# Xiugapurin/Etude

Measured on AMD Instinct MI355X. Metric: audio-sec/s transcribed + decoder tokens/s, 3-min clip batch, higher is better.
Workload: dtype f16

## Files before the change

etude_amd/_lib.py:

```python
from __future__ import annotations

import ctypes as C
import os
from pathlib import Path

import torch

LIB_PATH = Path(os.environ["ETD_LIB_PATH"]) if os.environ.get("ETD_LIB_PATH") else Path(__file__).resolve().parent / "libetude_hip.so"

c_int_p = C.POINTER(C.c_int)
c_i32_p = C.POINTER(C.c_int32)
c_i64_p = C.POINTER(C.c_int64)
c_f32_p = C.POINTER(C.c_float)


class _SizedCfg(C.Structure):

    def __init__(self, *a, **k):
        super().__init__(*a, **k)
        self.struct_bytes = C.sizeof(type(self))


class ExtCfg(_SizedCfg):
    _fields_ = [("struct_bytes", C.c_int)] + [(n, C.c_int) for n in ("n_margin", "n_frame", "n_bin", "cnn_channel", "cnn_kernel", "hid_dim", "pf_dim",
# ... 13 lines not shown
    _fields_ = [("struct_bytes", C.c_int)] + [(n, C.c_int) for n in ("attn_len", "instr", "ntoken", "dmodel", "nhead", "d_hid", "nlayers", "norm_first",
                                       "n_mels", "tempo_out", "max_rows")]


class DbnCfg(_SizedCfg):
    _fields_ = [("struct_bytes", C.c_int), ("fps", C.c_double), ("min_bpm", C.c_double), ("max_bpm", C.c_double), ("transition_lambda", C.c_double),
                ("observation_lambda", C.c_double), ("threshold", C.c_double), ("correct", C.c_int), ("num_tempi", C.c_int), ("n_bars", C.c_int),
                ("beats_per_bar", C.c_int * 8)]


class StemFeatCfg(_SizedCfg):
    _fields_ = [("struct_bytes", C.c_int), ("n_fft", C.c_int), ("hop", C.c_int), ("n_mels", C.c_int), ("framing", C.c_int), ("amin", C.c_float), ("top_db", C.c_float)]


class DtwCfg(_SizedCfg):
    _fields_ = [("struct_bytes", C.c_int), ("cens_window", C.c_int), ("cens_decimation", C.c_int), ("reserved", C.c_int), ("step_weights", C.c_double * 3),
                ("shift_weights", C.c_double * 3), ("alpha", C.c_float), ("norm_threshold", C.c_float)]


class G3Case(_SizedCfg):
    _fields_ = [("struct_bytes", C.c_int), ("kernel", C.c_int), ("epi", C.c_int)] + [(n, C.c_int) for n in ("M", "N", "K", "ldx", "ldy")] + \
               [("X", C.c_void_p), ("x_elems", C.c_longlong), ("W", C.c_void_p), ("bias", C.c_void_p), ("x_bound", C.c_float),
                ("ln_g", C.c_void_p), ("ln_b", C.c_void_p), ("ln_eps", C.c_float), ("Y", C.c_void_p), ("y_elems", C.c_longlong),
                ("add", C.c_void_p), ("hin", C.c_void_p), ("hout", C.c_void_p), ("h_elems", C.c_longlong),
                ("pos", C.c_void_p), ("slot", C.c_void_p), ("active", C.c_void_p)] + [(n, C.c_int) for n in ("n_heads", "max_ctx", "n_slots", "rope_rows")] + \
               [("rope_cos", C.c_void_p), ("rope_sin", C.c_void_p), ("Q", C.c_void_p), ("q_elems", C.c_longlong), ("Kc", C.c_void_p), ("Vc", C.c_void_p), ("kv_elems", C.c_longlong)]


G3_KERNEL_AUTO, G3_KERNEL_TILE, G3_KERNEL_SMALL = 0, 1, 2
G3_EPI = {"bias": 0, "gelu": 1, "resid": 2, "logits": 3, "qkv": 4, "relu": 6}


class Job(C.Structure):
    _fields_ = [("x_ids", C.c_void_p), ("x_offsets", C.c_void_p), ("n_bars", C.c_int), ("attrs4", C.c_void_p), ("ready", C.c_void_p)]


class ScoreJob(C.Structure):
    _fields_ = [("x_ids", C.c_void_p), ("x_offsets", C.c_void_p), ("n_bars", C.c_int), ("attrs4", C.c_void_p),
                ("y_ids", C.c_void_p), ("y_offsets", C.c_void_p), ("n_y_bars", C.c_int)]


class SchedCfg(_SizedCfg):
    _fields_ = [("struct_bytes", C.c_int)] + [(n, C.c_int) for n in ("bar_bos_id", "bar_eos_id", "n_ctx_pairs", "max_position_embeddings", "max_output_tokens",
                                       "max_bar_token_limit")] + [("context_overlap_ratio", C.c_float)] + \
               [(n, C.c_int) for n in ("force_bar_tokens", "max_streams", "max_prefill_rows", "steps_per_poll")] + \
               [("temperature", C.c_float), ("top_p", C.c_float), ("seed", C.c_ulonglong), ("job_key_offset", C.c_int), ("job_key_stride", C.c_int)]


class TempoRegion(C.Structure):
    _fields_ = [("bpm", C.c_double), ("time_sig", C.c_int), ("start", C.c_double), ("downbeats", C.c_void_p), ("n_downbeats", C.c_int)]


class TokEvent(C.Structure):
    _fields_ = [("type", C.c_int32), ("value", C.c_int32)]


class Note(C.Structure):
    _fields_ = [("onset", C.c_double), ("offset", C.c_double), ("pitch", C.c_int32), ("velocity", C.c_int32)]


ABI_VERSION = 3

SIGNATURES = {
    "etd_version": (C.c_int, []),
    "etd_last_error": (C.c_char_p, []),
    "etd_build_id": (C.c_char_p, []),
    "etd_extractor_operand_type": (C.c_int, []),
    "etd_decoder_operand_type": (C.c_int, []),
    "etd_has_experiments": (C.c_int, []),
    "etd_prof_enable": (C.c_int, [C.c_int]),
    "etd_prof_reset": (C.c_int, []),
    "etd_prof_collect": (C.c_int, []),
    "etd_prof_count": (C.c_int, []),
    "etd_prof_entry": (C.c_int, [C.c_int, C.c_char_p, C.c_int, C.POINTER(C.c_double), C.POINTER(C.c_longlong),
                                 C.POINTER(C.c_double), C.POINTER(C.c_double)]),
    "etd_debug_boundary_cost": (C.c_int, [C.c_int, C.c_int, C.c_int, C.c_void_p, C.POINTER(C.c_double), C.POINTER(C.c_double)]),
    "etd_debug_linear": (C.c_int, [C.c_int, C.c_int, C.c_int, C.c_int, C.c_void_p, C.POINTER(C.c_double)]),
    "etd_debug_kernel_loop": (C.c_int, [C.c_int, C.c_int, C.c_void_p]),
    "etd_debug_g3_bounds": (C.c_int, [C.c_void_p, C.c_void_p, C.c_int, C.c_int, C.c_void_p, C.c_void_p, C.c_float, C.c_void_p, C.c_void_p]),
    "etd_debug_gemm3": (C.c_int, [C.c_void_p, C.c_int, C.c_int, C.c_void_p, C.c_void_p, C.c_int, C.c_float, C.c_int, C.c_void_p, C.c_void_p, C.c_void_p, C.c_void_p]),
    "etd_debug_gemm3_case": (C.c_int, [C.POINTER(G3Case), C.c_void_p]),
    "etd_debug_ln_rows_f32": (C.c_int, [C.c_void_p, C.c_int, C.c_int, C.c_void_p, C.c_void_p, C.c_void_p, C.c_void_p, C.c_float, C.c_void_p, C.c_void_p, C.c_void_p]),
    "etd_debug_g3_pack": (C.c_int, [C.c_void_p, C.c_int, C.c_int, C.c_void_p, C.c_longlong, C.POINTER(C.c_longlong), C.POINTER(C.c_int32)]),
    "etd_debug_attn3": (C.c_int, [C.c_void_p, C.c_void_p, C.c_void_p, C.c_void_p, C.c_int, C.c_int, C.c_int, C.c_int, C.c_float, C.c_float, C.c_float, C.c_int, C.c_void_p, C.c_void_p]),
    "etd_debug_empty_launch": (C.c_int, [C.c_int, C.c_int, C.c_int, C.c_void_p, C.c_void_p]),
    "etd_frontend_create": (C.c_int, [C.c_int, C.c_int, C.c_int, C.c_int, C.c_int, C.c_int, C.c_void_p, C.c_int, C.c_int,
                                      C.c_void_p, C.c_int, C.c_void_p, C.c_void_p, C.c_void_p, C.c_float, C.POINTER(C.c_void_p)]),
    "etd_frontend_destroy": (None, [C.c_void_p]),
    "etd_frontend_set_pad_mode": (C.c_int, [C.c_void_p, C.c_int]),
    "etd_rms_frames": (C.c_int, [C.c_void_p, C.c_longlong, C.c_int, C.c_int, C.c_void_p, C.c_longlong, C.c_void_p]),
    "etd_frontend_resampled_len": (C.c_longlong, [C.c_void_p, C.c_longlong]),
    "etd_frontend_num_frames": (C.c_longlong, [C.c_void_p, C.c_longlong]),
    "etd_frontend_run": (C.c_int, [C.c_void_p, C.c_void_p, C.c_int, C.c_longlong, C.c_void_p, C.c_void_p, C.c_longlong,
                                   C.POINTER(C.c_longlong), C.c_void_p]),
    "etd_extractor_create": (C.c_int, [C.POINTER(ExtCfg), C.POINTER(C.c_char_p), C.POINTER(C.c_void_p), c_i64_p, C.c_int,
                                       C.POINTER(C.c_void_p)]),
    "etd_extractor_destroy": (None, [C.c_void_p]),
    "etd_transcript": (C.c_int, [C.c_void_p, C.c_void_p, C.c_longlong] + [C.c_void_p] * 8 + [C.c_void_p]),
    "etd_transcript_windows": (C.c_int, [C.c_void_p, C.c_void_p, C.c_int] + [C.c_void_p] * 8 + [C.c_void_p]),
    "etd_extractor_debug_vel_logits": (C.c_int, [C.c_void_p, C.c_void_p]),
    "etd_extractor_debug_tap": (C.c_int, [C.c_void_p, C.c_int, C.c_void_p]),
    "etd_extractor_window_flops": (C.c_double, [C.c_void_p]),
    "etd_mpe2note": (C.c_int, [C.c_void_p, C.c_void_p, C.c_void_p, C.c_void_p, C.c_longlong, C.c_int, C.c_float, C.c_float,
                               C.c_float, C.c_int, C.c_int, C.c_int, C.POINTER(Note), C.c_longlong, C.POINTER(C.c_longlong)]),
    "etd_mpe2note_modes": (C.c_int, [C.c_void_p, C.c_void_p, C.c_void_p, C.c_void_p, C.c_longlong, C.c_int, C.c_float, C.c_float,
                                     C.c_float, C.c_int, C.c_int, C.c_int, C.c_int, C.c_int, C.POINTER(Note), C.c_longlong, C.POINTER(C.c_longlong)]),
    "etd_mpe2note_dev_create": (C.c_int, [C.c_int, C.POINTER(C.c_void_p)]),
    "etd_mpe2note_dev_destroy": (None, [C.c_void_p]),
    "etd_mpe2note_dev": (C.c_int, [C.c_void_p, C.c_void_p, C.c_void_p, C.c_void_p, C.c_void_p, C.c_longlong, C.c_float, C.c_float, C.c_float,
                                   C.c_int, C.c_int, C.c_int, C.POINTER(Note), C.c_longlong, C.POINTER(C.c_longlong), C.c_void_p]),
    "etd_mpe2note_dev_modes": (C.c_int, [C.c_void_p, C.c_void_p, C.c_void_p, C.c_void_p, C.c_void_p, C.c_longlong, C.c_float, C.c_float, C.c_float,
                                         C.c_int, C.c_int, C.c_int, C.c_int, C.c_int, C.POINTER(Note), C.c_longlong, C.POINTER(C.c_longlong), C.c_void_p]),
    "etd_tok_create": (C.c_int, [C.c_void_p, C.c_int, C.POINTER(C.c_void_p)]),
    "etd_tok_destroy": (None, [C.c_void_p]),
    "etd_tok_num_measures": (C.c_int, [C.c_void_p]),
    "etd_tok_measures": (C.c_int, [C.c_void_p, C.c_void_p, C.c_void_p, C.c_void_p, C.c_void_p]),
    "etd_tok_encode": (C.c_int, [C.c_void_p, C.c_void_p, C.c_longlong, C.c_int, C.c_void_p, C.c_longlong, C.POINTER(C.c_longlong)]),
    "etd_tok_split_bars": (C.c_int, [C.c_void_p, C.c_longlong, C.c_int, C.c_int, C.c_void_p, C.c_longlong, C.c_void_p, C.c_longlong,
                                     C.POINTER(C.c_longlong)]),
    "etd_tok_decode": (C.c_int, [C.c_void_p, C.c_void_p, C.c_longlong, C.c_void_p, C.c_longlong, C.c_void_p, C.c_longlong,
                                 C.POINTER(C.c_longlong)]),
    "etd_midi_write": (C.c_int, [C.c_void_p, C.c_longlong, C.c_char_p]),
    "etd_decoder_create": (C.c_int, [C.POINTER(DecCfg), C.POINTER(C.c_char_p), C.POINTER(C.c_void_p), c_i64_p, C.c_int,
                                     C.POINTER(C.c_void_p)]),
    "etd_decoder_destroy": (None, [C.c_void_p]),
    "etd_decoder_clone": (C.c_int, [C.c_void_p, C.POINTER(C.c_void_p)]),
    "etd_decoder_set_sampling": (C.c_int, [C.c_void_p, C.c_float, C.c_float, C.c_ulonglong, C.c_void_p]),
    "etd_decoder_set_keys": (C.c_int, [C.c_void_p, C.c_int, C.c_void_p, C.c_void_p]),
    "etd_decoder_begin_bar": (C.c_int, [C.c_void_p, C.c_int, C.c_void_p, C.c_void_p, C.c_void_p, C.c_int, C.c_void_p, C.c_int,
                                        C.c_int, C.c_void_p]),
    "etd_decoder_begin_bars": (C.c_int, [C.c_void_p, C.c_int] + [C.c_void_p] * 8 + [C.c_void_p]),
    "etd_decoder_step": (C.c_int, [C.c_void_p, C.c_void_p, C.c_int, C.c_int, C.c_void_p]),
    "etd_decoder_poll": (C.c_int, [C.c_void_p, C.c_void_p, C.c_int, C.c_void_p, C.c_void_p, C.c_void_p]),
    "etd_decoder_read_tokens": (C.c_int, [C.c_void_p, C.c_int, C.c_void_p, C.c_int, c_int_p, C.c_void_p]),
    "etd_decoder_read_many": (C.c_int, [C.c_void_p, C.c_int, C.c_void_p, C.c_void_p, C.c_int, C.c_void_p, C.c_void_p]),
    "etd_decoder_run_jobs": (C.c_int, [C.c_void_p, C.POINTER(SchedCfg), C.POINTER(Job), C.c_int, C.c_void_p, C.c_longlong, C.c_void_p,
                                       C.POINTER(C.c_longlong), C.c_void_p]),
    "etd_debug_assemble_prompt": (C.c_int, [C.POINTER(SchedCfg), C.c_int, C.c_void_p, C.c_void_p, C.c_void_p, C.c_void_p, C.c_void_p, C.c_void_p,
                                            C.c_int, C.c_void_p, C.c_void_p, C.c_void_p, C.c_void_p, C.c_int, c_int_p]),
    "etd_decoder_generate_bar": (C.c_int, [C.c_void_p, C.c_int, C.c_void_p, C.c_void_p, C.c_void_p, C.c_int, C.c_void_p,
                                           C.c_int, C.c_int, C.c_void_p, c_int_p, C.c_void_p]),
    "etd_decoder_prefill_logits": (C.c_int, [C.c_void_p, C.c_int, C.c_void_p, C.c_void_p, C.c_void_p, C.c_int, C.c_void_p,
                                             C.c_void_p]),
    "etd_decoder_score": (C.c_int, [C.c_void_p, C.c_int] + [C.c_void_p] * 11 + [C.c_void_p]),
    "etd_decoder_score_jobs": (C.c_int, [C.c_void_p, C.POINTER(SchedCfg), C.POINTER(ScoreJob), C.c_int, C.c_void_p, C.c_void_p, C.c_void_p, C.c_void_p]),
    "etd_debug_assemble_scored": (C.c_int, [C.POINTER(SchedCfg), C.c_int, C.c_void_p, C.c_void_p, C.c_void_p, C.c_void_p, C.c_void_p, C.c_void_p,
                                            C.c_int, C.c_void_p, C.c_int, C.c_void_p, C.c_void_p, C.c_void_p, C.c_void_p, C.c_void_p, C.c_int, c_int_p]),
    "etd_decoder_step_bytes": (C.c_double, [C.c_void_p, C.c_int, C.c_int]),
    "etd_decoder_stats": (C.c_int, [C.c_void_p, C.POINTER(C.c_double), C.c_int, C.c_void_p]),
    "etd_decoder_stats_reset": (C.c_int, [C.c_void_p, C.c_void_p]),
    "etd_decoder_stamp": (C.c_int, [C.c_void_p, C.c_int, C.c_int, C.c_void_p]),
    "etd_decoder_stamp_log": (C.c_int, [C.c_void_p, C.c_void_p, C.c_longlong, C.POINTER(C.c_longlong), C.c_void_p]),
    "etd_debug_decoder_force_pair": (C.c_int, [C.c_void_p, C.c_int]),
    "etd_debug_decoder_step_logits": (C.c_int, [C.c_void_p, C.c_int, C.c_void_p, C.c_int, C.c_void_p]),
    "etd_debug_decoder_checksum": (C.c_int, [C.c_void_p, C.POINTER(C.c_ulonglong), C.c_int, C.c_void_p]),
    "etd_debug_decoder_kv_rowsums": (C.c_int, [C.c_void_p, C.c_void_p, C.c_longlong, C.c_void_p]),
    "etd_debug_decoder_trace_begin": (C.c_int, [C.c_void_p, C.c_int, C.c_void_p]),
    "etd_debug_decoder_trace_slabs": (C.c_int, [C.c_void_p, C.c_void_p, C.c_longlong, C.c_int, C.c_void_p]),
    "etd_debug_decoder_trace_lanes": (C.c_int, [C.c_void_p, C.c_void_p, C.c_longlong, C.c_int, C.c_void_p]),
    "etd_debug_decoder_trace_q": (C.c_int, [C.c_void_p, C.c_void_p, C.c_longlong, C.c_int, C.c_void_p]),
    "etd_debug_decoder_peek_kv": (C.c_int, [C.c_void_p, C.c_int, C.c_int, C.c_int, C.c_int, C.c_void_p, C.c_void_p, C.c_void_p]),
    "etd_beat_create": (C.c_int, [C.POINTER(BeatCfg), C.POINTER(C.c_char_p), C.POINTER(C.c_void_p), c_i64_p, C.c_int, C.POINTER(C.c_void_p)]),
    "etd_beat_destroy": (None, [C.c_void_p]),
    "etd_beat_forward": (C.c_int, [C.c_void_p, C.c_void_p, C.c_int, c_i64_p, C.c_void_p, C.c_void_p, C.c_void_p]),
    "etd_beat_flops": (C.c_double, [C.c_void_p, C.c_longlong]),
    "etd_beat_debug_taps": (C.c_int, [C.c_void_p, C.c_void_p, C.c_void_p]),
    "etd_dbn_describe": (C.c_int, [C.POINTER(DbnCfg), C.c_int, C.c_void_p, C.c_int, c_int_p, c_int_p, c_int_p, C.c_void_p, C.c_void_p]),
    "etd_dbn_workspace_bytes": (C.c_longlong, [C.POINTER(DbnCfg), C.c_longlong, C.c_int]),
    "etd_dbn_create": (C.c_int, [C.POINTER(DbnCfg), C.POINTER(C.c_void_p)]),
    "etd_dbn_destroy": (None, [C.c_void_p]),
    "etd_dbn_track": (C.c_int, [C.c_void_p, C.c_void_p, C.c_int, C.c_int, c_i64_p, C.c_void_p, C.c_longlong, C.c_void_p, C.c_void_p, C.c_void_p, C.c_longlong,
                                C.c_void_p, C.c_void_p, C.POINTER(C.c_longlong), C.c_void_p]),
    "etd_dbn_debug_viterbi": (C.c_int, [C.c_void_p, C.c_int, C.c_void_p, C.c_longlong, C.c_void_p, C.POINTER(C.c_double)]),
    "etd_stemfeat_create": (C.c_int, [C.POINTER(StemFeatCfg), C.c_void_p, C.c_void_p, C.c_void_p, C.c_void_p, C.POINTER(C.c_void_p)]),
    "etd_stemfeat_destroy": (None, [C.c_void_p]),
    "etd_stemfeat_num_frames": (C.c_longlong, [C.c_void_p, C.c_longlong]),
    "etd_stemfeat_workspace_bytes": (C.c_longlong, [C.c_void_p, C.c_int, C.c_int, c_i64_p]),
    "etd_stemfeat_run": (C.c_int, [C.c_void_p, C.POINTER(C.c_void_p), C.c_int, C.c_int, C.c_int, c_i64_p, C.c_void_p, C.c_void_p]),
    "etd_dtw_create": (C.c_int, [C.POINTER(DtwCfg), C.POINTER(C.c_void_p)]),
    "etd_dtw_destroy": (None, [C.c_void_p]),
    "etd_dtw_limits": (C.c_int, [c_int_p, c_int_p, C.POINTER(C.c_longlong), c_int_p]),
    "etd_dtw_workspace_bytes": (C.c_longlong, [C.c_void_p, C.c_int, c_i64_p, c_i64_p, C.POINTER(C.c_longlong), c_i64_p]),
    "etd_dtw_align": (C.c_int, [C.c_void_p, C.POINTER(C.c_void_p), C.c_int, c_i64_p, c_i64_p, C.c_void_p, C.c_longlong, C.c_void_p, C.c_longlong, C.c_void_p, C.c_void_p]),
    "etd_dtw_debug_cost": (C.c_int, [C.c_void_p, C.POINTER(C.c_void_p), C.c_longlong, C.c_longlong, C.c_int, C.c_void_p]),
    "etd_dtw_debug_path": (C.c_int, [C.c_void_p, C.POINTER(C.c_void_p), C.c_longlong, C.c_longlong, C.c_int, C.c_void_p, C.c_longlong, C.POINTER(C.c_longlong)]),
    "etd_dtw_debug_total": (C.c_int, [C.c_void_p, C.POINTER(C.c_void_p), C.c_longlong, C.c_longlong, C.c_int, C.POINTER(C.c_double)]),
    "etd_debug_decoder_trace_read": (C.c_int, [C.c_void_p, C.c_void_p, C.c_longlong, C.c_int, C.POINTER(C.c_int), C.c_void_p]),
}

_lib = None


class EtudeHipError(RuntimeError):
    pass


def lib() -> C.CDLL:
    global _lib
    if _lib is None:
        if not LIB_PATH.exists():
            raise EtudeHipError(f"{LIB_PATH} not found: build it with `python -m etude_amd.build` "
                                "(hipcc --offload-arch=gfx950); etude_amd has no CPU fallback")
        l = C.CDLL(str(LIB_PATH))
        for name, (res, args) in SIGNATURES.items():
            if os.environ.get("ETD_PARTIAL") and not hasattr(l, name):
                continue
            fn = getattr(l, name)
            fn.restype = res
            fn.argtypes = args
        if l.etd_version() != ABI_VERSION:
            raise EtudeHipError(f"{LIB_PATH} speaks ABI version {l.etd_version()}, this binding {ABI_VERSION}; rebuild with `python -m etude_amd.build`")
        if not os.environ.get("ETD_PARTIAL") and not os.environ.get("ETD_ALLOW_STALE_LIB"):
            from .build import src_hash
            have, want = (l.etd_build_id() or b"").decode(), src_hash()
            if have != want:
                raise EtudeHipError(f"{LIB_PATH} is stale: built from sources {have}, the tree is {want}; rebuild with `python -m etude_amd.build`")
        _lib = l
    return _lib


def check(rc: int, what: str = "") -> None:
    if rc != 0:
        msg = lib().etd_last_error()
        raise EtudeHipError(f"{what} failed (rc={rc}): {msg.decode() if msg else ''}")


def weights_arrays(state: dict):
    import numpy as np
    names = list(state.keys())
    arrs = [np.ascontiguousarray(np.asarray(state[k], dtype=np.float32)) for k in names]
    c_names = (C.c_char_p * len(names))(*[k.encode() for k in names])
    c_ptrs = (C.c_void_p * len(names))(*[a.ctypes.data for a in arrs])
    c_num = (C.c_int64 * len(names))(*[a.size for a in arrs])
    return c_names, c_ptrs, c_num, len(names), arrs


def prof_enable(on: bool) -> None:
    lib().etd_prof_enable(1 if on else 0)


def prof_reset() -> None:
    lib().etd_prof_reset()


def prof_report() -> dict:
    l = lib()
    l.etd_prof_collect()
    out = {}
    for i in range(l.etd_prof_count()):
        name = C.create_string_buffer(64)
        ms, n, fl, by = C.c_double(), C.c_longlong(), C.c_double(), C.c_double()
        check(l.etd_prof_entry(i, name, 64, C.byref(ms), C.byref(n), C.byref(fl), C.byref(by)), "etd_prof_entry")
        out[name.value.decode()] = dict(ms=ms.value, launches=n.value, flops=fl.value, bytes=by.value)
    return out
```

etude_amd/csrc/api_dec.hip:

```cpp
#include <algorithm>
#include <atomic>
#include <chrono>
#include <cmath>
#include <cstdlib>
#include <cstring>
#include <map>
#include <string>
#include <mutex>
#include <vector>

#include "../../include/etude_hip_debug.h"
#include "dec_kernels.h"
#include "gemm3.h"
#include "ext_kernels.h"
#include "dec_score.h"
#include "prof.h"

namespace {

inline uint16_t f2bf_h(float f) { return ETD_DEC_IS_F16 ? f32_to_f16_bits(f) : f32_to_bf16_bits(f); }

struct Lin { void* W = nullptr; float* b = nullptr; int N = 0, Npad = 0, K = 0;
             void* Wf = nullptr;
             G3Lin g3; };
struct Layer { float *ln1g, *ln1b, *ln2g, *ln2b; Lin qkv, dense, up, down;
               void* dense_hw = nullptr;
               Lin cat;
               void* mlp_frag = nullptr;
               int q_log2 = 0, k_log2 = 0, v_log2 = 0; };

}

#define ETD_STAMP_WORDS (ETD_STAMP_HDR + 2 * ETD_STAMP_LOGCAP)
struct etd_dec {
  etd_dec_cfg cfg;
  DevPool pool;
  bool bf16w = false;
  int H, I, V, L, nh, S, ctx, Mmax, Mcap, out_cap;
  float *word = nullptr, *cls_emb = nullptr, *attr_tab = nullptr;
  std::vector<Layer> layers;
  float *lnfg = nullptr, *lnfb = nullptr;
  Lin head;
  float *X1f = nullptr, *X2f = nullptr;
  float *t_q = nullptr, *t_ao = nullptr, *t_do = nullptr, *t_m1 = nullptr;
  void* head_frag = nullptr;
  float *rope_cos = nullptr, *rope_sin = nullptr;
  void *Kc = nullptr, *Vc = nullptr;
  long long slot_stride = 0, layer_stride = 0;
  float *h = nullptr, *h2 = nullptr, *Q = nullptr, *AO = nullptr, *DO = nullptr, *M1 = nullptr, *logits = nullptr;
  int *row_slot = nullptr, *row_pos = nullptr, *row_active = nullptr, *row_sp = nullptr, *ids = nullptr, *slots_dev = nullptr;
  int *cur_tok = nullptr, *len = nullptr, *done = nullptr, *n_out = nullptr, *eos = nullptr, *limit = nullptr, *tgt_attrs = nullptr, *out_tok = nullptr;
  float* tgt_proj = nullptr;
  std::vector<int> last_slots;
  float* qkv_raw = nullptr;
  d16 *X1b = nullptr, *X2b = nullptr, *AOb = nullptr, *M1b = nullptr;
  d16* Qb = nullptr;
  float* hlast = nullptr;
  DSampleCfg* samp_dev = nullptr;
  unsigned long long* rng_key = nullptr;
  std::vector<unsigned long long> host_key; bool keys_dirty = true; bool sampling = false;
  float* Pk = nullptr;
  unsigned* trace = nullptr; int* trace_step = nullptr; int trace_cap = 0; float* trace_pk = nullptr; float* trace_q = nullptr; float* trace_dbg = nullptr;
  int* row_cnt = nullptr;
  d16* Xcat = nullptr;
  std::vector<int> stage;
  int* pin_stage = nullptr; size_t pin_stage_ints = 0; hipEvent_t pin_stage_evt = nullptr;
  int* pin_rb = nullptr;
  std::vector<int> host_n_out; bool host_n_out_valid = false;
  std::map<int, hipGraphExec_t> graphs;
  bool rows_identity = false;
  std::vector<int> host_len;
  double attn_bytes_hint = 0;
  bool step_pair = false;
  double stat_steps = 0, stat_row_steps = 0, stat_kv_bytes = 0, stat_attn_launches = 0, stat_stamp_bytes = 0;
  int force_pair = -1;
  unsigned long long* stamp_dev = nullptr;
  bool stamp_on = false, stamp_armed = false; long long stamp_skip = 0;
  float* logits_dbg = nullptr; bool logits_dbg_on = false, last_step_fused = false;
  int* sc_i = nullptr; float* sc_f = nullptr; double* sc_d = nullptr; float* sc_x = nullptr; int score_hb = 0;
  etd_dec* weights_owner = nullptr;
  size_t n_weight_allocs = 0;
  int n_clones = 0; bool zombie = false;
};

namespace {

int load_lin(etd_dec* d, const WeightTable& L, const std::string& pfx, int N, int K, bool has_bias, Lin* w) {
  const float* W = L.get(pfx + ".weight", (int64_t)N * K);
  if (!W) return ETD_EINVAL;
  const float* b = nullptr;
  if (has_bias) { b = L.get(pfx + ".bias", N); if (!b) return ETD_EINVAL; }
  const int Npad = ((N + 127) / 128) * 128;
  w->N = N; w->Npad = Npad; w->K = K;
  DevPool& P = d->pool;
  if (d->bf16w) {
    std::vector<uint16_t> hb((size_t)Npad * K, 0);
    for (size_t i = 0; i < (size_t)N * K; ++i) hb[i] = f2bf_h(W[i]);
    uint16_t* p; ETD_TRY(P.upload(&p, hb.data(), hb.size()));
    w->W = p;
    if (K % 16 == 0) {
      std::vector<uint16_t> hp(hb.size());
      pack_wfrag_host(hb.data(), Npad, K, hp.data());
      uint16_t* pf; ETD_TRY(P.upload(&pf, hp.data(), hp.size()));
      w->Wf = pf;
    }
  } else {
    std::vector<float> hf((size_t)Npad * K, 0.f);
    memcpy(hf.data(), W, (size_t)N * K * 4);
    float* p; ETD_TRY(P.upload(&p, hf.data(), hf.size()));
    w->W = p;
    if (K % 32 == 0) {
      ETD_TRY(g3_lin_upload(P, W, b, N, K, 0.f, &w->g3));
      w->b = w->g3.b;
      return ETD_OK;
    }
  }
  std::vector<float> hb2(Npad, 0.f);
  if (b) memcpy(hb2.data(), b, (size_t)N * 4);
  return P.upload(&w->b, hb2.data(), hb2.size());
}

int load_vec(etd_dec* d, const WeightTable& L, const std::string& name, int n, float** dst) {
  const float* p = L.get(name, n);
  if (!p) return ETD_EINVAL;
  return d->pool.upload(dst, p, n);
}

struct PrefillInfo { int n; const int* seq_row0; const int* seq_len; int max_len; double attn_flops; };
__global__ __launch_bounds__(64) void k_trace_rows(const unsigned* buf, long long row_stride, int words, long long slab_stride, int M,
                                                   unsigned* trace, const int* step, int cap, long long wps, int off) {
  const int row = blockIdx.x, slab = blockIdx.y, lane = threadIdx.x;
  const unsigned* p = buf + (long long)slab * slab_stride + (long long)row * row_stride;
  unsigned acc = 0;
  for (int i = lane; i < words; i += 64) acc += p[i] * (2654435761u * (unsigned)(i + 1) | 1u);
  for (int o = 32; o; o >>= 1) acc += __shfl_xor(acc, o);
  if (lane == 0) trace[(long long)(*step % cap) * wps + off + slab * M + row] = acc;
}
__global__ __launch_bounds__(64) void k_trace_kv(const unsigned* Kc, const unsigned* Vc, long long slot_stride_w, int max_ctx, const int* row_slot, const int* row_pos, int M,
                                                 unsigned* trace, const int* step, int cap, long long wps, int off) {
  const int row = blockIdx.x, head = blockIdx.y, lane = threadIdx.x;
  const int slot = row_slot[row], pos = row_pos[row] < max_ctx ? row_pos[row] : max_ctx - 1;
  unsigned* out = trace + (long long)(*step % cap) * wps + off;
  for (int which = 0; which < 2; ++which) {
    const unsigned* base = (which ? Vc : Kc) + (long long)slot * slot_stride_w + (long long)head * max_ctx * 32;
    unsigned a_new = 0, a_all = 0;
    for (long long i = lane; i < (long long)(pos + 1) * 32; i += 64) {
      const unsigned w = base[i] * (2654435761u * (unsigned)(i + 1) | 1u);
      a_all += w;
      if (i >= (long long)pos * 32) a_new += w;
    }
    for (int o = 32; o; o >>= 1) { a_new += __shfl_xor(a_new, o); a_all += __shfl_xor(a_all, o); }
    if (lane == 0) { out[(which * 8 + head) * M + row] = a_new; out[(16 + which * 8 + head) * M + row] = a_all; }
  }
}
__global__ void k_trace_next(int* step) { *step += 1; }
#define ETD_TRACE_LAYER 49
static inline long long trace_wps(const etd_dec* d, int M) { return (long long)(ETD_TRACE_LAYER * d->L + 2) * M; }
static int trace_rows(etd_dec* d, const void* buf, long long row_stride, int words, int nslab, long long slab_stride, int M, int off, hipStream_t st) {
  hipLaunchKernelGGL(k_trace_rows, dim3(M, nslab), dim3(64), 0, st, (const unsigned*)buf, row_stride, words, slab_stride, M, d->trace, d->trace_step,
                     d->trace_cap, trace_wps(d, M), off);
  HIP_TRY(hipGetLastError());
  return ETD_OK;
}

static inline bool fused_pmlp_on() { const char* e = getenv("ETD_FUSED_PMLP"); return !e || atoi(e) > 0; }
struct LastOnly { int n; const int* idx; DecRows rows; };
constexpr int DS_K_SPLITS = 5;
static inline bool ksplit_fits(const etd_dec* d) { return (d->I + d->H) % (DS_K_SPLITS * 64 * 8) == 0; }
static inline bool step_shape(const etd_dec* d) { return ksplit_fits(d) && d->H == 512; }
#ifdef ETD_EXPERIMENTS
static inline bool rowfin_on() { static const bool on = getenv("ETD_ROWFIN") && atoi(getenv("ETD_ROWFIN")) > 0; return on; }
#else
static inline bool rowfin_on() { return false; }
#endif

static DGemmArgs lin_args(const Lin& w, const float* X, int ldx, int M) {
  DGemmArgs a = {};
  a.X = X; a.ldx = ldx; a.M = M; a.W = w.W; a.Wf = w.Wf; a.bias = w.b; a.N = w.N; a.Npad = w.Npad; a.K = w.K; a.Wp = w.g3.Wp; a.w_log2 = w.g3.w_log2; a.x_log2 = w.g3.x_log2;
  return a;
}
static inline void* kv_layer(const etd_dec* d, void* cache, int l) { return (char*)cache + (size_t)l * d->layer_stride * (d->bf16w ? 2 : 4); }
static DGemmArgs qkv_args(const etd_dec* d, int l, const float* X, const DecRows& rows, int M) {
  DGemmArgs q = lin_args(d->layers[l].qkv, X, d->H, M);
  q.rows = rows; q.rope_cos = d->rope_cos; q.rope_sin = d->rope_sin; q.rot_half = 8; q.Q = d->Q;
  q.Kc = kv_layer(d, d->Kc, l); q.Vc = kv_layer(d, d->Vc, l); q.slot_stride = d->slot_stride; q.max_ctx = d->ctx; q.n_heads = d->nh;
  return q;
}
static DAttnArgs attn_args(const etd_dec* d, int l, const DecRows& rows, int M) {
  DAttnArgs at = {};
  at.Q = d->Q; at.Kc = kv_layer(d, d->Kc, l); at.Vc = kv_layer(d, d->Vc, l); at.slot_stride = d->slot_stride; at.max_ctx = d->ctx; at.n_heads = d->nh;
  at.rows = rows; at.M = M; at.scale = 0.125f; at.bytes_hint = d->attn_bytes_hint;
  return at;
}
static inline void attn_step_pairs(const etd_dec* d, DAttnArgs* at) { at->row_sp = d->row_sp; at->identity = d->rows_identity ? 1 : 0; }
static inline void attn_stamp(const etd_dec* d, int l, DAttnArgs* at) { at->stamp = d->stamp_on ? d->stamp_dev : nullptr; at->stamp_par = l & 1; }
struct NextLn { const float *g1, *b1, *g2, *b2; d16 *x1, *x2; };
static NextLn next_ln(const etd_dec* d, int l) {
  const Layer* nx = l + 1 < d->L ? &d->layers[l + 1] : nullptr;
  return nx ? NextLn{nx->ln1g, nx->ln1b, nx->ln2g, nx->ln2b, d->X1b, d->X2b} : NextLn{};
}
static int ln_rows16(etd_dec* d, int l, const float* h, int M, hipStream_t st) {
  const Layer& w = d->layers[l];
  return launch_ln_rows(h, M, d->H, w.ln1g, w.ln1b, w.ln2g, w.ln2b, d->cfg.layer_norm_eps, d->X1b, d->X2b, st);
}
static int layer_dattn(etd_dec* d, int l, const DecRows& rows, int M, d16* Ob, int ldob, hipStream_t st) {
  DAttnArgs at = attn_args(d, l, rows, M); at.O = d->AO; at.Ob = Ob; at.ldob = ldob;
  if (rows.slot == d->row_slot) { attn_step_pairs(d, &at); attn_stamp(d, l, &at); }
  return launch_dattn(at, d->bf16w, st);
}
static int step_qkv_up(etd_dec* d, int l, const float* X, const DecRows& rows, int M, hipStream_t st) {
  DGemmArgs q = qkv_args(d, l, X, rows, M); q.Xb = d->X1b; q.Y = d->qkv_raw; q.ldy = 3 * d->H;
  DGemmArgs up = lin_args(d->layers[l].up, X, d->H, M); up.Xb = d->X2b; up.Y = d->M1; up.Yb = d->Xcat; up.ldy = d->I + d->H;
  return launch_dstep_qkv_up(q, up, st);
}
static int resid_ln(etd_dec* d, int l, int nslab, const float* hin, float* hout, int M, const NextLn& nx, hipStream_t st) {
  return launch_resid_ln_rows(d->Pk, nslab, d->layers[l].cat.b, nullptr, hin, hout, M, d->H, nx.g1, nx.b1, nx.g2, nx.b2, d->cfg.layer_norm_eps, nx.x1, nx.x2, st);
}
static int down_splitk(etd_dec* d, int l, const float* hin, float* hout, int M, const NextLn& nx, hipStream_t st) {
  DGemmArgs dn = lin_args(d->layers[l].cat, d->M1, d->I + d->H, M); dn.Xb = d->Xcat; dn.hin = hin; dn.hout = hout; dn.k_splits = DS_K_SPLITS; dn.Y = d->Pk; dn.ldy = d->H;
  ETD_TRY(launch_dgemm(dn, DEPI_PARTIAL, true, st));
  return resid_ln(d, l, DS_K_SPLITS, hin, hout, M, nx, st);
}
static int linear16(const Lin& w, const d16* X, int M, const DGemmArgs& dec, int epi, hipStream_t st) {
  LinArgs a = {};
  a.X = (const e16*)X; a.ldx = w.K; a.W = (const e16*)w.Wf;
  a.bias = w.b; a.M = M; a.N = w.N; a.K = w.K; a.vt_block = -1; a.dec = dec;
  return launch_linear_dec(a, epi, st);
}

static int gemm3_auto(const DGemmArgs& a, int epi, hipStream_t st) { return gemm3_s_takes(a, epi) ? launch_gemm3_s(a, epi, st) : launch_gemm3(a, epi, st); }
static int x3_last_rows(etd_dec* d, const LastOnly& lo, const float* hin, float* hout, hipStream_t st) {
  const int n = lo.n, l = d->L - 1, H = d->H; const Layer& w = d->layers[l];
  ETD_TRY(launch_gather_rows(hin, lo.idx, n, H, d->hlast, st)); ETD_TRY(launch_gather_rows(d->Q, lo.idx, n, H, d->t_q, st));
  DAttnArgs at = attn_args(d, l, lo.rows, n); at.Q = d->t_q; at.O = d->t_ao; at.bytes_hint = 0;
  ETD_TRY(launch_dattn(at, false, st));
  DGemmArgs de = lin_args(w.dense, d->t_ao, H, n); de.Y = d->t_do; de.ldy = H;
  ETD_TRY(launch_dgemm(de, DEPI_BIAS, false, st));
  DGemmArgs up = lin_args(w.up, d->hlast, H, n); up.Y = d->t_m1; up.ldy = d->I; up.ln_g = w.ln2g; up.ln_b = w.ln2b; up.ln_eps = d->cfg.layer_norm_eps;
  ETD_TRY(launch_dgemm(up, DEPI_GELU, false, st));
  DGemmArgs dn = lin_args(w.down, d->t_m1, d->I, n); dn.add = d->t_do; dn.hin = d->hlast; dn.hout = hout;
  return launch_dgemm(dn, DEPI_RESID, false, st);
}
static int x3_layer_rest(etd_dec* d, int l, const DecRows& rows, int M, const PrefillInfo* pf, const float* hin, float* hout, hipStream_t st) {
  const Layer& w = d->layers[l]; const int H = d->H;
  if (pf) {
    Attn3Args t = {};
    t.Q = d->Q; t.ldq = H; t.K = (const float*)kv_layer(d, d->Kc, l); t.V = (const float*)kv_layer(d, d->Vc, l); t.O = d->AO; t.ldo = H; t.n_seq = pf->n; t.n_heads = d->nh;
    t.seq_row0 = pf->seq_row0; t.seq_len = pf->seq_len; t.row_slot = rows.slot; t.slot_stride = d->slot_stride; t.max_ctx = d->ctx; t.max_len = pf->max_len;
    t.scale = 0.125f; t.q_log2 = w.q_log2; t.k_log2 = w.k_log2; t.v_log2 = w.v_log2; t.flops_hint = pf->attn_flops;
    ETD_TRY(launch_attn3(t, st));
  } else {
    DAttnArgs at = attn_args(d, l, rows, M);
    at.O = d->AO; attn_stamp(d, l, &at);
    if (rows.slot == d->row_slot) attn_step_pairs(d, &at);
    ETD_TRY(launch_dattn(at, false, st));
  }
  DGemmArgs de = lin_args(w.dense, d->AO, H, M); de.Y = d->DO; de.ldy = H;
  ETD_TRY(gemm3_auto(de, DEPI_BIAS, st));
  DGemmArgs up = lin_args(w.up, d->X2f, H, M); up.Y = d->M1; up.ldy = d->I;
  ETD_TRY(gemm3_auto(up, DEPI_GELU, st));
  DGemmArgs dn = lin_args(w.down, d->M1, d->I, M); dn.add = d->DO; dn.hin = hin; dn.hout = hout;
  return gemm3_auto(dn, DEPI_RESID, st);
}
static int forward_x3(etd_dec* d, int M, const DecRows& rows, const PrefillInfo* pf, const LastOnly* lo, hipStream_t st, float** hfinal, bool* compact) {
  const bool tail = lo && pf && lo->n >= 1 && lo->n < G3_MIN_ROWS && lo->n <= d->S;
  float* hin = d->h; float* hout = d->h2;
  for (int l = 0; l < d->L; ++l) {
    const Layer& w = d->layers[l];
    ETD_TRY(launch_ln_rows_f32(hin, M, d->H, w.ln1g, w.ln1b, w.ln2g, w.ln2b, d->cfg.layer_norm_eps, d->X1f, d->X2f, st));
    ETD_TRY(gemm3_auto(qkv_args(d, l, d->X1f, rows, M), DEPI_QKV, st));
    ETD_TRY(tail && l == d->L - 1 ? x3_last_rows(d, *lo, hin, hout, st) : x3_layer_rest(d, l, rows, M, pf, hin, hout, st));
    std::swap(hin, hout);
  }
  *hfinal = hin; if (tail) *compact = true;
  return ETD_OK;
}

static int forward_plain(etd_dec* d, int M, const DecRows& rows, bool act16, hipStream_t st, float** hfinal) {
  float* hin = d->h; float* hout = d->h2; const float eps = d->cfg.layer_norm_eps;
  for (int l = 0; l < d->L; ++l) {
    const Layer& w = d->layers[l];
    if (act16) ETD_TRY(ln_rows16(d, l, hin, M, st));
    DGemmArgs q = qkv_args(d, l, hin, rows, M); q.Y = d->qkv_raw; q.ldy = 3 * d->H;
    if (act16) q.Xb = d->X1b; else { q.ln_g = w.ln1g; q.ln_b = w.ln1b; q.ln_eps = eps; }
    ETD_TRY(launch_dgemm(q, DEPI_QKV, d->bf16w, st));
    ETD_TRY(layer_dattn(d, l, rows, M, act16 ? d->AOb : nullptr, 0, st));
    DGemmArgs de = lin_args(w.dense, d->AO, d->H, M); de.Y = d->DO; de.ldy = d->H; if (act16) de.Xb = d->AOb;
    ETD_TRY(launch_dgemm(de, DEPI_BIAS, d->bf16w, st));
    DGemmArgs up = lin_args(w.up, hin, d->H, M); up.Y = d->M1; up.ldy = d->I;
    if (act16) { up.Xb = d->X2b; up.Yb = d->M1b; } else { up.ln_g = w.ln2g; up.ln_b = w.ln2b; up.ln_eps = eps; }
    ETD_TRY(launch_dgemm(up, DEPI_GELU, d->bf16w, st));
    DGemmArgs dn = lin_args(w.down, d->M1, d->I, M); dn.add = d->DO; dn.hin = hin; dn.hout = hout; if (act16) dn.Xb = d->M1b;
    ETD_TRY(launch_dgemm(dn, DEPI_RESID, d->bf16w, st));
    std::swap(hin, hout);
  }
  *hfinal = hin;
  return ETD_OK;
}

static int trace_qkv_up(etd_dec* d, int l, int M, hipStream_t st) {
  if (!d->trace) return ETD_OK;
  ETD_TRY(trace_rows(d, d->Q, d->H, d->H, 1, 0, M, l * ETD_TRACE_LAYER * M, st));
  if (l == 0) HIP_TRY(hipMemcpyAsync(d->trace_q, d->Q, (size_t)M * d->H * 4, hipMemcpyDeviceToDevice, st));
  ETD_TRY(trace_rows(d, d->Xcat, (d->I + d->H) / 2, d->I / 2, 1, 0, M, l * ETD_TRACE_LAYER * M + M, st));
  if (d->nh == 8) {
    hipLaunchKernelGGL(k_trace_kv, dim3(M, 8), dim3(64), 0, st, (const unsigned*)kv_layer(d, d->Kc, l), (const unsigned*)kv_layer(d, d->Vc, l), d->slot_stride / 2, d->ctx,
                       d->row_slot, d->row_pos, M, d->trace, d->trace_step, d->trace_cap, trace_wps(d, M), l * ETD_TRACE_LAYER * M + 17 * M);
    HIP_TRY(hipGetLastError());
  }
  return ETD_OK;
}
static int skinny_attn_down(etd_dec* d, int l, const DecRows& rows, int M, const float* hin, float* hout, hipStream_t st) {
  const Layer& w = d->layers[l]; const NextLn nx = next_ln(d, l);
  const int ksd = d->I / 512;
  DAttnArgs at = attn_args(d, l, rows, M);
  attn_step_pairs(d, &at); attn_stamp(d, l, &at); at.pair = d->step_pair ? 1 : 0;
  at.dense_w = (const d16*)w.dense_hw; at.dense_out = d->Pk + (size_t)ksd * M * d->H; at.dbg = (d->trace && l == 0) ? d->trace_dbg : nullptr;
  DGemmArgs dn = lin_args(w.cat, nullptr, d->I + d->H, M); dn.Xb = d->Xcat; dn.k_splits = ksd; dn.Y = d->Pk; dn.ldy = d->H;
  if (rowfin_on() && ksd + d->nh == 12 && M <= DS_STEP_MAX_ROWS) {
    DRowFin fin = {};
    fin.cnt = d->row_cnt + (size_t)l * DS_STEP_MAX_ROWS; fin.target = d->nh + 16 * ksd; fin.P = d->Pk; fin.nslab = 12;
    fin.bias = w.cat.b; fin.hin = hin; fin.hout = hout; fin.eps = d->cfg.layer_norm_eps;
    fin.g1 = nx.g1; fin.b1 = nx.b1; fin.g2 = nx.g2; fin.b2 = nx.b2; fin.x1 = nx.x1; fin.x2 = nx.x2;
    return launch_dstep_attn_down(at, dn, &fin, st);
  }
  ETD_TRY(launch_dstep_attn_down(at, dn, nullptr, st));
  if (d->trace && ksd + d->nh == 12) ETD_TRY(trace_rows(d, d->Pk, d->H, d->H, 12, (long long)M * d->H, M, l * ETD_TRACE_LAYER * M + 2 * M, st));
  if (d->trace && l == 0 && ksd + d->nh == 12) HIP_TRY(hipMemcpyAsync(d->trace_pk, d->Pk, (size_t)12 * M * d->H * 4, hipMemcpyDeviceToDevice, st));
  ETD_TRY(resid_ln(d, l, ksd + d->nh, hin, hout, M, nx, st));
  if (d->trace) {
    ETD_TRY(trace_rows(d, hout, d->H, d->H, 1, 0, M, l * ETD_TRACE_LAYER * M + 14 * M, st));
    if (nx.x1) {
      ETD_TRY(trace_rows(d, d->X1b, d->H / 2, d->H / 2, 1, 0, M, l * ETD_TRACE_LAYER * M + 15 * M, st));
      ETD_TRY(trace_rows(d, d->X2b, d->H / 2, d->H / 2, 1, 0, M, l * ETD_TRACE_LAYER * M + 16 * M, st));
    }
  }
  return ETD_OK;
}
static int forward_skinny16(etd_dec* d, int M, const DecRows& rows, bool ln0_done, hipStream_t st, float** hfinal) {
  const bool attn_down = rows.slot == d->row_slot && d->H == 512 && d->nh == 8 && d->I % 512 == 0 && d->I / 512 + d->nh <= 12 && d->layers[0].dense_hw &&
                         d->ctx >= 256 && !getenv("ETD_NO_ATTN_DOWN");
  float* hin = d->h; float* hout = d->h2;
  if (!ln0_done) ETD_TRY(ln_rows16(d, 0, hin, M, st));
  for (int l = 0; l < d->L; ++l) {
    ETD_TRY(step_qkv_up(d, l, hin, rows, M, st));
    ETD_TRY(trace_qkv_up(d, l, M, st));
    if (attn_down) ETD_TRY(skinny_attn_down(d, l, rows, M, hin, hout, st));
    else { ETD_TRY(layer_dattn(d, l, rows, M, d->Xcat + d->I, d->I + d->H, st)); ETD_TRY(down_splitk(d, l, hin, hout, M, next_ln(d, l), st)); }
    std::swap(hin, hout);
  }
  *hfinal = hin;
  return ETD_OK;
}

static int prefill16_qkv(etd_dec* d, int l, const float* hin, const DecRows& rows, int M, bool mfma_attn, hipStream_t st) {
  const Layer& w = d->layers[l];
  DGemmArgs q = qkv_args(d, l, hin, rows, M); q.Xb = d->X1b; q.Y = d->qkv_raw; q.ldy = 3 * d->H;
  if (mfma_attn) q.Qb = d->Qb;
  static const bool pqkv_on = !getenv("ETD_NO_PQKV");
  if (!(mfma_attn && pqkv_on && M >= 49152 && d->H == 512 && d->nh == 8 && w.qkv.N == 1536)) return linear16(w.qkv, d->X1b, M, q, DEPI_QKV, st);
  PQkvArgs pa = {};
  pa.X = d->X1b; pa.ldx = d->H; pa.Wf = (const d16*)w.qkv.Wf; pa.bias = w.qkv.b; pa.M = M; pa.N = w.qkv.N; pa.rows = rows;
  pa.rope_cos = d->rope_cos; pa.rope_sin = d->rope_sin; pa.Qb = d->Qb; pa.Kc = (d16*)q.Kc; pa.Vc = (d16*)q.Vc; pa.slot_stride = d->slot_stride; pa.max_ctx = d->ctx; pa.n_heads = d->nh;
  return launch_pqkv(pa, st);
}
static int prefill16_layer_rest(etd_dec* d, int l, const DecRows& rows, int M, const PrefillInfo* pf, bool fmlp, const float* hin, float* hout, hipStream_t st) {
  const Layer& w = d->layers[l];
  if (pf) {
    PAttnArgs t = {};
    t.Q = d->Qb; t.ldq = d->H; t.Kc = (const d16*)kv_layer(d, d->Kc, l); t.Vc = (const d16*)kv_layer(d, d->Vc, l); t.slot_stride = d->slot_stride; t.max_ctx = d->ctx; t.n_heads = d->nh;
    t.O = d->Xcat + d->I; t.ldo = d->I + d->H; t.seq_row0 = pf->seq_row0; t.seq_len = pf->seq_len; t.row_slot = rows.slot;
    t.n_seq = pf->n; t.max_len = pf->max_len; t.scale_log2e = 0.125f * 1.4426950408889634f; t.flops_hint = pf->attn_flops;
    ETD_TRY(launch_pattn(t, st));
  } else ETD_TRY(layer_dattn(d, l, rows, M, d->Xcat + d->I, d->I + d->H, st));
  if (fmlp) {
    const NextLn nx = next_ln(d, l); DMlpArgs ma = {};
    ma.X2 = d->X2b; ma.AO = d->Xcat + d->I; ma.ldao = d->I + d->H; ma.hin = hin; ma.hout = hout; ma.Wm = (const d16*)w.mlp_frag;
    ma.b_up = w.up.b; ma.b_cat = w.cat.b; ma.eps = d->cfg.layer_norm_eps; ma.M = M;
    ma.g1 = nx.g1; ma.b1 = nx.b1; ma.g2 = nx.g2; ma.b2 = nx.b2; ma.nx1 = nx.x1; ma.nx2 = nx.x2;
    return launch_dmlp_fused(ma, st);
  }
  DGemmArgs up = {}; up.Yb = d->Xcat; up.ldy = d->I + d->H;
  ETD_TRY(linear16(w.up, d->X2b, M, up, DEPI_GELU, st));
  DGemmArgs dn = {}; dn.N = d->H; dn.hin = hin; dn.hout = hout;
  return linear16(w.cat, d->Xcat, M, dn, DEPI_RESID, st);
}
static int prefill16_last_rows(etd_dec* d, const LastOnly& lo, const float* hin, float* hout, hipStream_t st) {
  const int n = lo.n, l = d->L - 1;
  ETD_TRY(launch_gather_rows(hin, lo.idx, n, d->H, d->hlast, st));
  ETD_TRY(ln_rows16(d, l, d->hlast, n, st));
  ETD_TRY(step_qkv_up(d, l, d->hlast, lo.rows, n, st));
  DAttnArgs at = attn_args(d, l, lo.rows, n); at.O = d->AO; at.Ob = d->Xcat + d->I; at.ldob = d->I + d->H; at.bytes_hint = 0;
  ETD_TRY(launch_dattn(at, d->bf16w, st));
  return down_splitk(d, l, d->hlast, hout, n, NextLn{}, st);
}
static int forward_prefill16(etd_dec* d, int M, const DecRows& rows, const PrefillInfo* pf, const LastOnly* lo, hipStream_t st, float** hfinal, bool* compact) {
  const bool fmlp = d->layers[0].mlp_frag && d->H == 512 && d->I == 2048 && fused_pmlp_on();
  const bool tail = lo && pf && lo->n > 1 && lo->n <= DS_STEP_MAX_ROWS && step_shape(d) && !getenv("ETD_NO_LAST_ONLY");
  float* hin = d->h; float* hout = d->h2;
  for (int l = 0; l < d->L; ++l) {
    if (l == 0 || !fmlp) ETD_TRY(ln_rows16(d, l, hin, M, st));
    ETD_TRY(prefill16_qkv(d, l, hin, rows, M, pf != nullptr, st));
    ETD_TRY(tail && l == d->L - 1 ? prefill16_last_rows(d, *lo, hin, hout, st) : prefill16_layer_rest(d, l, rows, M, pf, fmlp, hin, hout, st));
    std::swap(hin, hout);
  }
  *hfinal = hin; if (tail) *compact = true;
  return ETD_OK;
}

static int forward_rows(etd_dec* d, int M, const DecRows& rows, const PrefillInfo* pf, const LastOnly* lo, hipStream_t st, float** hfinal, bool* compact) {
  if (compact) *compact = false; else lo = nullptr;
  const Layer& w0 = d->layers[0];
  if (!d->bf16w && M >= G3_MIN_ROWS && d->X1f && w0.qkv.g3.Wp && w0.down.g3.Wp && g3_enabled()) return forward_x3(d, M, rows, pf, lo, st, hfinal, compact);
  const bool act16 = d->bf16w && M > 1;
  if (act16 && M > DS_MAX_ROWS && w0.qkv.Wf && w0.up.Wf && w0.cat.Wf) return forward_prefill16(d, M, rows, pf, lo, st, hfinal, compact);
  if (act16 && ksplit_fits(d)) return forward_skinny16(d, M, rows, false, st, hfinal);
  return forward_plain(d, M, rows, act16, st, hfinal);
}

int head_logits(etd_dec* d, const float* X, int n, float* logits, hipStream_t st) {
  const bool g3 = !d->bf16w && n >= G3_MIN_ROWS && d->X1f && d->head.g3.Wp && g3_enabled();
  if (g3) ETD_TRY(launch_ln_rows_f32(X, n, d->H, d->lnfg, d->lnfb, nullptr, nullptr, d->cfg.layer_norm_eps, d->X1f, nullptr, st));
  DGemmArgs lm = lin_args(d->head, g3 ? d->X1f : X, d->H, n);
  lm.bias = nullptr; lm.Y = logits; lm.ldy = d->V;
  if (g3) return launch_gemm3(lm, DEPI_LOGITS, st);
  lm.ln_g = d->lnfg; lm.ln_b = d->lnfb; lm.ln_eps = d->cfg.layer_norm_eps;
  return launch_dgemm(lm, DEPI_LOGITS, d->bf16w, st);
}

int check_slot(etd_dec* d, int slot) {
  if (!d || slot < 0 || slot >= d->S) ETD_FAIL(ETD_EINVAL, "decoder: bad slot %d", slot);
  return ETD_OK;
}

__global__ void k_init_slots(const int* __restrict__ init, int n, int* tgt_attrs, int* cur_tok, int* len, int* done, int* n_out, int* eos, int* limit) {
  const int i = blockIdx.x * blockDim.x + threadIdx.x;
  if (i >= n) return;
  const int* p = init + i * 7;
  const int s = p[0];
  tgt_attrs[4 * s] = p[1]; tgt_attrs[4 * s + 1] = p[2]; tgt_attrs[4 * s + 2] = p[3]; tgt_attrs[4 * s + 3] = p[4];
  cur_tok[s] = 0; len[s] = 0; done[s] = 0; n_out[s] = 0; eos[s] = p[5]; limit[s] = p[6];
}

__global__ __launch_bounds__(128) void k_slot_proj(const int* __restrict__ init, const float* __restrict__ attr_tab, int n_bins, int H, float* proj) {
  const int* p = init + blockIdx.x * 7;
  const int s = p[0];
  for (int k = threadIdx.x * 4; k < H; k += 128 * 4) {
    f32x4 t[4];
#pragma unroll
    for (int a = 0; a < 4; ++a) t[a] = *reinterpret_cast<const f32x4*>(attr_tab + (long long)(a * n_bins + p[1 + a]) * H + k);
    f32x4 o;
#pragma unroll
    for (int c = 0; c < 4; ++c) o[c] = ((t[0][c] + t[1][c]) + t[2][c]) + t[3][c];
    *reinterpret_cast<f32x4*>(proj + (long long)s * H + k) = o;
  }
}

struct Staged { int Mtot; const int *ids, *cls, *attrs, *row_slot, *row_pos, *row_active, *last_idx, *last_slot, *last_pos, *last_active, *init, *row_seq, *seq_row0, *seq_len; };

int stage_and_forward(etd_dec* d, int n, const int32_t* slots, const int32_t* T, const int32_t* ids, const int32_t* cls,
                      const int32_t* attrs4, const int32_t* init7 , Staged* sg, float** hfinal, hipStream_t st, bool* last_only = nullptr) {
  if (!d || n < 1 || n > d->S || !slots || !T || !ids || !cls || !attrs4) ETD_FAIL(ETD_EINVAL, "prefill: bad arguments");
  long long Mtot = 0;
  std::vector<char> seen((size_t)d->S, 0);
  for (int i = 0; i < n; ++i) {
    ETD_TRY(check_slot(d, slots[i]));
    if (T[i] <= 0 || T[i] > d->ctx) ETD_FAIL(ETD_EINVAL, "prefill: prompt %d has T=%d (max_ctx=%d)", i, T[i], d->ctx);
    if (seen[slots[i]]) ETD_FAIL(ETD_EINVAL, "prefill: slot %d listed twice", slots[i]);
    seen[slots[i]] = 1;
    Mtot += T[i];
  }
  if (Mtot > d->Mcap) ETD_FAIL(ETD_EINVAL, "prefill: %lld prompt rows exceed max_prefill_rows=%d", Mtot, d->Mcap);
  const int M = (int)Mtot;
  for (int i = 0; i < M; ++i) {
    if (ids[i] < 0 || ids[i] >= d->V || cls[i] < 0 || cls[i] >= d->cfg.num_classes) ETD_FAIL(ETD_EINVAL, "prefill: token/class id out of range at row %d", i);
    for (int k = 0; k < 4; ++k) if (attrs4[(size_t)k * M + i] < 0 || attrs4[(size_t)k * M + i] >= d->cfg.num_attribute_bins) ETD_FAIL(ETD_EINVAL, "prefill: attribute bin out of range at row %d", i);
  }
  const size_t sv_ints = (size_t)10 * M + 13 * n;
  int* svp;
  const bool pinned = d->pin_stage && sv_ints <= d->pin_stage_ints;
  if (pinned) {
    HIP_TRY(hipEventSynchronize(d->pin_stage_evt));
    svp = d->pin_stage;
  } else {
    d->stage.resize(sv_ints);
    svp = d->stage.data();
  }
  memcpy(svp, ids, (size_t)M * 4);
  memcpy(svp + M, cls, (size_t)M * 4);
  memcpy(svp + 2 * (size_t)M, attrs4, (size_t)4 * M * 4);
  int* rs = svp + 6 * (size_t)M; int* rp = rs + M; int* ra = rp + M;
  int* li = ra + M; int* ls = li + n; int* lp = ls + n; int* la = lp + n; int* in7 = la + n;
  int* rq = in7 + 7 * n; int* sr0 = rq + M; int* sln = sr0 + n;
  int row = 0, max_len = 0; double kvb = 0, aflops = 0;
  for (int i = 0; i < n; ++i) {
    sr0[i] = row; sln[i] = T[i]; if (T[i] > max_len) max_len = T[i];
    aflops += 0.5 * 256.0 * d->nh * (double)T[i] * T[i];
    for (int t = 0; t < T[i]; ++t, ++row) { rs[row] = slots[i]; rp[row] = t; ra[row] = 1; rq[row] = i; }
    li[i] = row - 1; ls[i] = slots[i]; lp[i] = T[i] - 1; la[i] = 1;
    d->host_len[slots[i]] = T[i];
    kvb += (double)T[i] * d->nh * 64 * (2.0 * (d->bf16w ? 2 : 4) + 4 + 4);
  }
  if (init7) memcpy(in7, init7, (size_t)7 * n * 4); else memset(in7, 0, (size_t)7 * n * 4);
  d->attn_bytes_hint = kvb;
  HIP_TRY(hipMemcpyAsync(d->ids, svp, sv_ints * 4, hipMemcpyHostToDevice, st));
  if (pinned) HIP_TRY(hipEventRecord(d->pin_stage_evt, st));
  d->host_n_out_valid = false;
  const int* b = d->ids;
  *sg = Staged{M, b, b + M, b + 2 * (size_t)M, b + 6 * (size_t)M, b + 7 * (size_t)M, b + 8 * (size_t)M, b + 9 * (size_t)M, b + 9 * (size_t)M + n,
               b + 9 * (size_t)M + 2 * n, b + 9 * (size_t)M + 3 * n, b + 9 * (size_t)M + 4 * n,
               b + 9 * (size_t)M + 11 * n, b + 10 * (size_t)M + 11 * n, b + 10 * (size_t)M + 12 * n};
  if (init7) {
    hipLaunchKernelGGL(k_init_slots, dim3((n + 63) / 64), dim3(64), 0, st, sg->init, n, d->tgt_attrs, d->cur_tok, d->len, d->done, d->n_out, d->eos, d->limit);
    HIP_TRY(hipGetLastError());
    hipLaunchKernelGGL(k_slot_proj, dim3(n), dim3(128), 0, st, sg->init, d->attr_tab, d->cfg.num_attribute_bins, d->H, d->tgt_proj);
    HIP_TRY(hipGetLastError());
  }
  DEmbedArgs e = {};
  e.ids = sg->ids; e.cls = sg->cls; e.attrs = sg->attrs; e.M = M; e.H = d->H; e.n_bins = d->cfg.num_attribute_bins;
  e.word = d->word; e.cls_emb = d->cls_emb; e.attr_tab = d->attr_tab; e.h = d->h;
  e.rows = DecRows{sg->row_slot, sg->row_pos, sg->row_active, sg->row_seq};
  ETD_TRY(launch_dembed(e, st));
  PrefillInfo pf{n, sg->seq_row0, sg->seq_len, max_len, aflops};
  const bool can_mfma_attn = (d->bf16w ? d->Qb != nullptr : d->X1f != nullptr) && !ETD_XENV("ETD_NO_MFMA_PREFILL_ATTN");
  LastOnly lo{n, sg->last_idx, DecRows{sg->last_slot, sg->last_pos, sg->last_active}};
  return forward_rows(d, M, e.rows, can_mfma_attn ? &pf : nullptr, &lo, st, hfinal, last_only);
}

int alloc_workspaces(etd_dec* d) {
  const int H = d->H;
  DevPool& P = d->pool;
  d->slot_stride = (long long)d->nh * d->ctx * 64;
  d->layer_stride = d->slot_stride * d->S;
  const size_t kv_elems = (size_t)d->layer_stride * d->L;
  if (d->bf16w) { uint16_t *k, *v; ETD_TRY(P.alloc(&k, kv_elems, true)); ETD_TRY(P.alloc(&v, kv_elems, true)); d->Kc = k; d->Vc = v; }
  else { float *k, *v; ETD_TRY(P.alloc(&k, kv_elems, true)); ETD_TRY(P.alloc(&v, kv_elems, true)); d->Kc = k; d->Vc = v; }
  const size_t M = d->Mcap;
  const size_t Mf = d->bf16w ? (size_t)(d->S > 1 ? d->S : 1) : M;
  ETD_TRY(P.alloc(&d->h, M * H)); ETD_TRY(P.alloc(&d->h2, M * H));
  ETD_TRY(P.alloc(&d->Q, M * H)); ETD_TRY(P.alloc(&d->AO, M * H)); ETD_TRY(P.alloc(&d->DO, M * H));
  ETD_TRY(P.alloc(&d->M1, Mf * d->I)); ETD_TRY(P.alloc(&d->logits, (size_t)d->Mmax * d->V));
  ETD_TRY(P.alloc(&d->qkv_raw, (size_t)3 * H)); ETD_TRY(P.alloc(&d->hlast, (size_t)d->S * H));
  if (d->bf16w) {
    ETD_TRY(P.alloc(&d->X1b, M * H)); ETD_TRY(P.alloc(&d->X2b, M * H)); ETD_TRY(P.alloc(&d->AOb, M * H));
    ETD_TRY(P.alloc(&d->M1b, M * d->I));
    ETD_TRY(P.alloc(&d->Pk, (size_t)12 * DS_STEP_MAX_ROWS * H));
    ETD_TRY(P.alloc(&d->row_cnt, (size_t)d->L * DS_STEP_MAX_ROWS, true));
    ETD_TRY(P.alloc(&d->Xcat, M * (d->I + H)));
    ETD_TRY(P.alloc(&d->Qb, M * H));
  }
  if (!d->bf16w) {
    ETD_TRY(P.alloc(&d->X1f, M * H)); ETD_TRY(P.alloc(&d->X2f, M * H));
    const size_t Sr = d->S > 1 ? d->S : 1;
    ETD_TRY(P.alloc(&d->t_q, Sr * H)); ETD_TRY(P.alloc(&d->t_ao, Sr * H)); ETD_TRY(P.alloc(&d->t_do, Sr * H)); ETD_TRY(P.alloc(&d->t_m1, Sr * d->I));
  }
  ETD_TRY(P.alloc(&d->samp_dev, (size_t)1, true)); ETD_TRY(P.alloc(&d->rng_key, (size_t)d->S, true));
// ... 368 lines not shown
    d->step_pair = d->force_pair < 0 ? pair : (d->force_pair > 0 && n_active >= 2);
  }
  d->rows_identity = true;
  for (int i = 0; i < n_active; ++i) if (slots[i] != i) { d->rows_identity = false; break; }
  const int vpad = (d->V + 31) / 32 * 32;
  static const bool fused_m1 = !(ETD_XENV("ETD_FUSED_M1") && atoi(ETD_XENV("ETD_FUSED_M1")) == 0);
  const bool fused = d->bf16w && (n_active > 1 || fused_m1) && n_active <= DS_STEP_MAX_ROWS && step_shape(d) && vpad <= 256 &&
                     vpad <= d->head.Npad && d->head_frag && !ETD_XENV("ETD_NO_FUSED_STEP");
  d->last_step_fused = fused;
  d->stamp_on = d->stamp_armed && d->stamp_skip <= 0;
  if (d->stamp_armed && d->stamp_skip > 0) d->stamp_skip -= n_steps;
  auto embed = [&](hipStream_t s_) -> int {
    DEmbedArgs e = {};
    e.slots = d->slots_dev; e.len = d->len; e.done = d->done; e.row_slot_out = d->row_slot; e.row_pos_out = d->row_pos; e.row_active_out = d->row_active; e.row_sp_out = d->row_sp;
    e.cur_tok = d->cur_tok; e.tgt_attrs = d->tgt_attrs; e.tgt_cls = 2 ;
    e.M = n_active; e.H = d->H; e.n_bins = d->cfg.num_attribute_bins;
    e.word = d->word; e.cls_emb = d->cls_emb; e.attr_tab = d->attr_tab; e.h = d->h;
    e.rows = DecRows{d->row_slot, d->row_pos, d->row_active};
    return launch_dembed(e, s_);
  };
  const double kv_row_bytes = (double)d->nh * 64 * 2 * (d->bf16w ? 2 : 4);
  auto step_kv_bytes = [&](int s) {
    double b = 0;
    for (int i = 0; i < n_active; ++i) { const int c = d->host_len[slots[i]] + 1 + s; b += (double)(c < d->ctx ? c : d->ctx) * kv_row_bytes; }
    return b;
  };
  int eager_step = 0;
  auto one_step = [&](hipStream_t s_) -> int {
    d->attn_bytes_hint = step_kv_bytes(eager_step);
    ++eager_step;
    const DecRows rows{d->row_slot, d->row_pos, d->row_active};
    if (!fused) ETD_TRY(embed(s_));
    float* hf = nullptr;
    ETD_TRY(fused ? forward_skinny16(d, n_active, rows, true, s_, &hf) : forward_rows(d, n_active, rows, nullptr, nullptr, s_, &hf, nullptr));
    if (fused) {
      ETD_TRY(launch_dstep_head(head_args(d, hf, n_active, vpad), s_));
      if (d->trace) {
        ETD_TRY(trace_rows(d, d->h, d->H, d->H, 1, 0, n_active, ETD_TRACE_LAYER * d->L * n_active, s_));
        ETD_TRY(trace_rows(d, d->cur_tok, 1, 1, 1, 0, n_active, ETD_TRACE_LAYER * d->L * n_active + n_active, s_));
        hipLaunchKernelGGL(k_trace_next, dim3(1), dim3(1), 0, s_, d->trace_step);
      }
      return ETD_OK;
    }
    ETD_TRY(head_logits(d, hf, n_active, d->logits, s_));
    DArgmaxArgs am = argmax_args(d, rows, n_active);
    am.samp = d->samp_dev; am.rng_key = d->rng_key;
    ETD_TRY(launch_dargmax(am, s_));
    return ETD_OK;
  };
  if (fused) {
    ETD_TRY(embed(st));
    ETD_TRY(ln_rows16(d, 0, d->h, n_active, st));
  }
  const bool use_graph = st != nullptr && !prof_enabled() && !ETD_XENV("ETD_NO_GRAPH");
  if (use_graph) {
    const int gkey = 16 * n_active + (d->logits_dbg_on ? 8 : 0) + (d->stamp_on ? 4 : 0) + (d->step_pair ? 2 : 0) + (d->rows_identity ? 1 : 0);
    auto it = d->graphs.find(gkey);
    if (it == d->graphs.end()) {
      hipGraph_t g = nullptr;
      HIP_TRY(hipStreamBeginCapture(st, hipStreamCaptureModeThreadLocal));
      const int rc = one_step(st);
      const hipError_t ce = hipStreamEndCapture(st, &g);
      eager_step = 0;
      if (rc != ETD_OK) { if (g) (void)hipGraphDestroy(g); return rc; }
      if (ce != hipSuccess || !g) ETD_FAIL(ETD_EHIP, "decoder_step: stream capture failed: %s", hipGetErrorString(ce));
      hipGraphExec_t ge = nullptr;
      const hipError_t ie = hipGraphInstantiate(&ge, g, nullptr, nullptr, 0);
      (void)hipGraphDestroy(g);
      if (ie != hipSuccess) ETD_FAIL(ETD_EHIP, "decoder_step: graph instantiate failed: %s", hipGetErrorString(ie));
      it = d->graphs.emplace(gkey, ge).first;
    }
    for (int s = 0; s < n_steps; ++s) HIP_TRY(hipGraphLaunch(it->second, st));
  } else {
    for (int s = 0; s < n_steps; ++s) ETD_TRY(one_step(st));
  }
  {
    double kv = 0;
    for (int s2 = 0; s2 < n_steps; ++s2) kv += step_kv_bytes(s2);
    kv *= d->L;
    d->stat_steps += n_steps; d->stat_row_steps += (double)n_steps * n_active; d->stat_kv_bytes += kv; d->stat_attn_launches += (double)n_steps * d->L;
    if (d->stamp_on) d->stat_stamp_bytes += kv + (fused ? (double)n_steps * d->L * ((double)d->I + d->H) * d->H * 2.0 : 0.0);
    for (int i = 0; i < n_active; ++i) { int& hl = d->host_len[slots[i]]; hl = hl + n_steps < d->ctx - 1 ? hl + n_steps : d->ctx - 1; }
  }
  return ETD_OK;
}

extern "C" int etd_decoder_stats(etd_dec* d, double* out, int n, void* stream) {
  if (!d || !out || n < 1) ETD_FAIL(ETD_EINVAL, "decoder_stats: bad arguments");
  unsigned long long sum_ticks = 0, n_stamped = 0;
  if (d->stamp_dev) {
    std::vector<unsigned long long> sp(ETD_STAMP_HDR);
    HIP_TRY(hipStreamSynchronize((hipStream_t)stream));
    HIP_TRY(hipMemcpy(sp.data(), d->stamp_dev, ETD_STAMP_HDR * 8, hipMemcpyDeviceToHost));
    sum_ticks = sp[0]; n_stamped = sp[1];
    for (int bank = 0; bank < 2; ++bank) {
      unsigned long long e = 0;
      for (int i = 0; i < 64; ++i) e = std::max(e, sp[8 + 64 * bank + i]);
      if (sp[2 + bank] != 0 && e > sp[2 + bank]) { sum_ticks += e - sp[2 + bank]; ++n_stamped; }
    }
  }
  double w = 0;
  for (const Layer& l : d->layers) w += ((double)l.qkv.N * l.qkv.K + (double)l.dense.N * l.dense.K + (double)l.up.N * l.up.K + (double)l.down.N * l.down.K) * (d->bf16w ? 2.0 : 4.0);
  w += (double)d->V * d->H * (d->bf16w ? 2.0 : 4.0);
  const double v[8] = {d->stat_steps, d->stat_row_steps, d->stat_kv_bytes, d->stat_attn_launches, (double)n_stamped, (double)sum_ticks * 1e-8 , d->stat_stamp_bytes, w};
  for (int i = 0; i < n; ++i) out[i] = i < 8 ? v[i] : 0.0;
  return ETD_OK;
}

extern "C" int etd_decoder_stamp_log(etd_dec* d, unsigned long long* out_pairs, long long cap, long long* n, void* stream) {
  if (!d || !out_pairs || cap < 1 || !n) ETD_FAIL(ETD_EINVAL, "decoder_stamp_log: bad arguments");
  *n = 0;
  if (!d->stamp_dev) return ETD_OK;
  std::vector<unsigned long long> sp(ETD_STAMP_WORDS);
  HIP_TRY(hipStreamSynchronize((hipStream_t)stream));
  HIP_TRY(hipMemcpy(sp.data(), d->stamp_dev, ETD_STAMP_WORDS * 8, hipMemcpyDeviceToHost));
  long long k = (long long)std::min<unsigned long long>(sp[1], ETD_STAMP_LOGCAP), w = 0;
  for (long long i = 0; i < k && w < cap; ++i, ++w) { out_pairs[2 * w] = sp[ETD_STAMP_HDR + 2 * i]; out_pairs[2 * w + 1] = sp[ETD_STAMP_HDR + 2 * i + 1]; }
  for (int bank = 0; bank < 2 && w < cap; ++bank) {
    unsigned long long e = 0;
    for (int i = 0; i < 64; ++i) e = std::max(e, sp[8 + 64 * bank + i]);
    if (sp[2 + bank] != 0 && e > sp[2 + bank]) { out_pairs[2 * w] = sp[2 + bank]; out_pairs[2 * w + 1] = e; ++w; }
  }
  *n = w;
  return ETD_OK;
}

extern "C" int etd_decoder_stats_reset(etd_dec* d, void* stream) {
  if (!d) ETD_FAIL(ETD_EINVAL, "decoder_stats_reset: null handle");
  d->stat_steps = d->stat_row_steps = d->stat_kv_bytes = d->stat_attn_launches = d->stat_stamp_bytes = 0;
  if (d->stamp_dev) {
    HIP_TRY(hipStreamSynchronize((hipStream_t)stream));
    HIP_TRY(hipMemset(d->stamp_dev, 0, ETD_STAMP_HDR * 8));
  }
  return ETD_OK;
}

extern "C" int etd_decoder_stamp(etd_dec* d, int on, int skip_steps, void* stream) {
  if (!d || skip_steps < 0) ETD_FAIL(ETD_EINVAL, "decoder_stamp: bad arguments");
  if (on && !d->stamp_dev) {
    HIP_TRY(hipMalloc((void**)&d->stamp_dev, ETD_STAMP_WORDS * 8));
    HIP_TRY(hipMemset(d->stamp_dev, 0, ETD_STAMP_WORDS * 8));
  }
  HIP_TRY(hipStreamSynchronize((hipStream_t)stream));
  d->stamp_armed = on != 0; d->stamp_on = false; d->stamp_skip = on ? skip_steps : 0;
  return ETD_OK;
}

extern "C" int etd_debug_decoder_force_pair(etd_dec* d, int mode) {
  if (!d || mode < -1 || mode > 1) ETD_FAIL(ETD_EINVAL, "force_pair: bad arguments");
  d->force_pair = mode;
  return ETD_OK;
}

extern "C" int etd_debug_decoder_step_logits(etd_dec* d, int on, float* out_host, int n_active, void* stream) {
  hipStream_t st = (hipStream_t)stream;
  if (!d || n_active < 0 || n_active > d->S) ETD_FAIL(ETD_EINVAL, "step_logits: bad arguments");
  HIP_TRY(hipStreamSynchronize(st));
  if (out_host && n_active > 0) {
    if (d->last_step_fused && !(d->logits_dbg_on && d->logits_dbg)) ETD_FAIL(ETD_EINVAL, "step_logits: the fused step stores its logits only while the hook is on");
    const float* src = d->last_step_fused ? d->logits_dbg : d->logits;
    HIP_TRY(hipMemcpy(out_host, src, (size_t)n_active * d->V * 4, hipMemcpyDeviceToHost));
  }
  if (on && !d->logits_dbg) HIP_TRY(hipMalloc((void**)&d->logits_dbg, (size_t)d->S * d->V * 4));
  d->logits_dbg_on = on != 0;
  return ETD_OK;
}

extern "C" int etd_decoder_poll(etd_dec* d, const int32_t* slots, int n, int32_t* done_out, int32_t* n_out_out, void* stream) {
  hipStream_t st = (hipStream_t)stream;
  if (!d || !slots || n < 1 || !done_out || !n_out_out) ETD_FAIL(ETD_EINVAL, "decoder_poll: bad args");
  std::vector<int> dnv, nov;
  int *dn, *no;
  if (d->pin_rb) { dn = d->pin_rb; no = d->pin_rb + d->S; }
  else { dnv.resize(d->S); nov.resize(d->S); dn = dnv.data(); no = nov.data(); }
  HIP_TRY(hipMemcpyAsync(dn, d->done, (size_t)d->S * 4, hipMemcpyDeviceToHost, st));
  HIP_TRY(hipMemcpyAsync(no, d->n_out, (size_t)d->S * 4, hipMemcpyDeviceToHost, st));
  HIP_TRY(hipStreamSynchronize(st));
  for (int i = 0; i < n; ++i) { ETD_TRY(check_slot(d, slots[i])); done_out[i] = dn[slots[i]]; n_out_out[i] = no[slots[i]]; }
  memcpy(d->host_n_out.data(), no, (size_t)d->S * 4);
  d->host_n_out_valid = true;
  return ETD_OK;
}

extern "C" int etd_decoder_read_tokens(etd_dec* d, int slot, int32_t* out, int cap, int* n, void* stream) {
  hipStream_t st = (hipStream_t)stream;
  ETD_TRY(check_slot(d, slot));
  if (!out || !n) ETD_FAIL(ETD_EINVAL, "read_tokens: null");
  int cnt = 0;
  HIP_TRY(hipMemcpyAsync(&cnt, d->n_out + slot, 4, hipMemcpyDeviceToHost, st));
  HIP_TRY(hipStreamSynchronize(st));
  if (cnt > d->out_cap) cnt = d->out_cap;
  *n = cnt;
  if (cnt > cap) ETD_FAIL(ETD_ENOMEM, "read_tokens: need room for %d tokens", cnt);
  if (cnt > 0) {
    HIP_TRY(hipMemcpyAsync(out, d->out_tok + (size_t)slot * d->out_cap, (size_t)cnt * 4, hipMemcpyDeviceToHost, st));
    HIP_TRY(hipStreamSynchronize(st));
  }
  return ETD_OK;
}

extern "C" int etd_decoder_read_many(etd_dec* d, int n, const int32_t* slots, int32_t* out, int cap, int32_t* counts, void* stream) {
  hipStream_t st = (hipStream_t)stream;
  if (!d || n < 1 || !slots || !out || !counts || cap < 1) ETD_FAIL(ETD_EINVAL, "read_many: bad args");
  for (int i = 0; i < n; ++i) ETD_TRY(check_slot(d, slots[i]));
  if (!d->host_n_out_valid) {
    HIP_TRY(hipMemcpyAsync(d->host_n_out.data(), d->n_out, (size_t)d->S * 4, hipMemcpyDeviceToHost, st));
    HIP_TRY(hipStreamSynchronize(st));
  }
  int wmax = 0;
  for (int i = 0; i < n; ++i) { int c = d->host_n_out[slots[i]]; if (c > d->out_cap) c = d->out_cap; if (c > wmax) wmax = c; }
  std::vector<int> allv;
  int* all;
  if (d->pin_rb) all = d->pin_rb + 2 * (size_t)d->S; else { allv.resize((size_t)d->S * (wmax > 0 ? wmax : 1)); all = allv.data(); }
  if (wmax > 0) {
    HIP_TRY(hipMemcpy2DAsync(all, (size_t)wmax * 4, d->out_tok, (size_t)d->out_cap * 4, (size_t)wmax * 4, (size_t)d->S, hipMemcpyDeviceToHost, st));
    HIP_TRY(hipStreamSynchronize(st));
  }
  for (int i = 0; i < n; ++i) {
    int c = d->host_n_out[slots[i]]; if (c > d->out_cap) c = d->out_cap;
    if (c > cap) ETD_FAIL(ETD_ENOMEM, "read_many: slot %d holds %d tokens (cap %d)", slots[i], c, cap);
    counts[i] = c;
    memcpy(out + (size_t)i * cap, all + (size_t)slots[i] * wmax, (size_t)c * 4);
  }
  return ETD_OK;
}

extern "C" int etd_decoder_generate_bar(etd_dec* d, int slot, const int32_t* ids, const int32_t* cls, const int32_t* attrs4, int T,
                                        const int32_t* tgt_attrs4, int eos_id, int limit, int32_t* out, int* n_out, void* stream) {
  ETD_TRY(etd_decoder_begin_bar(d, slot, ids, cls, attrs4, T, tgt_attrs4, eos_id, limit, stream));
  int dn = 0, no = 0;
  const int32_t sl = slot;
  int chunk = 8;
  while (true) {
    ETD_TRY(etd_decoder_poll(d, &sl, 1, &dn, &no, stream));
    if (dn) break;
    ETD_TRY(etd_decoder_step(d, &sl, 1, chunk, stream));
    if (chunk < 32) chunk *= 2;
  }
  return etd_decoder_read_tokens(d, slot, out, limit, n_out, stream);
}

extern "C" int etd_decoder_prefill_logits(etd_dec* d, int slot, const int32_t* ids, const int32_t* cls, const int32_t* attrs4, int T,
                                          float* logits_host, void* stream) {
  hipStream_t st = (hipStream_t)stream;
  if (!logits_host) ETD_FAIL(ETD_EINVAL, "prefill_logits: null");
  if (T > d->Mmax) ETD_FAIL(ETD_EINVAL, "prefill_logits: T=%d exceeds %d", T, d->Mmax);
  const int32_t sl = slot, tt = T;
  Staged sg; float* hf = nullptr;
  ETD_TRY(stage_and_forward(d, 1, &sl, &tt, ids, cls, attrs4, nullptr, &sg, &hf, st));
  ETD_TRY(head_logits(d, hf, T, d->logits, st));
  HIP_TRY(hipMemcpyAsync(logits_host, d->logits, (size_t)T * d->V * 4, hipMemcpyDeviceToHost, st));
  HIP_TRY(hipStreamSynchronize(st));
  return ETD_OK;
}

extern "C" int etd_decoder_score(etd_dec* d, int n, const int32_t* T, const int32_t* ids, const int32_t* cls, const int32_t* attrs4,
                                 const int32_t* labels, double* seq_logprob, int32_t* seq_tokens, int32_t* seq_hits,
                                 float* row_lp, int32_t* row_argmax, float* logits_dev, void* stream) {
  hipStream_t st = (hipStream_t)stream;
  if (!d || n < 1 || !T || !ids || !cls || !attrs4 || !labels || !seq_logprob || !seq_tokens || !seq_hits) ETD_FAIL(ETD_EINVAL, "score: bad arguments");
  long long M = 0;
  for (int i = 0; i < n; ++i) {
    if (T[i] < 1 || T[i] > d->ctx) ETD_FAIL(ETD_EINVAL, "score: sequence %d has %d rows (max_ctx=%d)", i, T[i], d->ctx);
    M += T[i];
  }
  if (M > 0x7fffffffLL) ETD_FAIL(ETD_EINVAL, "score: %lld rows in one call", M);
  for (long long r = 0; r < M; ++r) {
    if (ids[r] < 0 || ids[r] >= d->V) ETD_FAIL(ETD_EINVAL, "score: token id %d out of range [0, %d) at row %lld", ids[r], d->V, r);
    if (cls[r] < 0 || cls[r] >= d->cfg.num_classes) ETD_FAIL(ETD_EINVAL, "score: class id %d out of range [0, %d) at row %lld", cls[r], d->cfg.num_classes, r);
    for (int k = 0; k < 4; ++k)
      if (attrs4[k * M + r] < 0 || attrs4[k * M + r] >= d->cfg.num_attribute_bins) ETD_FAIL(ETD_EINVAL, "score: attribute bin %d out of range [0, %d) at row %lld", attrs4[k * M + r], d->cfg.num_attribute_bins, r);
    if (labels[r] != ETD_IGNORE_LABEL && (labels[r] < 0 || labels[r] >= d->V)) ETD_FAIL(ETD_EINVAL, "score: label %d at row %lld is neither -100 nor in [0, %d)", labels[r], r, d->V);
  }
  const int S = d->S, Mcap = d->Mcap;
  if (!d->sc_x) {
    for (void* p : {(void*)d->sc_i, (void*)d->sc_f, (void*)d->sc_d}) if (p) (void)hipFree(p);
    d->sc_i = nullptr; d->sc_f = nullptr; d->sc_d = nullptr;
    d->score_hb = d->Mmax < 256 ? d->Mmax : 256;
    const int hb = d->score_hb;
    HIP_TRY(hipMalloc((void**)&d->sc_i, ((size_t)3 * Mcap + hb + 4 * (size_t)S) * sizeof(int)));
    HIP_TRY(hipMalloc((void**)&d->sc_f, (size_t)2 * Mcap * sizeof(float)));
    HIP_TRY(hipMalloc((void**)&d->sc_d, (size_t)S * sizeof(double)));
    HIP_TRY(hipMalloc((void**)&d->sc_x, (size_t)hb * d->H * sizeof(float)));
  }
  const int hb = d->score_hb;
  int* lab_dev = d->sc_i; int* idx_dev = lab_dev + Mcap; int* r0_dev = idx_dev + Mcap + hb; int* len_dev = r0_dev + S;
  int* am_dev = len_dev + S; int* tok_dev = am_dev + Mcap; int* hit_dev = tok_dev + S;
  float* lp_dev = d->sc_f; float* lse_dev = lp_dev + Mcap;
  const int rowcap = d->bf16w ? Mcap : std::min(Mcap, G3_MIN_ROWS - 1);
  const bool full = logits_dev != nullptr;
  std::vector<int32_t> slots(S), a4c, up;
  for (int i = 0; i < S; ++i) slots[i] = i;
  long long r0 = 0;
  for (int i0 = 0; i0 < n;) {
    int k = 0; long long Mc = 0;
    while (i0 + k < n && k < S && (k == 0 || Mc + T[i0 + k] <= rowcap)) Mc += T[i0 + k++];
    const int mc = (int)Mc;
    a4c.resize((size_t)4 * mc);
    for (int a = 0; a < 4; ++a) memcpy(a4c.data() + (size_t)a * mc, attrs4 + a * M + r0, (size_t)mc * 4);
    up.assign(labels + r0, labels + r0 + mc);
    for (int r = 0; r < mc; ++r) if (full || labels[r0 + r] != ETD_IGNORE_LABEL) up.push_back(r);
    const int nl = (int)up.size() - mc;
    const int nblk = (nl + hb - 1) / hb;
    up.resize((size_t)mc + (size_t)nblk * hb, 0);
    HIP_TRY(hipMemcpyAsync(lab_dev, up.data(), (size_t)mc * 4, hipMemcpyHostToDevice, st));
    if (nblk) HIP_TRY(hipMemcpyAsync(idx_dev, up.data() + mc, (size_t)nblk * hb * 4, hipMemcpyHostToDevice, st));
// ... 156 lines not shown
```

etude_amd/csrc/dec_kernels.h:

```cpp
#pragma once
#include "common.h"

#ifdef ETD_DEC_BF16
typedef bf16 d16; typedef bf16x8 d16x8; typedef bf16x4 d16x4; typedef bf16x2 d16x2;
#define ETD_MFMA16_DEC "v_mfma_f32_32x32x16_bf16"
#define ETD_DEC_IS_F16 0
#ifdef __HIPCC__
__device__ __forceinline__ d16x4 pack4d(float a, float b, float c, float d) { return pack4(a, b, c, d); }
#endif
#else
typedef f16 d16; typedef f16x8 d16x8; typedef f16x4 d16x4; typedef f16x2 d16x2;
#define ETD_MFMA16_DEC "v_mfma_f32_32x32x16_f16"
#define ETD_DEC_IS_F16 1
#ifdef __HIPCC__
__device__ __forceinline__ d16x4 pack4d(float a, float b, float c, float d) { return pack4h(a, b, c, d); }
#endif
#endif

#define DS_MAX_ROWS 512
#define DS_STEP_MAX_ROWS 2048

struct DecRows {
  const int* slot;
  const int* pos;
  const int* active;
  const int* seq;
};

struct DSampleCfg { float inv_temp; float top_p; unsigned long long seed; };

#define ETD_STAMP_HDR (8 + 2 * 64)
#define ETD_STAMP_LOGCAP 131072

enum { DEPI_BIAS = 0, DEPI_GELU = 1, DEPI_RESID = 2, DEPI_LOGITS = 3, DEPI_QKV = 4, DEPI_PARTIAL = 5, DEPI_RELU = 6  };

struct DGemmArgs {
  const float* X; int ldx;
  const void* W;
  const void* Wf;
  const float* bias;
  int M, N, K;
  int Npad;
  const float* ln_g; const float* ln_b; float ln_eps;
  float* Y; int ldy;
  d16* Yb;
  int k_splits;
  const d16* Xb;
  const float* add; const float* hin; float* hout;
  DecRows rows;
  const float* rope_cos; const float* rope_sin;
  int rot_half;
  float* Q;
  void* Kc; void* Vc;
  long long slot_stride;
  int max_ctx, n_heads;
  d16* Qb;
  const void* Wp; int w_log2;
  int x_log2;
};
int launch_dgemm(const DGemmArgs& a, int epi, bool w_bf16, hipStream_t st);
int launch_dstep_qkv_up(const DGemmArgs& q, const DGemmArgs& up, hipStream_t st);

struct DHeadArgs {
  const float* hfin; int M, H, V, Vpad;
  const float* lnf_g; const float* lnf_b; float eps;
  const d16* Whead;
  int* row_slot; int* row_pos; int* row_active; int* row_sp;
  int* cur_tok; int* len; int* done; int* n_out; int* out_tok; int out_cap; const int* eos; const int* limit;
  const int* tgt_attrs; const float* tgt_proj ; int tgt_cls; int n_bins;
  const float* word; const float* cls_emb; const float* attr_tab;
  const float* g1; const float* b1; const float* g2; const float* b2;
  float* h; d16* x1; d16* x2;
  const DSampleCfg* samp; const unsigned long long* rng_key;
  float* logits_dbg;
};
int launch_dstep_head(const DHeadArgs& a, hipStream_t st);

struct DAttnArgs {
  const float* Q;
  const void* Kc; const void* Vc; long long slot_stride; int max_ctx, n_heads;
  DecRows rows; int M;
  const int* row_sp;
  int identity;
  int pair;
  float* O;
  d16* Ob; int ldob;
  float scale;
  double bytes_hint;
  const d16* dense_w;
  float* dense_out;
  float* dbg;
  unsigned long long* stamp;
  int stamp_par;
};
int launch_dattn(const DAttnArgs& a, bool kv_bf16, hipStream_t st);
struct DRowFin {
  int* cnt; int target;
  const float* P; int nslab;
  const float* bias; const float* hin; float* hout;
  const float* g1; const float* b1; const float* g2; const float* b2; float eps;
  d16* x1; d16* x2;
};
int launch_dstep_attn_down(const DAttnArgs& a, const DGemmArgs& down, const DRowFin* fin, hipStream_t st);

struct PAttnArgs {
  const d16* Q; int ldq;
  const d16* Kc; const d16* Vc;
  long long slot_stride; int max_ctx, n_heads;
  d16* O; int ldo;
  const int* seq_row0; const int* seq_len; const int* row_slot;
  int n_seq, max_len;
  float scale_log2e;
  double flops_hint;
};
int launch_pattn(const PAttnArgs& a, hipStream_t st);

struct PQkvArgs {
  const d16* X; int ldx;
  const d16* Wf;
  const float* bias;
  int M, N;
  DecRows rows;
  const float* rope_cos; const float* rope_sin;
  d16* Qb;
  d16* Kc; d16* Vc; long long slot_stride; int max_ctx, n_heads;
};
int launch_pqkv(const PQkvArgs& a, hipStream_t st);

int launch_ln_rows(const float* h, int M, int H, const float* g1, const float* b1, const float* g2, const float* b2, float eps,
                   d16* x1, d16* x2, hipStream_t st);
int launch_resid_ln_rows(const float* P, int k_splits, const float* bias, const float* add, const float* hin, float* hout, int M, int H,
                         const float* g1, const float* b1, const float* g2, const float* b2, float eps, d16* x1, d16* x2, hipStream_t st);
int launch_gather_rows(const float* src, const int* idx, int n, int H, float* out, hipStream_t st);

#define DMLP_NCHUNK 73
#define DMLP_STREAM_ELEMS (DMLP_NCHUNK * 32 * 1024)
struct DMlpArgs {
  const d16* X2;
  const d16* AO; int ldao;
  const float* hin; float* hout;
  const d16* Wm;
  const float* b_up;
  const float* b_cat;
  const float* g1; const float* b1; const float* g2; const float* b2; float eps;
  d16* nx1; d16* nx2;
  int M;
};
int launch_dmlp_fused(const DMlpArgs& a, hipStream_t st);
void pack_dmlp_weights(const uint16_t* Wup_bf16 , const uint16_t* Wcat_bf16 , uint16_t* dst );

struct DEmbedArgs {
  const int* ids; const int* cls; const int* attrs;
  const int* cur_tok; const int* tgt_attrs;
  int tgt_cls;
  DecRows rows; int M, H, n_bins;
  const int* slots; const int* len; const int* done;
  int* row_slot_out; int* row_pos_out; int* row_active_out; int* row_sp_out;
  const float* word; const float* cls_emb; const float* attr_tab;
  float* h;
};
int launch_dembed(const DEmbedArgs& a, hipStream_t st);

struct DArgmaxArgs {
  const float* logits; int ldl; int V; int M;
  DecRows rows;
  int* cur_tok; int* len; int* done; int* n_out; int* out_tok; int out_cap; const int* eos; const int* limit;
  int set_len_from_pos;
  const DSampleCfg* samp; const unsigned long long* rng_key;
};
int launch_dargmax(const DArgmaxArgs& a, hipStream_t st);
```

etude_amd/csrc/dec_kernels.hip:

```cpp
#include "dec_kernels.h"
#include "prof.h"

#define DLD32 36
#define DLD16 72

#include "dec_epilogue.h"

#ifdef ETD_STEP_STAMP
__device__ long long* g_ss_buf;
__device__ unsigned long long g_ss_cap;
__device__ unsigned long long g_ss_cnt;
#define SS_DECL() long long ss_t[6] = {0, 0, 0, 0, 0, 0}
#define SS(i) do { __builtin_amdgcn_sched_barrier(0); ss_t[i] = (long long)__builtin_amdgcn_s_memrealtime(); __builtin_amdgcn_sched_barrier(0); } while (0)
#define SS_LANDED() asm volatile("s_waitcnt vmcnt(0)" ::: "memory")
#define SS_FLUSH(kid, role) do { if (threadIdx.x == 0 && g_ss_buf) { const unsigned long long i_ = atomicAdd(&g_ss_cnt, 1ull); if (i_ < g_ss_cap) { long long* o_ = g_ss_buf + i_ * 8;          \
      o_[0] = (long long)(kid) | ((long long)(role) << 8) | ((long long)blockIdx.x << 16); o_[1] = ss_t[0]; o_[2] = ss_t[1]; o_[3] = ss_t[2]; o_[4] = ss_t[3]; o_[5] = ss_t[4]; o_[6] = ss_t[5];   \
      o_[7] = (long long)__builtin_amdgcn_s_getreg((20 << 0) | (0 << 6) | (3 << 11)); } } } while (0)
extern "C" int etd_debug_step_stamps(long long* dev_buf, unsigned long long cap_records, unsigned long long* count_out) {
  HIP_TRY(hipDeviceSynchronize());
  if (count_out) HIP_TRY(hipMemcpyFromSymbol(count_out, HIP_SYMBOL(g_ss_cnt), 8));
  const unsigned long long zero = 0;
  HIP_TRY(hipMemcpyToSymbol(HIP_SYMBOL(g_ss_cnt), &zero, 8));
  HIP_TRY(hipMemcpyToSymbol(HIP_SYMBOL(g_ss_buf), &dev_buf, 8));
  HIP_TRY(hipMemcpyToSymbol(HIP_SYMBOL(g_ss_cap), &cap_records, 8));
// ... 705 lines not shown
    for (int j = 0; j < 4; ++j) {
      const int rl = wave * 4 + j;
      const float rstd = rsqrtf(q4[j] / (float)H + a.eps);
#pragma unroll
      for (int half = 0; half < 2; ++half) {
        const int k = lane * 4 + half * 256;
        const f32x4 x = half ? hv1[j] : hv0[j];
        const f32x4 g = lg_[half], b = lb_[half];
        *reinterpret_cast<d16x4*>(Xs + rl * DH_LDX + k) =
            pack4d((x[0] - mean[j]) * rstd * g[0] + b[0], (x[1] - mean[j]) * rstd * g[1] + b[1], (x[2] - mean[j]) * rstd * g[2] + b[2], (x[3] - mean[j]) * rstd * g[3] + b[3]);
      }
    }
  }
  __builtin_amdgcn_sched_barrier(0);
  int statev;
  {
    const int j = lane & 3, f = (lane >> 2) < 5 ? (lane >> 2) : 5;
    const int sl = __shfl(mapv, j, 64);
    const int* sp = f == 0 ? a.cur_tok : f == 1 ? a.len : f == 2 ? a.done : f == 3 ? a.n_out : f == 4 ? a.eos : a.limit;
    statev = sp[sl];
  }
  __builtin_amdgcn_sched_barrier(0);
  HSTAMP(7);
  __syncthreads();
  HSTAMP(1);
  if (wave * 32 < a.Vpad) {
    const d16* xrow = Xs + r * DH_LDX;
    f32x16 tot;
#pragma unroll
    for (int sl = 0; sl < 8; ++sl) {
      f32x16 acc;
#pragma unroll
      for (int i = 0; i < 16; ++i) acc[i] = 0.f;
#pragma unroll
      for (int s4 = 0; s4 < 4; ++s4) {
        const int k = sl * 64 + s4 * 16 + h * 8;
        acc = mfma32(wf[sl * 4 + s4], *reinterpret_cast<const d16x8*>(xrow + k), acc);
      }
      if (sl == 0) tot = acc;
      else {
#pragma unroll
        for (int i = 0; i < 16; ++i) tot[i] += acc[i];
      }
    }
#pragma unroll
    for (int i = 0; i < 16; ++i) {
      const int f = wave * 32 + acc_row(i, h);
      if (f < a.V) Ls[r * DH_LDL + f] = tot[i];
    }
  }
  __syncthreads();
  HSTAMP(2);
  if (a.logits_dbg) {
    for (int i = tid; i < 32 * a.V; i += 512) {
      const int rr = i / a.V, f = i - rr * a.V;
      if (m0 + rr < a.M) a.logits_dbg[(long long)(m0 + rr) * a.V + f] = Ls[rr * DH_LDL + f];
    }
  }
  int gbi[4] = {0, 0, 0, 0};
  if (inv_temp > 0.f) {
#pragma unroll
    for (int j = 0; j < 4; ++j) {
      if (m0 + wave * 4 + j >= a.M) continue;
      gbi[j] = wave_sample(Ls + (wave * 4 + j) * DH_LDL, a.V, lane, inv_temp, a.samp->top_p, a.samp->seed, a.rng_key[__builtin_amdgcn_readlane(mapv, j)],
                           (unsigned)__builtin_amdgcn_readlane(statev, 12 + j), sps[wave], sss[wave], sis[wave]);
    }
  } else {
    wave_argmax4(Ls + wave * 4 * DH_LDL, DH_LDL, a.V, lane, gbi);
  }
  int n_tok[4], r_slot[4];
  {
    const int jr = lane & 3, m = m0 + wave * 4 + jr;
    const int slot = __shfl(mapv, jr, 64), act = __shfl(mapv, 4 + jr, 64), pos = __shfl(mapv, 8 + jr, 64);
    const int tok = __shfl(statev, jr, 64), len0 = __shfl(statev, 4 + jr, 64), done0 = __shfl(statev, 8 + jr, 64);
    const int n = __shfl(statev, 12 + jr, 64), eos = __shfl(statev, 16 + jr, 64), lim = __shfl(statev, 20 + jr, 64);
    const int bi = jr == 0 ? gbi[0] : jr == 1 ? gbi[1] : jr == 2 ? gbi[2] : gbi[3];
    int ntok = tok, ln = len0, dn = done0;
    const bool mine = (lane < 4) & (m < a.M);
    if (act && !done0) {
      ntok = bi; ln = pos + 1;
      const int fin = ((bi == eos) | (n + 1 >= lim)) ? 1 : 0;
      if (mine) {
        if (n < a.out_cap) a.out_tok[(long long)slot * a.out_cap + n] = bi;
        a.n_out[slot] = n + 1;
        a.cur_tok[slot] = bi;
        a.len[slot] = ln;
        if (fin) a.done[slot] = 1;
      }
      dn = fin;
    }
    if (mine) { a.row_pos[m] = ln; a.row_active[m] = dn ? 0 : 1; if (a.row_sp) a.row_sp[2 * m + 1] = ln; }
#pragma unroll
    for (int j = 0; j < 4; ++j) {
      n_tok[j] = __builtin_amdgcn_readlane(ntok, j); r_slot[j] = __builtin_amdgcn_readlane(mapv, j);
    }
  }
  HSTAMP(3);
  f32x4 r_c[2], pg1[2], pb1[2], pg2[2], pb2[2], wv[4][2], pv[4][2];
#pragma unroll
  for (int j = 0; j < 4; ++j)
#pragma unroll
    for (int hh = 0; hh < 2; ++hh) {
      wv[j][hh] = *reinterpret_cast<const f32x4*>(a.word + (long long)n_tok[j] * H + k8 + 4 * hh);
      pv[j][hh] = *reinterpret_cast<const f32x4*>(a.tgt_proj + (long long)r_slot[j] * H + k8 + 4 * hh);
    }
#pragma unroll
  for (int hh = 0; hh < 2; ++hh) {
    r_c[hh] = *reinterpret_cast<const f32x4*>(a.cls_emb + (long long)a.tgt_cls * H + k8 + 4 * hh);
    pg1[hh] = *reinterpret_cast<const f32x4*>(a.g1 + k8 + 4 * hh); pb1[hh] = *reinterpret_cast<const f32x4*>(a.b1 + k8 + 4 * hh);
    pg2[hh] = *reinterpret_cast<const f32x4*>(a.g2 + k8 + 4 * hh); pb2[hh] = *reinterpret_cast<const f32x4*>(a.b2 + k8 + 4 * hh);
  }
  {
    float v[4][8], s4[4], q4[4], mean[4];
#pragma unroll
    for (int j = 0; j < 4; ++j) {
      float s1 = 0.f;
#pragma unroll
      for (int e = 0; e < 8; ++e) {
        const int hh = e >> 2, c = e & 3;
        v[j][e] = (wv[j][hh][c] + r_c[hh][c]) + pv[j][hh][c];
        s1 += v[j][e];
      }
      s4[j] = s1;
    }
    wave_sum_n<4>(s4);
#pragma unroll
    for (int j = 0; j < 4; ++j) {
      mean[j] = s4[j] / (float)H;
      float q = 0.f;
#pragma unroll
      for (int e = 0; e < 8; ++e) { const float d0 = v[j][e] - mean[j]; q += d0 * d0; }
      q4[j] = q;
    }
    wave_sum_n<4>(q4);
#pragma unroll
    for (int j = 0; j < 4; ++j) {
      const int m = m0 + wave * 4 + j;
      if (m >= a.M) continue;
      const long long ro = (long long)m * H;
      { const f32x4 oa = {v[j][0], v[j][1], v[j][2], v[j][3]}, ob = {v[j][4], v[j][5], v[j][6], v[j][7]};
        *reinterpret_cast<f32x4*>(a.h + ro + k8) = oa; *reinterpret_cast<f32x4*>(a.h + ro + k8 + 4) = ob; }
      const float rstd = rsqrtf(q4[j] / (float)H + a.eps);
      d16x8 o1, o2;
#pragma unroll
      for (int e = 0; e < 8; ++e) {
        o1[e] = (d16)((v[j][e] - mean[j]) * rstd * pg1[e >> 2][e & 3] + pb1[e >> 2][e & 3]);
        o2[e] = (d16)((v[j][e] - mean[j]) * rstd * pg2[e >> 2][e & 3] + pb2[e >> 2][e & 3]);
      }
      *reinterpret_cast<d16x8*>(a.x1 + ro + k8) = o1;
      *reinterpret_cast<d16x8*>(a.x2 + ro + k8) = o2;
    }
  }
  HSTAMP(4);
  SS_FLUSH(0, 0);
}

#ifdef ETD_HEAD_STAMP
extern "C" int etd_debug_head_stamps(long long* out) {
  HIP_TRY(hipDeviceSynchronize());
  HIP_TRY(hipMemcpyFromSymbol(out, HIP_SYMBOL(g_head_stamp), sizeof(long long) * 8 * 16));
  return ETD_OK;
}
#endif
int launch_dstep_head(const DHeadArgs& a, hipStream_t st) {
  if (a.samp && !a.rng_key) ETD_FAIL(ETD_EINVAL, "dstep_head: sampling needs stream keys");
  if (a.M < 1 || a.H != 512 || a.V < 1 || a.V > a.Vpad || a.Vpad % 32 || a.Vpad > 256 || !a.hfin || !a.Whead || !a.tgt_proj || !a.h || !a.x1 || !a.x2)
    ETD_FAIL(ETD_EINVAL, "dstep_head: bad arguments (needs hidden 512, vocabulary <= 256)");
  ProfScope ps("k_dstep_head", st, 2.0 * a.M * a.V * a.H, (double)a.Vpad * a.H * 2);
  hipLaunchKernelGGL(k_dstep_head, dim3((a.M + 31) / 32), dim3(512), 0, st, a.hfin, a.M, a.row_slot, a.row_active, a.row_pos, a);
  HIP_TRY(hipGetLastError());
  return ETD_OK;
}

__device__ __forceinline__ float fma_scalar(float a, float b, float c) {
  asm volatile("v_fma_f32 %0, %1, %2, %0" : "+v"(c) : "v"(a), "v"(b));
  return c;
}
template <bool WBF16, int EPI>
__global__ __launch_bounds__(256) void k_dgemv(DGemmArgs a) {
  const int tid = threadIdx.x, lane = tid & 63, wave = tid >> 6;
  const int nb = (blockIdx.x * 4 + wave) * 4;
  const bool ln = a.ln_g != nullptr;
  float mean = 0.f, rstd = 1.f;
  if (ln) {
    float s = 0.f;
    for (int k = lane * 4; k < a.K; k += 256) { const f32x4 v = *reinterpret_cast<const f32x4*>(a.X + k); s += v[0] + v[1] + v[2] + v[3]; }
    s = wave_sum(s);
    mean = s / (float)a.K;
    float q = 0.f;
    for (int k = lane * 4; k < a.K; k += 256) {
      const f32x4 v = *reinterpret_cast<const f32x4*>(a.X + k);
      const float d0 = v[0] - mean, d1 = v[1] - mean, d2 = v[2] - mean, d3 = v[3] - mean;
      q += d0 * d0 + d1 * d1 + d2 * d2 + d3 * d3;
    }
    q = wave_sum(q);
    rstd = rsqrtf(q / (float)a.K + a.ln_eps);
  }
  float acc[4] = {0.f, 0.f, 0.f, 0.f};
  for (int k = lane * 8; k < a.K; k += 512) {
    f32x4 x0 = *reinterpret_cast<const f32x4*>(a.X + k), x1 = *reinterpret_cast<const f32x4*>(a.X + k + 4);
    if (ln) {
      const f32x4 g0 = *reinterpret_cast<const f32x4*>(a.ln_g + k), g1 = *reinterpret_cast<const f32x4*>(a.ln_g + k + 4);
      const f32x4 b0 = *reinterpret_cast<const f32x4*>(a.ln_b + k), b1 = *reinterpret_cast<const f32x4*>(a.ln_b + k + 4);
#pragma unroll
      for (int j = 0; j < 4; ++j) { x0[j] = (x0[j] - mean) * rstd * g0[j] + b0[j]; x1[j] = (x1[j] - mean) * rstd * g1[j] + b1[j]; }
    }
#pragma unroll
    for (int f = 0; f < 4; ++f) {
      float w[8];
      if constexpr (WBF16) {
        const d16x8 wv = *reinterpret_cast<const d16x8*>(reinterpret_cast<const d16*>(a.W) + (long long)(nb + f) * a.K + k);
#pragma unroll
        for (int j = 0; j < 8; ++j) w[j] = bf2f(wv[j]);
#pragma unroll
        for (int j = 0; j < 4; ++j) { acc[f] = fmaf(w[j], bf2f((d16)x0[j]), acc[f]); acc[f] = fmaf(w[4 + j], bf2f((d16)x1[j]), acc[f]); }
      } else {
        const float* wp = reinterpret_cast<const float*>(a.W) + (long long)(nb + f) * a.K + k;
        const f32x4 w0 = *reinterpret_cast<const f32x4*>(wp), w1 = *reinterpret_cast<const f32x4*>(wp + 4);
#pragma unroll
        for (int j = 0; j < 4; ++j) { acc[f] = fma_scalar(w0[j], x0[j], acc[f]); acc[f] = fma_scalar(w1[j], x1[j], acc[f]); }
      }
    }
  }
#pragma unroll
  for (int f = 0; f < 4; ++f) acc[f] = wave_sum(acc[f]);
  if (lane != 0) return;
#pragma unroll
  for (int f = 0; f < 4; ++f) {
    const int n = nb + f;
    if (n >= a.N) break;
    float v = acc[f];
    if (EPI != DEPI_LOGITS) v += a.bias[n];
    if (EPI == DEPI_GELU) v = gelu_erf(v);
    if (EPI == DEPI_RESID) a.hout[n] = (v + a.add[n]) + a.hin[n];
    else a.Y[n] = v;
  }
}

template <typename KVT>
__global__ void k_rope_scatter(DGemmArgs a, const float* __restrict__ raw) {
  const int m = blockIdx.x;
  const int pos = a.rows.pos[m], slot = a.rows.slot[m];
  const bool act = a.rows.active[m] && pos < a.max_ctx;
  const int H3 = a.n_heads * 192;
  for (int n = threadIdx.x; n < H3; n += blockDim.x) {
    const int head = n / 192, j = n - head * 192, part = j >> 6, d = j & 63;
    float v = raw[(long long)m * H3 + n];
    if (part < 2 && d < 2 * a.rot_half) {
      const int dd = d < a.rot_half ? d : d - a.rot_half;
      const float c = a.rope_cos[(long long)pos * a.rot_half + dd], s = a.rope_sin[(long long)pos * a.rot_half + dd];
      const float other = raw[(long long)m * H3 + (d < a.rot_half ? n + a.rot_half : n - a.rot_half)];
      v = d < a.rot_half ? v * c - other * s : v * c + other * s;
    }
    if (part == 0) a.Q[(long long)m * (a.n_heads * 64) + head * 64 + d] = v;
    else if (act) {
      const long long off = (long long)slot * a.slot_stride + ((long long)head * a.max_ctx + pos) * 64 + d;
      KVT* base = reinterpret_cast<KVT*>(part == 1 ? a.Kc : a.Vc);
      base[off] = (KVT)v;
    }
  }
}

template <bool WBF16>
static void dgemm_dispatch(const DGemmArgs& a, int epi, int path, hipStream_t st) {
  const int wtiles = (a.Npad / 32) * (a.k_splits > 1 ? a.k_splits : 1);
  const dim3 g0((a.M + 31) / 32, a.Npad / 128), g1((unsigned)(((wtiles + 7) / 8) * 8 * ((a.M + 31) / 32))), g2(a.Npad / 16);
#define ETD_DG(E)                                                                                   \
  if (path == 0) hipLaunchKernelGGL((k_dgemm<WBF16, E>), g0, dim3(256), 0, st, a);                  \
  else if (path == 1) hipLaunchKernelGGL((k_dgemm_s<WBF16, E>), g1, dim3(64 * DS_WAVES), 0, st, a.M, a.Npad, a.k_splits, a.K, a.W, a.Xb, a.ldx, a);  \
  else hipLaunchKernelGGL((k_dgemv<WBF16, E>), g2, dim3(256), 0, st, a);
  switch (epi) {
    case DEPI_BIAS: ETD_DG(DEPI_BIAS) break;
    case DEPI_GELU: ETD_DG(DEPI_GELU) break;
    case DEPI_RESID: ETD_DG(DEPI_RESID) break;
    case DEPI_LOGITS: ETD_DG(DEPI_LOGITS) break;
    case DEPI_PARTIAL: hipLaunchKernelGGL((k_dgemm_s<WBF16, DEPI_PARTIAL>), g1, dim3(64 * DS_WAVES), 0, st, a.M, a.Npad, a.k_splits, a.K, a.W, a.Xb, a.ldx, a); break;
    default:
      if (path == 0) hipLaunchKernelGGL((k_dgemm<WBF16, DEPI_QKV>), g0, dim3(256), 0, st, a);
      else hipLaunchKernelGGL((k_dgemm_s<WBF16, DEPI_QKV>), g1, dim3(64 * DS_WAVES), 0, st, a.M, a.Npad, a.k_splits, a.K, a.W, a.Xb, a.ldx, a);
      break;
  }
#undef ETD_DG
}

bool g3_enabled();
bool gemm3_s_takes(const DGemmArgs& a, int epi);
int launch_gemm3_s(const DGemmArgs& a, int epi, hipStream_t st);
int launch_dgemm(const DGemmArgs& a, int epi, bool w_bf16, hipStream_t st) {
  const bool g3s_on = g3_enabled();
  if (!w_bf16 && g3s_on && gemm3_s_takes(a, epi)) return launch_gemm3_s(a, epi, st);
  if (a.M <= 0 || a.Npad % 128 || a.K % 256 || a.N > a.Npad) ETD_FAIL(ETD_EINVAL, "dgemm: bad shape M=%d N=%d Npad=%d K=%d", a.M, a.N, a.Npad, a.K);
  if (epi == DEPI_QKV && (a.rot_half != 8 || a.N % 192)) ETD_FAIL(ETD_EINVAL, "dgemm: QKV epilogue needs head_dim 64 and rotary_ndims 16");
  if (epi == DEPI_RESID && (a.N % 4)) ETD_FAIL(ETD_EINVAL, "dgemm: resid needs N %% 4 == 0");
  const int path = a.M == 1 ? 2 : (a.M <= DS_MAX_ROWS || (epi == DEPI_PARTIAL && a.M <= DS_STEP_MAX_ROWS) ? 1 : 0);
  if (epi == DEPI_PARTIAL && (path != 1 || a.k_splits < 1 || (a.K / a.k_splits) % (64 * DS_WAVES) || !a.Y)) ETD_FAIL(ETD_EINVAL, "dgemm: bad split-K request");
  if (epi != DEPI_PARTIAL && a.k_splits > 1) ETD_FAIL(ETD_EINVAL, "dgemm: k_splits needs DEPI_PARTIAL");
  ProfScope ps(path == 2 ? "k_dgemv" : (path == 1 ? "k_dgemm_s" : "k_dgemm"), st, 2.0 * a.M * a.N * a.K, (double)a.Npad * a.K * (w_bf16 ? 2 : 4));
  if (path == 2 && epi == DEPI_QKV) {
    if (!a.Y) ETD_FAIL(ETD_EINVAL, "dgemm: M == 1 QKV path needs a scratch row in Y");
    if (w_bf16) { dgemm_dispatch<true>(a, DEPI_BIAS, 2, st); hipLaunchKernelGGL(k_rope_scatter<d16>, dim3(1), dim3(256), 0, st, a, a.Y); }
    else { dgemm_dispatch<false>(a, DEPI_BIAS, 2, st); hipLaunchKernelGGL(k_rope_scatter<float>, dim3(1), dim3(256), 0, st, a, a.Y); }
  } else if (w_bf16) dgemm_dispatch<true>(a, epi, path, st);
  else dgemm_dispatch<false>(a, epi, path, st);
  HIP_TRY(hipGetLastError());
  return ETD_OK;
}

template <typename KVT> struct Raw8;
template <> struct Raw8<float> {
  f32x4 a, b;
  __device__ __forceinline__ void load(const float* p) { a = *reinterpret_cast<const f32x4*>(p); b = *reinterpret_cast<const f32x4*>(p + 4); }
  __device__ __forceinline__ float get(int j) const { return j < 4 ? a[j] : b[j - 4]; }
};
template <> struct Raw8<d16> {
  d16x8 v;
  __device__ __forceinline__ void load(const d16* p) { v = __builtin_nontemporal_load(reinterpret_cast<const d16x8*>(p)); }
  __device__ __forceinline__ float get(int j) const { return bf2f(v[j]); }
};

#ifndef ETD_FIN_ZB
#define ETD_FIN_ZB 12
#endif
typedef __amdgpu_buffer_rsrc_t drsrc_t;
__device__ __forceinline__ drsrc_t d_rsrc(const void* p, long long bytes) {
  return __builtin_amdgcn_make_buffer_rsrc(const_cast<void*>(p), 0, (int)(bytes > 0x7fffffffLL ? 0x7fffffffLL : bytes), 0x00020000);
}
#define D_SC1 16
__device__ __forceinline__ void row_finish(const DRowFin& f, const int row_in, const int M_in, const int lane) {
  const int row = __builtin_amdgcn_readfirstlane(row_in), M = __builtin_amdgcn_readfirstlane(M_in);
  const drsrc_t ps = d_rsrc(f.P, (long long)f.nslab * M * 512 * 4);
  const long long ro = (long long)row * 512;
  const int k = lane * 8;
  float acc[8];
#pragma unroll
  for (int j = 0; j < 8; ++j) acc[j] = 0.f;
  const f32x4 ba = *reinterpret_cast<const f32x4*>(f.bias + k), bb = *reinterpret_cast<const f32x4*>(f.bias + k + 4);
  const f32x4 ha = *reinterpret_cast<const f32x4*>(f.hin + ro + k), hb = *reinterpret_cast<const f32x4*>(f.hin + ro + k + 4);
  f32x4 pg1[2], pb1[2], pg2[2], pb2[2];
  if (f.x1) {
#pragma unroll
    for (int hh = 0; hh < 2; ++hh) {
      pg1[hh] = *reinterpret_cast<const f32x4*>(f.g1 + k + 4 * hh); pb1[hh] = *reinterpret_cast<const f32x4*>(f.b1 + k + 4 * hh);
      pg2[hh] = *reinterpret_cast<const f32x4*>(f.g2 + k + 4 * hh); pb2[hh] = *reinterpret_cast<const f32x4*>(f.b2 + k + 4 * hh);
    }
  }
  constexpr int ZB = ETD_FIN_ZB;
#pragma unroll
  for (int z0 = 0; z0 < 12; z0 += ZB) {
    f32x4 pa[ZB], pb[ZB];
#pragma unroll
    for (int z = 0; z < ZB; ++z) {
      const int so = (int)((((long long)(z0 + z) * M + row) * 512) * 4);
      pa[z] = __builtin_bit_cast(f32x4, __builtin_amdgcn_raw_buffer_load_b128(ps, k * 4, so, D_SC1));
      pb[z] = __builtin_bit_cast(f32x4, __builtin_amdgcn_raw_buffer_load_b128(ps, k * 4 + 16, so, D_SC1));
    }
#pragma unroll
    for (int z = 0; z < ZB; ++z)
#pragma unroll
      for (int j = 0; j < 4; ++j) { acc[j] += pa[z][j]; acc[4 + j] += pb[z][j]; }
  }
  float v[8];
#pragma unroll
  for (int j = 0; j < 4; ++j) { v[j] = ((acc[j] + ba[j]) + 0.f) + ha[j]; v[4 + j] = ((acc[4 + j] + bb[j]) + 0.f) + hb[j]; }
  {
    const f32x4 oa = {v[0], v[1], v[2], v[3]}, ob = {v[4], v[5], v[6], v[7]};
    *reinterpret_cast<f32x4*>(f.hout + ro + k) = oa;
    *reinterpret_cast<f32x4*>(f.hout + ro + k + 4) = ob;
  }
  if (!f.x1) return;
  float s = 0.f;
#pragma unroll
  for (int j = 0; j < 8; ++j) s += v[j];
  s = wave_sum(s);
  const float mean = s / 512.f;
  float q = 0.f;
#pragma unroll
  for (int j = 0; j < 8; ++j) { const float d0 = v[j] - mean; q += d0 * d0; }
  q = wave_sum(q);
  const float rstd = rsqrtf(q / 512.f + f.eps);
  d16x8 o1, o2;
#pragma unroll
  for (int j = 0; j < 8; ++j) {
    const float n = (v[j] - mean) * rstd;
    o1[j] = (d16)(n * pg1[j >> 2][j & 3] + pb1[j >> 2][j & 3]);
    o2[j] = (d16)(n * pg2[j >> 2][j & 3] + pb2[j >> 2][j & 3]);
  }
  *reinterpret_cast<d16x8*>(f.x1 + ro + k) = o1;
  *reinterpret_cast<d16x8*>(f.x2 + ro + k) = o2;
}
#define D_ARRIVE(p) __hip_atomic_fetch_add((p), 1, __ATOMIC_RELAXED, __HIP_MEMORY_SCOPE_AGENT)
#define D_CNT_RESET(p) __hip_atomic_store((p), 0, __ATOMIC_RELAXED, __HIP_MEMORY_SCOPE_AGENT)

#define ABL_DENSE_LOAD(p) (*reinterpret_cast<const d16x8*>(p))
#define ABL_GEMMW_LOAD(p) (*reinterpret_cast<const d16x8*>(p))
#define ETD_XCH(v, O) __shfl_xor(v, O, 64)
#define ETD_TRANS_SETTLE(a_, b_) ((void)0)
#define ETD_TRANS_SETTLE_LOOP(a_, b_) ((void)0)
#define EXPF(x) (FAST ? __builtin_amdgcn_exp2f(x) : expf(x))
__device__ __forceinline__ float merge_sum(float a, float b, float c, float d) {
  float t, u, r;
  asm volatile("v_mul_f32 %0, %1, %2" : "=v"(t) : "v"(a), "v"(b));
  asm volatile("v_mul_f32 %0, %1, %2" : "=v"(u) : "v"(c), "v"(d));
  asm volatile("v_add_f32 %0, %1, %2" : "=v"(r) : "v"(t), "v"(u));
  return r;
}
template <typename KVT, bool DENSE, int NW, bool FIN = false, bool PAIR = false>
__device__ __forceinline__ void dattn_core(const int m, const int head, float (&red)[NW][8][10], float* osh, float* outsh,
                                           const int* p_row_sp, const float* p_Q, const void* p_Kc, const void* p_Vc, long long p_slot_stride,
                                           int p_max_ctx, int p_n_heads, float p_scale, int p_identity, const DAttnArgs& a, const DRowFin* fin = nullptr,
                                           const float* osh_other = nullptr, float* outsh_other = nullptr, bool dup = false) {
  const int tid = PAIR ? (int)(threadIdx.x & (64 * NW - 1)) : (int)threadIdx.x, lane = tid & 63, wave = tid >> 6, j = lane >> 3, c = lane & 7;
  SS_DECL(); SS(0);
  constexpr int G2 = 8 * NW;
  constexpr int KI = 16 * NW;
  int slot, pos;
  typedef int i32x2 __attribute__((ext_vector_type(2)));
  Raw8<KVT> kA, kB, wA, wB, nkA, nkB, nwA, nwB;
  if (p_identity) {
    const KVT* kb0 = reinterpret_cast<const KVT*>(p_Kc) + (long long)m * p_slot_stride + (long long)head * p_max_ctx * 64;
    const KVT* vb0 = reinterpret_cast<const KVT*>(p_Vc) + (long long)m * p_slot_stride + (long long)head * p_max_ctx * 64;
    const int ka = wave * 8 + j, kbb = ka + G2;
    kA.load(kb0 + (long long)ka * 64 + c * 8); kB.load(kb0 + (long long)kbb * 64 + c * 8);
    wA.load(vb0 + (long long)ka * 64 + c * 8); wB.load(vb0 + (long long)kbb * 64 + c * 8);
    slot = m; pos = __builtin_nontemporal_load(p_row_sp + 2 * m + 1);
  } else if (p_row_sp) { const i32x2 sp = __builtin_nontemporal_load(reinterpret_cast<const i32x2*>(p_row_sp + 2 * m)); slot = sp[0]; pos = sp[1]; }
  else { slot = a.rows.slot[m]; pos = a.rows.pos[m]; }
  const int ctx = (pos < p_max_ctx ? pos : p_max_ctx - 1) + 1;
  const int hidden = p_n_heads * 64;
  constexpr bool FAST = sizeof(KVT) == 2;
  const float qs = FAST ? p_scale * 1.4426950408889634f : p_scale;
  float q[8];
  {
    const float* qp = p_Q + (long long)m * hidden + head * 64 + c * 8;
    const f32x4 x = *reinterpret_cast<const f32x4*>(qp), y = *reinterpret_cast<const f32x4*>(qp + 4);
    q[0] = x[0] * qs; q[1] = x[1] * qs; q[2] = x[2] * qs; q[3] = x[3] * qs;
    q[4] = y[0] * qs; q[5] = y[1] * qs; q[6] = y[2] * qs; q[7] = y[3] * qs;
  }
  const KVT* kb = reinterpret_cast<const KVT*>(p_Kc) + (long long)slot * p_slot_stride + (long long)head * p_max_ctx * 64;
  const KVT* vb = reinterpret_cast<const KVT*>(p_Vc) + (long long)slot * p_slot_stride + (long long)head * p_max_ctx * 64;
  float mr = -INFINITY, lr = 0.f, o[8];
#pragma unroll
  for (int e = 0; e < 8; ++e) o[e] = 0.f;
  auto issue = [&](int k0, Raw8<KVT>& a_, Raw8<KVT>& b_, Raw8<KVT>& c_, Raw8<KVT>& d_) {
    int ka = k0 + j, kbb = k0 + G2 + j;
    ka = ka < ctx ? ka : ctx - 1; kbb = kbb < ctx ? kbb : ctx - 1;
    a_.load(kb + (long long)ka * 64 + c * 8);
    b_.load(kb + (long long)kbb * 64 + c * 8);
    c_.load(vb + (long long)ka * 64 + c * 8);
    d_.load(vb + (long long)kbb * 64 + c * 8);
  };
  int k0 = wave * 8;
  if (!p_identity && k0 < ctx) issue(k0, kA, kB, wA, wB);
#ifdef ETD_STEP_STAMP
  SS_LANDED(); SS(1);
#endif
  for (; k0 < ctx; k0 += KI) {
    const bool more = k0 + KI < ctx;
    if (more) issue(k0 + KI, nkA, nkB, nwA, nwB);
    const bool vA = k0 + j < ctx, vB = k0 + G2 + j < ctx;
    float sA = 0.f, sB = 0.f;
#pragma unroll
    for (int e = 0; e < 8; ++e) { sA = fmaf(q[e], kA.get(e), sA); sB = fmaf(q[e], kB.get(e), sB); }
    sA += ETD_XCH(sA, 1); sB += ETD_XCH(sB, 1);
    sA += ETD_XCH(sA, 2); sB += ETD_XCH(sB, 2);
    sA += ETD_XCH(sA, 4); sB += ETD_XCH(sB, 4);
    if (vA) {
      const float mn = fmaxf(mr, sA);
      float al = EXPF(mr - mn), p = EXPF(sA - mn);
      ETD_TRANS_SETTLE_LOOP(al, p);
      lr = lr * al + p;
#pragma unroll
      for (int e = 0; e < 8; ++e) o[e] = o[e] * al + p * wA.get(e);
      mr = mn;
    }
    if (vB) {
      const float mn = fmaxf(mr, sB);
      float al = EXPF(mr - mn), p = EXPF(sB - mn);
      ETD_TRANS_SETTLE_LOOP(al, p);
      lr = lr * al + p;
#pragma unroll
      for (int e = 0; e < 8; ++e) o[e] = o[e] * al + p * wB.get(e);
      mr = mn;
    }
    if (more) { kA = nkA; kB = nkB; wA = nwA; wB = nwB; }
  }

  SS(2);
  constexpr int FR = PAIR ? 64 / (2 * NW) : 64 / NW, FP = FR > 8 ? 8 : FR, NPASS = FR / FP;
  const int dwave = PAIR ? (int)(threadIdx.x >> 6) : wave;
  constexpr int DROWS = PAIR ? 512 / (2 * NW) : 512 / NW;
  d16x8 dwv[DENSE ? FP : 1];
  const d16* dwb = nullptr;
  if constexpr (DENSE) {
    dwb = a.dense_w + (long long)head * (512 * 64) + (long long)(dwave * DROWS + (lane >> 3)) * 64 + (lane & 7) * 8;
#pragma unroll
    for (int it = 0; it < FP; ++it) dwv[it] = ABL_DENSE_LOAD(dwb + it * 8 * 64);
  }
#define ETD_MERGE_STAGE(off)                                                                                                \
  {                                                                                                                         \
    const float m2 = ETD_XCH(mr, off), l2 = ETD_XCH(lr, off);                                                               \
    const float mn = fmaxf(mr, m2);                                                                                         \
    float f1 = (mr == -INFINITY) ? 0.f : EXPF(mr - mn), f2 = (m2 == -INFINITY) ? 0.f : EXPF(m2 - mn);                       \
    ETD_TRANS_SETTLE(f1, f2);                                                                                               \
    lr = merge_sum(lr, f1, l2, f2);                                                                                         \
    _Pragma("unroll") for (int e = 0; e < 8; ++e) { const float o2 = ETD_XCH(o[e], off); o[e] = merge_sum(o[e], f1, o2, f2); } \
    mr = mn;                                                                                                                \
  }
#define ETD_MERGE_STAGES() ETD_MERGE_STAGE(8) ETD_MERGE_STAGE(16) ETD_MERGE_STAGE(32)
  float* dp = a.dbg ? a.dbg + ((long long)(head * a.M + m) * 256 + tid) * 8 : nullptr;
  if (dp) { dp[0] = lr; dp[1] = mr; dp[2] = o[0]; }
  ETD_MERGE_STAGES()
  if (dp) { dp[5] = lr; dp[7] = o[0]; }
  if (j == 0) {
    red[wave][c][0] = mr; red[wave][c][1] = lr;
#pragma unroll
    for (int e = 0; e < 8; ++e) red[wave][c][2 + e] = o[e];
  }
  __syncthreads();
  if (wave == 0) {
    if constexpr (NW <= 4) {
      if (j == 0) {
        float M2 = -INFINITY;
        for (int w = 0; w < NW; ++w) M2 = fmaxf(M2, red[w][c][0]);
        float L = 0.f, acc[8] = {0, 0, 0, 0, 0, 0, 0, 0};
        for (int w = 0; w < NW; ++w) {
          const float mw = red[w][c][0];
          const float f = (mw == -INFINITY) ? 0.f : EXPF(mw - M2);
          L += red[w][c][1] * f;
#pragma unroll
          for (int e = 0; e < 8; ++e) acc[e] += red[w][c][2 + e] * f;
        }
        lr = L;
#pragma unroll
        for (int e = 0; e < 8; ++e) o[e] = acc[e];
      }
    } else {
      mr = red[j][c][0]; lr = red[j][c][1];
#pragma unroll
      for (int e = 0; e < 8; ++e) o[e] = red[j][c][2 + e];
#pragma unroll
      for (int w = j + 8; w < NW; w += 8) {
        const float m2 = red[w][c][0], l2 = red[w][c][1];
        const float mn = fmaxf(mr, m2);
        const float f1 = (mr == -INFINITY) ? 0.f : EXPF(mr - mn), f2 = (m2 == -INFINITY) ? 0.f : EXPF(m2 - mn);
        lr = merge_sum(lr, f1, l2, f2);
#pragma unroll
        for (int e = 0; e < 8; ++e) o[e] = merge_sum(o[e], f1, red[w][c][2 + e], f2);
        mr = mn;
      }
      ETD_MERGE_STAGES()
    }
    if (j == 0) {
      const float inv = 1.f / lr;
      const f32x4 x = {o[0] * inv, o[1] * inv, o[2] * inv, o[3] * inv}, y = {o[4] * inv, o[5] * inv, o[6] * inv, o[7] * inv};
      if constexpr (DENSE) {
#pragma unroll
        for (int e = 0; e < 4; ++e) { osh[c * 8 + e] = (float)(d16)x[e]; osh[c * 8 + 4 + e] = (float)(d16)y[e]; }
      } else {
        float* op = a.O + (long long)m * hidden + head * 64 + c * 8;
        *reinterpret_cast<f32x4*>(op) = x;
        *reinterpret_cast<f32x4*>(op + 4) = y;
        if (a.Ob) {
          const d16x8 ob = {(d16)x[0], (d16)x[1], (d16)x[2], (d16)x[3], (d16)y[0], (d16)y[1], (d16)y[2], (d16)y[3]};
          *reinterpret_cast<d16x8*>(a.Ob + (long long)m * (a.ldob > 0 ? a.ldob : hidden) + head * 64 + c * 8) = ob;
        }
      }
    }
  }
#undef ETD_MERGE_STAGES
#undef ETD_MERGE_STAGE
  if constexpr (DENSE) {
    __syncthreads();
    SS(3);
    const int g8 = lane >> 3, sub = lane & 7;
    float ov[8];
#pragma unroll
    for (int e = 0; e < 8; ++e) ov[e] = osh[sub * 8 + e];
    if constexpr (PAIR) {
      float ov2[8];
#pragma unroll
      for (int e = 0; e < 8; ++e) ov2[e] = osh_other[sub * 8 + e];
#pragma unroll
      for (int it = 0; it < FP; ++it) {
        float sacc = 0.f, sacc2 = 0.f;
#pragma unroll
        for (int e = 0; e < 8; ++e) { sacc = fmaf(bf2f(dwv[it][e]), ov[e], sacc); sacc2 = fmaf(bf2f(dwv[it][e]), ov2[e], sacc2); }
        sacc += lane_xor<1>(sacc); sacc += lane_xor<2>(sacc); sacc += lane_xor<4>(sacc);
        sacc2 += lane_xor<1>(sacc2); sacc2 += lane_xor<2>(sacc2); sacc2 += lane_xor<4>(sacc2);
        if (sub == 0) { outsh[dwave * DROWS + it * 8 + g8] = sacc; outsh_other[dwave * DROWS + it * 8 + g8] = sacc2; }
      }
    } else
#pragma unroll
    for (int pass = 0; pass < NPASS; ++pass) {
      if (pass == 1) {
#pragma unroll
        for (int it = 0; it < FP; ++it) dwv[it] = ABL_DENSE_LOAD(dwb + (FP + it) * 8 * 64);
      }
#pragma unroll
      for (int it = 0; it < FP; ++it) {
        float sacc = 0.f;
#pragma unroll
        for (int e = 0; e < 8; ++e) sacc = fmaf(bf2f(dwv[it][e]), ov[e], sacc);
        sacc += lane_xor<1>(sacc); sacc += lane_xor<2>(sacc); sacc += lane_xor<4>(sacc);
        if (sub == 0) outsh[wave * (512 / NW) + (pass * FP + it) * 8 + g8] = sacc;
      }
      __builtin_amdgcn_sched_barrier(0);
    }
    __syncthreads();
    SS(4);
    if constexpr (FIN) {
      if (tid < 128) {
        const drsrc_t os = d_rsrc(a.dense_out, (long long)p_n_heads * a.M * 512 * 4);
        const f32x4 o4 = {outsh[4 * tid], outsh[4 * tid + 1], outsh[4 * tid + 2], outsh[4 * tid + 3]};
        __builtin_amdgcn_raw_buffer_store_b128(__builtin_bit_cast(u32x4, o4), os, tid * 16, (int)((((long long)head * a.M + m) * 512) * 4), D_SC1);
      }
      asm volatile("s_waitcnt vmcnt(0)" ::: "memory");
      __syncthreads();
      SS(5); SS_FLUSH(2, 0);
      if (wave != 0) return;
#ifdef ETD_STEP_STAMP
      ss_t[0] = ss_t[5]; ss_t[3] = ss_t[4] = ss_t[5] = 0;
#endif
      int old = 0;
      if (lane == 0) old = D_ARRIVE(fin->cnt + m);
      old = __builtin_amdgcn_readfirstlane(old);
      SS(1);
#ifdef ETD_STEP_STAMP
      if (old != fin->target - 1) { SS_FLUSH(4, 0); return; }
#else
      if (old != fin->target - 1) return;
#endif
      row_finish(*fin, m, a.M, lane);
      if (lane == 0) D_CNT_RESET(fin->cnt + m);
#ifdef ETD_STEP_STAMP
      SS_LANDED(); SS(2); SS_FLUSH(4, 1);
#endif
    } else {
      if (tid < 256 && !dup) {
        typedef float f32x2 __attribute__((ext_vector_type(2)));
        const f32x2 o2 = {outsh[2 * tid], outsh[2 * tid + 1]};
        *reinterpret_cast<f32x2*>(a.dense_out + ((long long)head * a.M + m) * 512 + 2 * tid) = o2;
      }
      SS(5); SS_FLUSH(2, 0);
    }
  }
}
__device__ __forceinline__ void attn_stamp_begin(unsigned long long* stp, int par, int flat_block) {
  if (stp && flat_block == 0 && threadIdx.x < 64) {
    const int bank = par & 1, prev = bank ^ 1, lane = threadIdx.x;
    const unsigned long long now = (unsigned long long)__builtin_amdgcn_s_memrealtime();
    unsigned long long e = atomicExch(stp + 8 + 64 * prev + lane, 0ull);
    for (int o = 32; o > 0; o >>= 1) { const unsigned long long x = __shfl_xor(e, o, 64); e = x > e ? x : e; }
    if (lane == 0) {
      const unsigned long long s0 = atomicExch(stp + 2 + prev, 0ull);
      if (s0 != 0 && e > s0) {
        atomicAdd(stp, e - s0);
        const unsigned long long n = atomicAdd(stp + 1, 1ull);
        if (n < ETD_STAMP_LOGCAP) { stp[ETD_STAMP_HDR + 2 * n] = s0; stp[ETD_STAMP_HDR + 2 * n + 1] = e; }
      }
      atomicExch(stp + 2 + bank, now);
    }
  }
}
__device__ __forceinline__ void attn_stamp_end(unsigned long long* stp, int par, int flat_block) {
  if (stp) {
    __syncthreads();
    if (threadIdx.x == 0) atomicMax(stp + 8 + 64 * (par & 1) + (flat_block & 63), (unsigned long long)__builtin_amdgcn_s_memrealtime());
  }
}

template <typename KVT>
__global__ __launch_bounds__(256) void k_dattn(const int* p_row_sp, const float* p_Q, const void* p_Kc, const void* p_Vc, long long p_slot_stride,
                                               int p_max_ctx, int p_n_heads, float p_scale, int p_identity, DAttnArgs a) {
  __shared__ float red[4][8][10];
  const int flat = blockIdx.y * gridDim.x + blockIdx.x;
  attn_stamp_begin(a.stamp, a.stamp_par, flat);
  dattn_core<KVT, false, 4>(blockIdx.x, blockIdx.y, red, nullptr, nullptr, p_row_sp, p_Q, p_Kc, p_Vc, p_slot_stride, p_max_ctx, p_n_heads, p_scale, p_identity, a);
  attn_stamp_end(a.stamp, a.stamp_par, flat);
}

#undef EXPF
template <int NW> struct AdOcc { static constexpr int lo = 7, hi = 8; };
#ifndef ETD_AD_OCC
#define ETD_AD_OCC 5
#endif
template <> struct AdOcc<4> { static constexpr int lo = ETD_AD_OCC, hi = 8; };
#ifndef ETD_FIN_OCC
#define ETD_FIN_OCC 4
#endif
template <int NW, bool FIN, bool PAIR = false>
__device__ __forceinline__ void dstep_attn_down_body(const int* p_row_sp, const float* p_Q, const void* p_Kc, const void* p_Vc, long long p_slot_stride,
                                                     int p_max_ctx, int p_n_heads, float p_scale, int p_identity, int p_gemm_wgs, int p_M,
                                                     const DAttnArgs& a, const DGemmArgs& g, const DRowFin& fin) {
  constexpr int UNITS = NW / 2;
  __shared__ float red[NW][8][10];
  __shared__ float osh[PAIR ? 128 : 64];
  __shared__ __attribute__((aligned(16))) float sh[UNITS * 16 * 64 > 512 ? UNITS * 16 * 64 : 512];
  if constexpr (PAIR) {
    static_assert(!PAIR || (NW == 8 && !FIN), "paired rows: 8 waves, no in-launch row finish");
    if ((int)blockIdx.x >= p_gemm_wgs) {
      const int lid = blockIdx.x - p_gemm_wgs, P = (p_M + 1) >> 1, pr = lid % P, half = threadIdx.x >> 8;
      int m = 2 * pr + half;
      const bool dup = m >= p_M;
      m = dup ? 2 * pr : m;
      float (&redh)[4][8][10] = *reinterpret_cast<float (*)[4][8][10]>(&red[4 * half][0][0]);
      dattn_core<d16, true, 4, false, true>(m, lid / P, redh, osh + 64 * half, sh + 512 * half, p_row_sp, p_Q, p_Kc, p_Vc, p_slot_stride, p_max_ctx, p_n_heads, p_scale, p_identity, a,
                                             nullptr, osh + 64 * (half ^ 1), sh + 512 * (half ^ 1), dup);
      return;
    }
  }
  if ((int)blockIdx.x >= p_gemm_wgs) {
    const int lid = blockIdx.x - p_gemm_wgs;
    dattn_core<d16, true, NW, FIN>(lid % p_M, lid / p_M, red, osh, sh, p_row_sp, p_Q, p_Kc, p_Vc, p_slot_stride, p_max_ctx, p_n_heads, p_scale, p_identity, a, &fin);
    return;
  }
  const int tid = threadIdx.x, unit = tid >> 7, tl = tid & 127, lane = tl & 63, wave = tl >> 6, r = lane & 31, h = lane >> 5;
  const int RT = (p_M + 31) / 32, FT = g.Npad / 32, KS = g.k_splits;
  const int bid = blockIdx.x, slot = (bid >> 3) * UNITS + unit, wt = (slot / RT) * 8 + (bid & 7);
  const bool valid = wt < FT * KS;
  const int wtc = valid ? wt : 0;
  const int bz = wtc / FT, m0 = (slot % RT) * 32, n0 = (wtc - bz * FT) * 32;
  int gm = m0 + r; gm = gm < p_M ? gm : p_M - 1;
  const int Kz = 512;
  const int kb = bz * Kz + wave * 256;
  const d16* wrow = reinterpret_cast<const d16*>(g.W) + (long long)(n0 + r) * g.K + kb + h * 8;
  const d16* xrow = g.Xb + (long long)gm * g.ldx + kb + h * 8;
  SS_DECL(); SS(0);
  f32x16 acc;
#pragma unroll
  for (int i = 0; i < 16; ++i) acc[i] = 0.f;
#pragma unroll
  for (int ps = 0; ps < 4; ++ps) {
    d16x8 wf[4], xf[4];
#pragma unroll
    for (int s4 = 0; s4 < 4; ++s4) { wf[s4] = ABL_GEMMW_LOAD(wrow + (ps * 4 + s4) * 16); xf[s4] = *reinterpret_cast<const d16x8*>(xrow + (ps * 4 + s4) * 16); }
    __builtin_amdgcn_sched_barrier(0);
#pragma unroll
    for (int s4 = 0; s4 < 4; ++s4) acc = mfma32(wf[s4], xf[s4], acc);
  }
  SS(1);
  float* redg = sh + unit * (16 * 64);
  if (wave == 1) {
#pragma unroll
    for (int i = 0; i < 16; ++i) redg[i * 64 + lane] = acc[i];
  }
  __syncthreads();
  if (wave != 0 || !valid) return;
#pragma unroll
  for (int i = 0; i < 16; ++i) acc[i] += redg[i * 64 + lane];
  const int m = m0 + r;
  if constexpr (FIN) {
    if (m < p_M) {
      const drsrc_t ys = d_rsrc(g.Y, (long long)g.k_splits * p_M * 512 * 4);
      const int vo = ((bz * p_M + m) * 512 + n0 + 4 * h) * 4;
#pragma unroll
      for (int q = 0; q < 4; ++q) {
        const f32x4 o4 = {acc[4 * q], acc[4 * q + 1], acc[4 * q + 2], acc[4 * q + 3]};
        __builtin_amdgcn_raw_buffer_store_b128(__builtin_bit_cast(u32x4, o4), ys, vo + 32 * q, 0, D_SC1);
      }
    }
    asm volatile("s_waitcnt vmcnt(0)" ::: "memory");
    SS(2); SS_FLUSH(2, 1);
    int old = -1;
    if (h == 0 && m < p_M) old = D_ARRIVE(fin.cnt + m);
    unsigned long long last = __ballot(old == fin.target - 1);
    while (last) {
      const int rl = __builtin_ctzll(last);
      last &= last - 1;
      row_finish(fin, m0 + rl, p_M, lane);
      if (lane == 0) D_CNT_RESET(fin.cnt + m0 + rl);
    }
  } else {
    if (m >= p_M) return;
    DGemmArgs b = g;
    b.Y = g.Y + (long long)bz * p_M * g.ldy;
    dgemm_epilogue<true, DEPI_PARTIAL>(b, acc, m, n0, h);
    SS(2); SS_FLUSH(2, 1);
  }
}

template <int NW, bool FIN, bool PAIR = false>
__global__ __launch_bounds__(64 * NW) __attribute__((amdgpu_waves_per_eu(FIN ? ETD_FIN_OCC : (PAIR ? ETD_AD_OCC : AdOcc<NW>::lo), AdOcc<NW>::hi))) void k_dstep_attn_down(const int* p_row_sp, const float* p_Q, const void* p_Kc, const void* p_Vc, long long p_slot_stride,
                                                         int p_max_ctx, int p_n_heads, float p_scale, int p_identity, int p_gemm_wgs, int p_M,
                                                         DAttnArgs a, DGemmArgs g, DRowFin fin) {
  attn_stamp_begin(a.stamp, a.stamp_par, (int)blockIdx.x);
  dstep_attn_down_body<NW, FIN, PAIR>(p_row_sp, p_Q, p_Kc, p_Vc, p_slot_stride, p_max_ctx, p_n_heads, p_scale, p_identity, p_gemm_wgs, p_M, a, g, fin);
  attn_stamp_end(a.stamp, a.stamp_par, (int)blockIdx.x);
}

static int ad_waves(int M) {
  (void)M;
#ifdef ETD_EXPERIMENTS
  static const int env = getenv("ETD_AD_WAVES") ? atoi(getenv("ETD_AD_WAVES")) : 0;
  return (env == 8 || env == 16) ? env : 4;
#else
  return 4;
#endif
}
int launch_dstep_attn_down(const DAttnArgs& a, const DGemmArgs& g, const DRowFin* fin, hipStream_t st) {
#ifndef ETD_EXPERIMENTS
  if (fin) ETD_FAIL(ETD_EINVAL, "dstep_attn_down: the in-launch row finish is built with -DETD_EXPERIMENTS only");
#endif
  if (fin && (!fin->cnt || fin->target != a.n_heads + 16 * g.k_splits || fin->nslab != 12 || g.k_splits + a.n_heads != 12 || fin->P != g.Y ||
              a.dense_out != g.Y + (size_t)g.k_splits * a.M * 512 || !fin->bias || !fin->hin || !fin->hout || fin->hin == fin->hout || (fin->x1 && (!fin->x2 || !fin->g1 || !fin->b1 || !fin->g2 || !fin->b2))))
    ETD_FAIL(ETD_EINVAL, "dstep_attn_down: bad row-finish arguments");
  if (a.M < 1 || a.M > DS_STEP_MAX_ROWS || a.n_heads < 1 || !a.row_sp || !a.dense_w || !a.dense_out || a.max_ctx < 256 ||
      g.M != a.M || !g.Xb || !g.W || !g.Y || g.ldy != 512 || g.N != 512 || g.Npad != 512 || g.k_splits < 1 || g.k_splits * 512 > g.K || (g.K % 8) || a.n_heads * 64 != 512)
    ETD_FAIL(ETD_EINVAL, "dstep_attn_down: bad arguments");
  static const int pair_env = ETD_XENV("ETD_AD_PAIR") ? atoi(ETD_XENV("ETD_AD_PAIR")) : -1;
  const bool pair = (pair_env < 0 ? a.pair != 0 : pair_env > 0) && !fin && ad_waves(a.M) == 4;
  const int nw = pair ? 8 : ad_waves(a.M), units = nw / 2;
  const int RT = (a.M + 31) / 32, FT = g.Npad / 32;
  const int slots = ((FT * g.k_splits + 7) / 8) * RT;
  const int gemm_wgs = ((slots + units - 1) / units) * 8;
  ProfScope ps("k_dstep_attn_down", st, 2.0 * a.M * 512 * (512.0 * g.k_splits + 512.0), a.bytes_hint + 512.0 * (512.0 * g.k_splits + 512.0) * 2);
  const DRowFin f0 = fin ? *fin : DRowFin{};
#define ETD_AD_LAUNCH(NW_, FIN_) hipLaunchKernelGGL((k_dstep_attn_down<NW_, FIN_>), dim3(gemm_wgs + a.M * a.n_heads), dim3(64 * NW_), 0, st, a.row_sp, a.Q, a.Kc, a.Vc, a.slot_stride, a.max_ctx, a.n_heads, a.scale, \
                                              a.identity ? 1 : 0, gemm_wgs, a.M, a, g, f0)
  if (pair) {
    hipLaunchKernelGGL((k_dstep_attn_down<8, false, true>), dim3(gemm_wgs + ((a.M + 1) / 2) * a.n_heads), dim3(512), 0, st, a.row_sp, a.Q, a.Kc, a.Vc, a.slot_stride, a.max_ctx, a.n_heads, a.scale,
                       a.identity ? 1 : 0, gemm_wgs, a.M, a, g, f0);
  } else
#ifdef ETD_EXPERIMENTS
  if (fin) { if (nw == 16) ETD_AD_LAUNCH(16, true); else if (nw == 8) ETD_AD_LAUNCH(8, true); else ETD_AD_LAUNCH(4, true); }
  else if (nw == 16) ETD_AD_LAUNCH(16, false); else if (nw == 8) ETD_AD_LAUNCH(8, false); else ETD_AD_LAUNCH(4, false);
#else
  ETD_AD_LAUNCH(4, false);
#endif
#undef ETD_AD_LAUNCH
  HIP_TRY(hipGetLastError());
  return ETD_OK;
}

int launch_dattn(const DAttnArgs& a, bool kv_bf16, hipStream_t st) {
  if (a.M <= 0) ETD_FAIL(ETD_EINVAL, "dattn: bad M");
  ProfScope ps(a.M > 512 ? "k_dattn_prefill" : "k_dattn", st, 0, a.bytes_hint);
  dim3 g(a.M, a.n_heads);
  const int ident = a.identity && a.row_sp && a.max_ctx >= 64 ? 1 : 0;
  if (kv_bf16) hipLaunchKernelGGL(k_dattn<d16>, g, dim3(256), 0, st, a.row_sp, a.Q, a.Kc, a.Vc, a.slot_stride, a.max_ctx, a.n_heads, a.scale, ident, a);
  else hipLaunchKernelGGL(k_dattn<float>, g, dim3(256), 0, st, a.row_sp, a.Q, a.Kc, a.Vc, a.slot_stride, a.max_ctx, a.n_heads, a.scale, ident, a);
  HIP_TRY(hipGetLastError());
  return ETD_OK;
}

__global__ __launch_bounds__(256) void k_ln_rows(const float* __restrict__ hsrc, int M, int H, const float* __restrict__ g1, const float* __restrict__ b1,
                                                 const float* __restrict__ g2, const float* __restrict__ b2, float eps, d16* __restrict__ x1, d16* __restrict__ x2) {
  const int lane = threadIdx.x & 63, row = blockIdx.x * 4 + (threadIdx.x >> 6);
  if (row >= M) return;
  const float* xp = hsrc + (long long)row * H;
  float v[4][8];
  float s = 0.f;
#pragma unroll
  for (int it = 0; it < 4; ++it) {
    const int k = lane * 8 + it * 512;
    if (k < H) {
      const f32x4 a = *reinterpret_cast<const f32x4*>(xp + k), b = *reinterpret_cast<const f32x4*>(xp + k + 4);
      v[it][0] = a[0]; v[it][1] = a[1]; v[it][2] = a[2]; v[it][3] = a[3]; v[it][4] = b[0]; v[it][5] = b[1]; v[it][6] = b[2]; v[it][7] = b[3];
#pragma unroll
      for (int j = 0; j < 8; ++j) s += v[it][j];
    }
  }
  s = wave_sum(s);
  const float mean = s / (float)H;
  float q = 0.f;
#pragma unroll
  for (int it = 0; it < 4; ++it)
    if (lane * 8 + it * 512 < H) {
#pragma unroll
      for (int j = 0; j < 8; ++j) { const float d0 = v[it][j] - mean; q += d0 * d0; }
    }
  q = wave_sum(q);
  const float rstd = rsqrtf(q / (float)H + eps);
#pragma unroll
  for (int it = 0; it < 4; ++it) {
    const int k = lane * 8 + it * 512;
    if (k < H) {
      const f32x4 ga = *reinterpret_cast<const f32x4*>(g1 + k), gb = *reinterpret_cast<const f32x4*>(g1 + k + 4);
      const f32x4 ba = *reinterpret_cast<const f32x4*>(b1 + k), bb = *reinterpret_cast<const f32x4*>(b1 + k + 4);
      d16x8 o1;
#pragma unroll
      for (int j = 0; j < 4; ++j) { o1[j] = (d16)((v[it][j] - mean) * rstd * ga[j] + ba[j]); o1[4 + j] = (d16)((v[it][4 + j] - mean) * rstd * gb[j] + bb[j]); }
      *reinterpret_cast<d16x8*>(x1 + (long long)row * H + k) = o1;
      if (x2) {
        const f32x4 ha = *reinterpret_cast<const f32x4*>(g2 + k), hb = *reinterpret_cast<const f32x4*>(g2 + k + 4);
        const f32x4 ca = *reinterpret_cast<const f32x4*>(b2 + k), cb = *reinterpret_cast<const f32x4*>(b2 + k + 4);
        d16x8 o2;
#pragma unroll
        for (int j = 0; j < 4; ++j) { o2[j] = (d16)((v[it][j] - mean) * rstd * ha[j] + ca[j]); o2[4 + j] = (d16)((v[it][4 + j] - mean) * rstd * hb[j] + cb[j]); }
        *reinterpret_cast<d16x8*>(x2 + (long long)row * H + k) = o2;
      }
    }
  }
}
int launch_ln_rows(const float* hsrc, int M, int H, const float* g1, const float* b1, const float* g2, const float* b2, float eps,
                   d16* x1, d16* x2, hipStream_t st) {
  if (M <= 0 || H % 8 || H > 2048) ETD_FAIL(ETD_EINVAL, "ln_rows: bad shape");
  ProfScope ps("k_ln_rows", st, 0, (double)M * H * (4 + (x2 ? 4 : 2)));
  hipLaunchKernelGGL(k_ln_rows, dim3((M + 3) / 4), dim3(256), 0, st, hsrc, M, H, g1, b1, g2, b2, eps, x1, x2);
  HIP_TRY(hipGetLastError());
  return ETD_OK;
}

#ifndef ETD_RL_ROWS
#define ETD_RL_ROWS 4
#endif
template <int KS>
__global__ __launch_bounds__(64 * ETD_RL_ROWS) void k_resid_ln_rows(const float* __restrict__ P, int ks_rt, const float* __restrict__ bias, const float* __restrict__ add,
                                                       const float* __restrict__ hin, float* __restrict__ hout, int M, int H,
                                                       const float* __restrict__ g1, const float* __restrict__ b1, const float* __restrict__ g2,
                                                       const float* __restrict__ b2, float eps, d16* __restrict__ x1, d16* __restrict__ x2) {
  const int lane = threadIdx.x & 63, row = blockIdx.x * ETD_RL_ROWS + (threadIdx.x >> 6);
  if (row >= M) return;
  SS_DECL(); SS(0);
  const long long ro = (long long)row * H;
  float v[4][8];
  float s = 0.f;
  const int k0 = lane * 8;
  f32x4 pg1[2], pb1[2], pg2[2], pb2[2];
  if (x1 && k0 < H) {
#pragma unroll
    for (int hh = 0; hh < 2; ++hh) {
      pg1[hh] = *reinterpret_cast<const f32x4*>(g1 + k0 + 4 * hh); pb1[hh] = *reinterpret_cast<const f32x4*>(b1 + k0 + 4 * hh);
      pg2[hh] = *reinterpret_cast<const f32x4*>(g2 + k0 + 4 * hh); pb2[hh] = *reinterpret_cast<const f32x4*>(b2 + k0 + 4 * hh);
    }
  }
#pragma unroll
  for (int it = 0; it < 4; ++it) {
    const int k = lane * 8 + it * 512;
    if (k < H) {
      float acc[8];
#pragma unroll
      for (int j = 0; j < 8; ++j) acc[j] = 0.f;
      if constexpr (KS > 0) {
        f32x4 pa[KS], pb[KS];
#pragma unroll
        for (int z = 0; z < KS; ++z) {
          const float* pp = P + (long long)z * M * H + ro + k;
          pa[z] = *reinterpret_cast<const f32x4*>(pp); pb[z] = *reinterpret_cast<const f32x4*>(pp + 4);
        }
#pragma unroll
        for (int z = 0; z < KS; ++z)
#pragma unroll
          for (int j = 0; j < 4; ++j) { acc[j] += pa[z][j]; acc[4 + j] += pb[z][j]; }
      } else {
        for (int z = 0; z < ks_rt; ++z) {
          const float* pp = P + (long long)z * M * H + ro + k;
          const f32x4 a = *reinterpret_cast<const f32x4*>(pp), b = *reinterpret_cast<const f32x4*>(pp + 4);
#pragma unroll
          for (int j = 0; j < 4; ++j) { acc[j] += a[j]; acc[4 + j] += b[j]; }
        }
      }
      const f32x4 ba = *reinterpret_cast<const f32x4*>(bias + k), bb = *reinterpret_cast<const f32x4*>(bias + k + 4);
      f32x4 da = {0.f, 0.f, 0.f, 0.f}, db = {0.f, 0.f, 0.f, 0.f};
      if (add) { da = *reinterpret_cast<const f32x4*>(add + ro + k); db = *reinterpret_cast<const f32x4*>(add + ro + k + 4); }
      const f32x4 ha = *reinterpret_cast<const f32x4*>(hin + ro + k), hb = *reinterpret_cast<const f32x4*>(hin + ro + k + 4);
#pragma unroll
      for (int j = 0; j < 4; ++j) { v[it][j] = ((acc[j] + ba[j]) + da[j]) + ha[j]; v[it][4 + j] = ((acc[4 + j] + bb[j]) + db[j]) + hb[j]; }
      const f32x4 oa = {v[it][0], v[it][1], v[it][2], v[it][3]}, ob = {v[it][4], v[it][5], v[it][6], v[it][7]};
      *reinterpret_cast<f32x4*>(hout + ro + k) = oa;
      *reinterpret_cast<f32x4*>(hout + ro + k + 4) = ob;
#pragma unroll
      for (int j = 0; j < 8; ++j) s += v[it][j];
    }
  }
  if (!x1) return;
  SS(1);
  s = wave_sum(s);
  const float mean = s / (float)H;
  float q = 0.f;
#pragma unroll
  for (int it = 0; it < 4; ++it)
    if (lane * 8 + it * 512 < H) {
#pragma unroll
// ... 108 lines not shown
```

etude_amd/csrc/dec_prefill.hip:

```cpp
#include "dec_kernels.h"
#include "prof.h"

#include <cstdlib>

#define PA_LDK 72
#define PA_LDV 96

typedef __attribute__((ext_vector_type(4))) short pa_s16x4;
typedef __attribute__((address_space(3))) pa_s16x4* pa_lds_s16x4;

__global__ __launch_bounds__(256) void k_pattn(PAttnArgs a) {
  __shared__ __attribute__((aligned(16))) unsigned char smem[64 * PA_LDK * 2 + 64 * PA_LDV * 2];
  d16* Ks = reinterpret_cast<d16*>(smem);
  d16* Vs = Ks + 64 * PA_LDK;
  const int tid = threadIdx.x, lane = tid & 63, wave = __builtin_amdgcn_readfirstlane(tid >> 6), r = lane & 31, h = lane >> 5;
  const int nh = a.n_heads;
  const int seq = blockIdx.y / nh, head = blockIdx.y - seq * nh;
  const int S = a.seq_len[seq];
  const long long r0 = a.seq_row0[seq];
  const int off = (128 - (S & 127)) & 127;
  if ((int)blockIdx.x * 128 - off >= S) return;
  const int slot = a.row_slot[r0];
  const int q0 = (int)blockIdx.x * 128 + wave * 32 - off;
  int qi = q0 + r; const bool qvalid = qi >= 0 && qi < S; qi = qi < 0 ? 0 : (qi < S ? qi : S - 1);

  const d16* qp = a.Q + (r0 + qi) * a.ldq + head * 64;
  d16x8 qf[4];
#pragma unroll
  for (int s = 0; s < 4; ++s) qf[s] = *reinterpret_cast<const d16x8*>(qp + s * 16 + h * 8);

  const long long cbase = (long long)slot * a.slot_stride + (long long)head * a.max_ctx * 64;
  const d16* kbase = a.Kc + cbase;
  const d16* vbase = a.Vc + cbase;

  f32x16 o[2];
#pragma unroll
  for (int t = 0; t < 2; ++t)
#pragma unroll
    for (int i = 0; i < 16; ++i) o[t][i] = 0.f;
  float mrun = -INFINITY, lrun = 0.f;

  int ntile = (S + 63) >> 6;
  { const int lim = ((int)blockIdx.x * 128 + 127 - off) / 64 + 1; ntile = ntile < lim ? ntile : lim; }
  u32x4 kreg[2], vreg[2];
  auto tile_gload = [&](int kv0_) {
#pragma unroll
    for (int i = 0; i < 2; ++i) {
      const int c = tid + i * 256, row = c >> 3, ch = c & 7;
      int key = kv0_ + row; key = key < S ? key : S - 1;
      kreg[i] = *reinterpret_cast<const u32x4*>(kbase + (long long)key * 64 + ch * 8);
      vreg[i] = *reinterpret_cast<const u32x4*>(vbase + (long long)key * 64 + ch * 8);
    }
  };
  const int tq = (lane >> 2) & 3, tp = lane & 3, tg = (lane >> 4) & 1;
  const d16* vtr = Vs + (4 * h + tq) * PA_LDV + 16 * tg + 4 * tp;
  tile_gload(0);
  for (int jt = 0; jt < ntile; ++jt) {
    const int kv0 = jt * 64;
#pragma unroll
    for (int i = 0; i < 2; ++i) {
      const int c = tid + i * 256, row = c >> 3, ch = c & 7;
      *reinterpret_cast<u32x4*>(Ks + row * PA_LDK + ch * 8) = kreg[i];
      *reinterpret_cast<u32x4*>(Vs + row * PA_LDV + ch * 8) = vreg[i];
    }
    __syncthreads();
    if (jt + 1 < ntile) tile_gload(kv0 + 64);
    if (kv0 <= q0 + 31) {
      f32x16 sT[2];
#pragma unroll
      for (int kt = 0; kt < 2; ++kt) {
#pragma unroll
        for (int i = 0; i < 16; ++i) sT[kt][i] = 0.f;
#pragma unroll
        for (int s = 0; s < 4; ++s) {
          const d16x8 kf = *reinterpret_cast<const d16x8*>(Ks + (kt * 32 + r) * PA_LDK + s * 16 + h * 8);
          sT[kt] = mfma32(kf, qf[s], sT[kt]);
        }
      }
      const bool need_mask = (kv0 + 64 > S) || (kv0 + 63 > q0);
      float mx = -INFINITY;
      if (need_mask) {
#pragma unroll
        for (int kt = 0; kt < 2; ++kt)
#pragma unroll
          for (int i = 0; i < 16; ++i) {
            const int key = kv0 + kt * 32 + acc_row(i, h);
            const float v = (key < S && key <= qi) ? sT[kt][i] : -INFINITY;
            sT[kt][i] = v;
            mx = fmaxf(mx, v);
          }
      } else {
#pragma unroll
        for (int kt = 0; kt < 2; ++kt)
#pragma unroll
          for (int i = 0; i < 16; ++i) mx = fmaxf(mx, sT[kt][i]);
      }
      mx = fmaxf(mx, xhalf(mx));
      const float mnew = fmaxf(mrun, mx);
      const float c = a.scale_log2e;
      const float alpha = __builtin_amdgcn_exp2f((mrun - mnew) * c);
      mrun = mnew;
      const float mc = -mnew * c;
      float ps = 0.f;
#pragma unroll
      for (int kt = 0; kt < 2; ++kt)
#pragma unroll
        for (int i = 0; i < 16; ++i) { const float p = __builtin_amdgcn_exp2f(fmaf(sT[kt][i], c, mc)); sT[kt][i] = p; ps += p; }
      lrun = lrun * alpha + ps;
#pragma unroll
      for (int t = 0; t < 2; ++t)
#pragma unroll
        for (int i = 0; i < 16; ++i) o[t][i] *= alpha;
#pragma unroll
      for (int ks = 0; ks < 4; ++ks) {
        d16x8 pf;
#pragma unroll
        for (int j = 0; j < 8; ++j) pf[j] = (d16)sT[ks >> 1][8 * (ks & 1) + j];
#pragma unroll
        for (int dt = 0; dt < 2; ++dt) {
          const pa_s16x4 lo = __builtin_amdgcn_ds_read_tr16_b64_v4i16((pa_lds_s16x4)(vtr + (ks * 16) * PA_LDV + dt * 32));
          const pa_s16x4 hi = __builtin_amdgcn_ds_read_tr16_b64_v4i16((pa_lds_s16x4)(vtr + (ks * 16 + 8) * PA_LDV + dt * 32));
          const __attribute__((ext_vector_type(8))) short v8 = {lo[0], lo[1], lo[2], lo[3], hi[0], hi[1], hi[2], hi[3]};
          o[dt] = mfma32(__builtin_bit_cast(d16x8, v8), pf, o[dt]);
        }
      }
    }
    __syncthreads();
  }

  lrun += xhalf(lrun);
  const float inv = 1.f / lrun;
  if (qvalid) {
    d16* op = a.O + (r0 + q0 + r) * a.ldo + head * 64;
#pragma unroll
    for (int dt = 0; dt < 2; ++dt)
#pragma unroll
      for (int q = 0; q < 4; ++q) {
        const int d = dt * 32 + 8 * q + 4 * h;
        *reinterpret_cast<d16x4*>(op + d) = pack4d(o[dt][4 * q] * inv, o[dt][4 * q + 1] * inv, o[dt][4 * q + 2] * inv, o[dt][4 * q + 3] * inv);
      }
  }
}

int launch_pattn(const PAttnArgs& a, hipStream_t st) {
  if (a.n_seq <= 0 || a.max_len <= 0 || a.n_heads <= 0 || !a.Q || !a.Kc || !a.Vc || !a.O || !a.seq_row0 || !a.seq_len || !a.row_slot || a.max_len > a.max_ctx ||
      (a.ldq % 8) || (a.ldo % 4) || (((uintptr_t)a.Q | (uintptr_t)a.Kc | (uintptr_t)a.Vc) & 15) || ((uintptr_t)a.O & 7))
    ETD_FAIL(ETD_EINVAL, "pattn: bad arguments");
  ETD_LAUNCH_FILTER("k_pattn");
  ProfScope ps("k_pattn", st, a.flops_hint, ((double)a.n_seq * 4.0 * a.max_len * 64 * a.n_heads) * 2);
  dim3 g((a.max_len + 127) / 128, a.n_seq * a.n_heads);
  hipLaunchKernelGGL(k_pattn, g, dim3(256), 0, st, a);
  HIP_TRY(hipGetLastError());
  return ETD_OK;
}

#define PQ_EPP 136
#define PQ_TILE_ELEMS (32 * 512)
typedef const __attribute__((address_space(1))) void* pq_gptr_t;
typedef __attribute__((address_space(3))) void* pq_lptr_t;

template <int NW>
__global__ __launch_bounds__(64 * NW) void k_pqkv(PQkvArgs a) {
  __shared__ __attribute__((aligned(16))) unsigned char smem[2 * PQ_TILE_ELEMS * 2 + NW * 32 * PQ_EPP * 2 + 1536 * 4];
  d16* ring = reinterpret_cast<d16*>(smem);
  d16* stg_all = reinterpret_cast<d16*>(smem + 2 * PQ_TILE_ELEMS * 2);
  float* sb = reinterpret_cast<float*>(smem + 2 * PQ_TILE_ELEMS * 2 + NW * 32 * PQ_EPP * 2);
  const int tid = threadIdx.x, lane = tid & 63, wave = __builtin_amdgcn_readfirstlane(tid >> 6), r = lane & 31, h = lane >> 5;
  d16* stg = stg_all + wave * (32 * PQ_EPP);
  const int NT = a.N >> 5;
  const int mw = blockIdx.x * (32 * NW) + wave * 32;
  const int m = mw + r, mc = m < a.M ? m : a.M - 1;

  auto issue = [&](int t) {
    constexpr int PW = 32 / NW;
    const d16* src = a.Wf + (long long)t * PQ_TILE_ELEMS + wave * (PW * 512) + lane * 8;
    d16* dst = ring + (t & 1) * PQ_TILE_ELEMS + wave * (PW * 512);
    __builtin_amdgcn_global_load_lds((pq_gptr_t)src, (pq_lptr_t)dst, 16, 0, 0);
    __builtin_amdgcn_global_load_lds((pq_gptr_t)src, (pq_lptr_t)dst, 16, 1024, 0);
    __builtin_amdgcn_global_load_lds((pq_gptr_t)src, (pq_lptr_t)dst, 16, 2048, 0);
    __builtin_amdgcn_global_load_lds((pq_gptr_t)src, (pq_lptr_t)dst, 16, 3072, 0);
    if constexpr (PW == 8) {
      __builtin_amdgcn_global_load_lds((pq_gptr_t)(src + 2048), (pq_lptr_t)(dst + 2048), 16, 0, 0);
      __builtin_amdgcn_global_load_lds((pq_gptr_t)(src + 2048), (pq_lptr_t)(dst + 2048), 16, 1024, 0);
      __builtin_amdgcn_global_load_lds((pq_gptr_t)(src + 2048), (pq_lptr_t)(dst + 2048), 16, 2048, 0);
      __builtin_amdgcn_global_load_lds((pq_gptr_t)(src + 2048), (pq_lptr_t)(dst + 2048), 16, 3072, 0);
    }
  };
  issue(0);
  for (int i = tid; i < a.N; i += 64 * NW) sb[i] = a.bias[i];
  d16x8 xf[32];
  {
    const d16* xp = a.X + (long long)mc * a.ldx + 8 * h;
#pragma unroll
    for (int s = 0; s < 32; ++s) xf[s] = *reinterpret_cast<const d16x8*>(xp + 16 * s);
  }
  const int pos_l = a.rows.pos[mc];
  const f32x4 c4 = *reinterpret_cast<const f32x4*>(a.rope_cos + (long long)pos_l * 8 + 4 * h);
  const f32x4 s4 = *reinterpret_cast<const f32x4*>(a.rope_sin + (long long)pos_l * 8 + 4 * h);
  const int er8 = lane >> 3, ec8 = lane & 7;
  long long qoff[4], coff[4];
#pragma unroll
  for (int it = 0; it < 4; ++it) {
    const int mr = mw + it * 8 + er8, mrc = mr < a.M ? mr : a.M - 1;
    const int rpos = a.rows.pos[mrc], rslot = a.rows.slot[mrc], ract = a.rows.active[mrc];
    qoff[it] = mr < a.M ? (long long)mr * (a.n_heads * 64) + ec8 * 8 : -1;
    coff[it] = (mr < a.M && ract && rpos < a.max_ctx) ? (long long)rslot * a.slot_stride + (long long)rpos * 64 + ec8 * 8 : -1;
  }
  const unsigned ring_l = (unsigned)reinterpret_cast<uintptr_t>(ring) + lane * 16;

  auto store_block = [&](int u) {
    const int head = u / 3, part = u - head * 3;
    d16* cbase = (part == 1 ? a.Kc : a.Vc) + (long long)head * a.max_ctx * 64;
#pragma unroll
    for (int it = 0; it < 4; ++it) {
      const u32x4 val = *reinterpret_cast<const u32x4*>(stg + (it * 8 + er8) * PQ_EPP + ec8 * 8);
      if (part == 0) { if (qoff[it] >= 0) *reinterpret_cast<u32x4*>(a.Qb + qoff[it] + head * 64) = val; }
      else if (coff[it] >= 0) *reinterpret_cast<u32x4*>(cbase + coff[it]) = val;
    }
  };
#define PQ_RD4(buf, F0)                                                                                                  \
  do {                                                                                                                   \
    asm volatile("ds_read_b128 %0, %1 offset:%2" : "=v"(buf[0]) : "v"(sl), "n"((F0) * 1024));                            \
    asm volatile("ds_read_b128 %0, %1 offset:%2" : "=v"(buf[1]) : "v"(sl), "n"((F0) * 1024 + 1024));                     \
    asm volatile("ds_read_b128 %0, %1 offset:%2" : "=v"(buf[2]) : "v"(sl), "n"((F0) * 1024 + 2048));                     \
    asm volatile("ds_read_b128 %0, %1 offset:%2" : "=v"(buf[3]) : "v"(sl), "n"((F0) * 1024 + 3072));                     \
  } while (0)
#define PQ_MFMA(c, af, bfr) asm volatile(ETD_MFMA16_DEC " %0, %1, %2, %0" : "+v"(c) : "v"(af), "v"(bfr))
#define PQ_MFMA0(c, af, bfr) asm volatile(ETD_MFMA16_DEC " %0, %1, %2, 0" : "=&v"(c) : "v"(af), "v"(bfr))
#define PQ_GROUP(c, G)                                                                                                   \
  do {                                                                                                                   \
    if constexpr ((G) < 7) { PQ_RD4(wf[((G) + 1) & 1], ((G) + 1) * 4); asm volatile("s_waitcnt lgkmcnt(4)" ::: "memory"); } \
    else asm volatile("s_waitcnt lgkmcnt(0)" ::: "memory");                                                              \
    if constexpr ((G) == 0) PQ_MFMA0(c, wf[0][0], xf[0]); else PQ_MFMA(c, wf[(G) & 1][0], xf[4 * (G)]);                  \
    PQ_MFMA(c, wf[(G) & 1][1], xf[4 * (G) + 1]);                                                                         \
    PQ_MFMA(c, wf[(G) & 1][2], xf[4 * (G) + 2]);                                                                         \
    PQ_MFMA(c, wf[(G) & 1][3], xf[4 * (G) + 3]);                                                                         \
    __builtin_amdgcn_sched_barrier(0);                                                                                   \
  } while (0)
#define PQ_TILE(c, t)                                                                                                    \
  do {                                                                                                                   \
    asm volatile("s_waitcnt vmcnt(0) lgkmcnt(0)" ::: "memory");    \
    __syncthreads();                                               \
    if ((t) + 1 < NT) issue((t) + 1);                                                                                    \
    if ((t) >= 2 && !((t) & 1)) store_block(((t) - 2) >> 1);                                                              \
    const unsigned sl = ring_l + ((t) & 1) * (PQ_TILE_ELEMS * 2);                                                        \
    d16x8 wf[2][4];                                                                                                     \
    asm volatile("s_waitcnt lgkmcnt(0)" ::: "memory");             \
    __builtin_amdgcn_sched_barrier(0);                                                                                   \
    PQ_RD4(wf[0], 0);                                                                                                    \
    PQ_GROUP(c, 0); PQ_GROUP(c, 1); PQ_GROUP(c, 2); PQ_GROUP(c, 3); PQ_GROUP(c, 4); PQ_GROUP(c, 5); PQ_GROUP(c, 6); PQ_GROUP(c, 7); \
  } while (0)
  for (int u = 0; u < (NT >> 1); ++u) {
    f32x16 c0, c1;
    PQ_TILE(c0, 2 * u);
    PQ_TILE(c1, 2 * u + 1);
    asm volatile("s_nop 15\n\ts_nop 15" : "+v"(c1) : : "memory");
    {
      const int part = u % 3;
      float v[2][16];
#pragma unroll
      for (int i = 0; i < 16; ++i) { v[0][i] = c0[i] + sb[64 * u + acc_row(i, h)]; v[1][i] = c1[i] + sb[64 * u + 32 + acc_row(i, h)]; }
      if (part < 2) {
#pragma unroll
        for (int i = 0; i < 4; ++i) {
          const float x1 = v[0][i], x2 = v[0][i + 4];
          v[0][i] = x1 * c4[i] - x2 * s4[i];
          v[0][i + 4] = x2 * c4[i] + x1 * s4[i];
        }
      }
#pragma unroll
      for (int nn = 0; nn < 2; ++nn)
#pragma unroll
        for (int q = 0; q < 4; ++q)
          *reinterpret_cast<d16x4*>(stg + r * PQ_EPP + nn * 32 + 8 * q + 4 * h) = pack4d(v[nn][4 * q], v[nn][4 * q + 1], v[nn][4 * q + 2], v[nn][4 * q + 3]);
    }
  }
#undef PQ_TILE
#undef PQ_GROUP
#undef PQ_MFMA
#undef PQ_MFMA0
#undef PQ_RD4
  store_block((NT >> 1) - 1);
}

int launch_pqkv(const PQkvArgs& a, hipStream_t st) {
  if (a.M <= 0 || a.N != 1536 || a.ldx < 512 || (a.ldx % 8) || !a.X || !a.Wf || !a.bias || !a.Qb || !a.Kc || !a.Vc || !a.rows.pos || !a.rows.slot || !a.rows.active ||
      !a.rope_cos || !a.rope_sin || a.n_heads != 8 || (((uintptr_t)a.X | (uintptr_t)a.Wf | (uintptr_t)a.Qb | (uintptr_t)a.Kc | (uintptr_t)a.Vc) & 15) || (a.slot_stride % 8))
    ETD_FAIL(ETD_EINVAL, "pqkv: bad arguments");
  ETD_LAUNCH_FILTER("k_pqkv");
  ProfScope ps("k_pqkv", st, 2.0 * a.M * a.N * 512.0, ((double)a.M * 512 + (double)a.N * 512 + 3.0 * a.M * 512) * 2);
  static const int nw = getenv("ETD_PQKV_WAVES") ? atoi(getenv("ETD_PQKV_WAVES")) : 8;
  if (nw == 4) hipLaunchKernelGGL(k_pqkv<4>, dim3((a.M + 127) / 128), dim3(256), 0, st, a);
  else hipLaunchKernelGGL(k_pqkv<8>, dim3((a.M + 255) / 256), dim3(512), 0, st, a);
  HIP_TRY(hipGetLastError());
  return ETD_OK;
}
```

include/etude_hip_debug.h:

```cpp
#ifndef ETUDE_HIP_DEBUG_H
#define ETUDE_HIP_DEBUG_H
#include "etude_hip.h"

#ifdef __cplusplus
extern "C" {
#endif

int etd_debug_boundary_cost(int n_nodes, int iters, int big_args, void* stream, double* eager_us, double* graph_us);
int etd_debug_linear(int M, int N, int K, int iters, void* stream, double* us);
int etd_debug_kernel_loop(int which, int iters, void* stream);
int etd_debug_empty_launch(int gx, int gy, int gz, int* sink_dev, void* stream);

int etd_extractor_debug_vel_logits(etd_ext*, float* vel_logits_dev);
int etd_extractor_debug_tap(etd_ext*, int stage, void* dst_dev);

int etd_debug_assemble_prompt(const etd_sched_cfg* cfg, int n_hist, const int32_t* const* hx, const int32_t* hxn, const int32_t* const* hy,
                              const int32_t* hyn, const int32_t* hattrs4, const int32_t* x, int xn, const int32_t* y_attrs4,
                              int32_t* ids_out, int32_t* cls_out, int32_t* attrs4_out, int cap, int* T_out);
int etd_debug_assemble_scored(const etd_sched_cfg* cfg, int n_hist, const int32_t* const* hx, const int32_t* hxn, const int32_t* const* hy,
                              const int32_t* hyn, const int32_t* hattrs4, const int32_t* x, int xn, const int32_t* y, int yn, const int32_t* y_attrs4,
                              int32_t* ids_out, int32_t* cls_out, int32_t* attrs4_out, int32_t* labels_out, int cap, int* T_out);

int etd_debug_decoder_checksum(etd_dec*, unsigned long long* out, int cap, void* stream);
int etd_debug_decoder_kv_rowsums(etd_dec*, unsigned* out_host, long long cap, void* stream);
int etd_debug_decoder_trace_begin(etd_dec*, int cap_steps, void* stream);
int etd_debug_decoder_trace_slabs(etd_dec*, float* out_host, long long cap_floats, int n_active, void* stream);
int etd_debug_decoder_trace_lanes(etd_dec*, float* out_host, long long cap_floats, int n_active, void* stream);
int etd_debug_decoder_trace_q(etd_dec*, float* out_host, long long cap_floats, int n_active, void* stream);
int etd_debug_decoder_peek_kv(etd_dec*, int layer, int slot, int head, int n_pos, unsigned short* k_out, unsigned short* v_out, void* stream);
int etd_debug_decoder_trace_read(etd_dec*, unsigned* out_host, long long cap_words, int n_active, int* steps_done, void* stream);

int etd_debug_decoder_force_pair(etd_dec*, int mode);
int etd_debug_decoder_step_logits(etd_dec*, int on, float* out_host, int n_active, void* stream);

int etd_debug_gemm3(const float* x_dev, int M, int K, const float* w_host, const float* bias_host, int N, float x_bound, int gelu, float* y_dev,
                    const float* ln_g_host, const float* ln_b_host, void* stream);
enum { ETD_G3_KERNEL_AUTO = 0 , ETD_G3_KERNEL_TILE = 1 , ETD_G3_KERNEL_SMALL = 2  };
enum { ETD_G3_EPI_BIAS = 0, ETD_G3_EPI_GELU = 1, ETD_G3_EPI_RESID = 2, ETD_G3_EPI_LOGITS = 3, ETD_G3_EPI_QKV = 4, ETD_G3_EPI_RELU = 6 };
typedef struct etd_debug_g3_case {
  int struct_bytes;
  int kernel, epi;
  int M, N, K, ldx, ldy;
  const float* X; long long x_elems;
  const float* W; const float* bias;
  float x_bound;
  const float* ln_g; const float* ln_b; float ln_eps;
  float* Y; long long y_elems;
  const float* add; const float* hin; float* hout; long long h_elems;
  const int32_t* pos; const int32_t* slot; const int32_t* active;
  int n_heads, max_ctx, n_slots, rope_rows;
  const float* rope_cos; const float* rope_sin;
  float* Q; long long q_elems;
  float* Kc; float* Vc; long long kv_elems;
} etd_debug_g3_case;
int etd_debug_gemm3_case(const etd_debug_g3_case* c, void* stream);
int etd_debug_ln_rows_f32(const float* h_dev, int M, int H, const float* g1_host, const float* b1_host, const float* g2_host, const float* b2_host, float eps,
                          float* x1_dev, float* x2_dev, void* stream);
int etd_debug_g3_pack(const float* W, int N, int K, uint16_t* planes_out, long long cap, long long* n_out, int32_t* log2_out);

int etd_debug_attn3(const float* q_dev, const float* k_dev, const float* v_dev, float* o_dev, int n_seq, int n_heads, int Sq, int Sk, float q_bound, float k_bound, float v_bound,
                    int causal, const int32_t* lens_host, void* stream);

int etd_debug_g3_bounds(const float* W, const float* c, int N, int K, const float* g, const float* b, float elem_bound, float* out4, int32_t* log2_out4);

int etd_beat_debug_taps(etd_beat*, float* front_dev, float* layer0_dev);

int etd_dbn_debug_viterbi(etd_dbn*, int hmm_index, const double* densities_dev, long long T, int32_t* path_out, double* logprob_out);

int etd_dtw_debug_cost(etd_dtw*, const float* const* feat_ptrs, long long N1, long long N2, int shift, float* cost_dev);
int etd_dtw_debug_total(etd_dtw*, const float* const* feat_ptrs, long long N1, long long N2, int shift, double* total_host);
int etd_dtw_debug_path(etd_dtw*, const float* const* feat_ptrs, long long N1, long long N2, int shift, int32_t* path_host, long long cap, long long* n_out);

#ifdef __cplusplus
}
#endif
#endif
```

Measured before the change: 579.2.

## Skip Q projection in last prefill layer; add chained attention units option

In the final prefill layer only the tail rows need outputs, so the fused QKV prefill kernel gains a SKIPQ variant that skips the Q-column tiles and reschedules tile issue and stores around the skipped groups. Separately, the paired-row decode attention kernel gains a CHAIN mode in which one workgroup processes several (row-pair, head) units and prefetches the next unit's first KV block. CHAIN is gated behind a debug setter that defaults to zero, so only the Q-skip runs by default. The Q skip depends on the last-row path not needing Q from this kernel, and a stray SS_FLUSH was removed.

```diff
diff --git a/etude_amd/_lib.py b/etude_amd/_lib.py
--- a/etude_amd/_lib.py
+++ b/etude_amd/_lib.py
@@ -189,6 +189,7 @@
     "etd_decoder_stamp": (C.c_int, [C.c_void_p, C.c_int, C.c_int, C.c_void_p]),
     "etd_decoder_stamp_log": (C.c_int, [C.c_void_p, C.c_void_p, C.c_longlong, C.POINTER(C.c_longlong), C.c_void_p]),
     "etd_debug_decoder_force_pair": (C.c_int, [C.c_void_p, C.c_int]),
+    "etd_debug_decoder_attn_units": (C.c_int, [C.c_void_p, C.c_int]),
     "etd_debug_decoder_step_logits": (C.c_int, [C.c_void_p, C.c_int, C.c_void_p, C.c_int, C.c_void_p]),
     "etd_debug_decoder_checksum": (C.c_int, [C.c_void_p, C.POINTER(C.c_ulonglong), C.c_int, C.c_void_p]),
     "etd_debug_decoder_kv_rowsums": (C.c_int, [C.c_void_p, C.c_void_p, C.c_longlong, C.c_void_p]),
diff --git a/etude_amd/csrc/api_dec.hip b/etude_amd/csrc/api_dec.hip
--- a/etude_amd/csrc/api_dec.hip
+++ b/etude_amd/csrc/api_dec.hip
@@ -73,6 +73,7 @@
   double attn_bytes_hint = 0;
   bool step_pair = false;
   double stat_steps = 0, stat_row_steps = 0, stat_kv_bytes = 0, stat_attn_launches = 0, stat_stamp_bytes = 0;
+  int attn_units = 0;
   int force_pair = -1;
   unsigned long long* stamp_dev = nullptr;
   bool stamp_on = false, stamp_armed = false; long long stamp_skip = 0;
@@ -314,7 +315,7 @@
   const Layer& w = d->layers[l]; const NextLn nx = next_ln(d, l);
   const int ksd = d->I / 512;
   DAttnArgs at = attn_args(d, l, rows, M);
-  attn_step_pairs(d, &at); attn_stamp(d, l, &at); at.pair = d->step_pair ? 1 : 0;
+  attn_step_pairs(d, &at); attn_stamp(d, l, &at); at.pair = d->step_pair ? 1 : 0; at.units = d->attn_units;
   at.dense_w = (const d16*)w.dense_hw; at.dense_out = d->Pk + (size_t)ksd * M * d->H; at.dbg = (d->trace && l == 0) ? d->trace_dbg : nullptr;
   DGemmArgs dn = lin_args(w.cat, nullptr, d->I + d->H, M); dn.Xb = d->Xcat; dn.k_splits = ksd; dn.Y = d->Pk; dn.ldy = d->H;
   if (rowfin_on() && ksd + d->nh == 12 && M <= DS_STEP_MAX_ROWS) {
@@ -353,7 +354,7 @@
   return ETD_OK;
 }
 
-static int prefill16_qkv(etd_dec* d, int l, const float* hin, const DecRows& rows, int M, bool mfma_attn, hipStream_t st) {
+static int prefill16_qkv(etd_dec* d, int l, const float* hin, const DecRows& rows, int M, bool mfma_attn, bool skip_q, hipStream_t st) {
   const Layer& w = d->layers[l];
   DGemmArgs q = qkv_args(d, l, hin, rows, M); q.Xb = d->X1b; q.Y = d->qkv_raw; q.ldy = 3 * d->H;
   if (mfma_attn) q.Qb = d->Qb;
@@ -362,6 +363,7 @@
   PQkvArgs pa = {};
   pa.X = d->X1b; pa.ldx = d->H; pa.Wf = (const d16*)w.qkv.Wf; pa.bias = w.qkv.b; pa.M = M; pa.N = w.qkv.N; pa.rows = rows;
   pa.rope_cos = d->rope_cos; pa.rope_sin = d->rope_sin; pa.Qb = d->Qb; pa.Kc = (d16*)q.Kc; pa.Vc = (d16*)q.Vc; pa.slot_stride = d->slot_stride; pa.max_ctx = d->ctx; pa.n_heads = d->nh;
+  pa.skip_q = skip_q ? 1 : 0;
   return launch_pqkv(pa, st);
 }
 static int prefill16_layer_rest(etd_dec* d, int l, const DecRows& rows, int M, const PrefillInfo* pf, bool fmlp, const float* hin, float* hout, hipStream_t st) {
@@ -400,8 +402,9 @@
   float* hin = d->h; float* hout = d->h2;
   for (int l = 0; l < d->L; ++l) {
     if (l == 0 || !fmlp) ETD_TRY(ln_rows16(d, l, hin, M, st));
-    ETD_TRY(prefill16_qkv(d, l, hin, rows, M, pf != nullptr, st));
-    ETD_TRY(tail && l == d->L - 1 ? prefill16_last_rows(d, *lo, hin, hout, st) : prefill16_layer_rest(d, l, rows, M, pf, fmlp, hin, hout, st));
+    const bool last_rows = tail && l == d->L - 1;
+    ETD_TRY(prefill16_qkv(d, l, hin, rows, M, pf != nullptr, last_rows && !getenv("ETD_NO_LAST_Q_SKIP"), st));
+    ETD_TRY(last_rows ? prefill16_last_rows(d, *lo, hin, hout, st) : prefill16_layer_rest(d, l, rows, M, pf, fmlp, hin, hout, st));
     std::swap(hin, hout);
   }
   *hfinal = hin; if (tail) *compact = true;
@@ -1076,6 +1079,15 @@
   return ETD_OK;
 }
 
+extern "C" int etd_debug_decoder_attn_units(etd_dec* d, int units) {
+  if (!d || units < 0 || units > DS_STEP_MAX_ROWS * 4) ETD_FAIL(ETD_EINVAL, "attn_units: bad arguments");
+  HIP_TRY(hipDeviceSynchronize());
+  for (auto& kv : d->graphs) (void)hipGraphExecDestroy(kv.second);
+  d->graphs.clear();
+  d->attn_units = units;
+  return ETD_OK;
+}
+
 extern "C" int etd_debug_decoder_step_logits(etd_dec* d, int on, float* out_host, int n_active, void* stream) {
   hipStream_t st = (hipStream_t)stream;
   if (!d || n_active < 0 || n_active > d->S) ETD_FAIL(ETD_EINVAL, "step_logits: bad arguments");
diff --git a/etude_amd/csrc/dec_kernels.h b/etude_amd/csrc/dec_kernels.h
--- a/etude_amd/csrc/dec_kernels.h
+++ b/etude_amd/csrc/dec_kernels.h
@@ -92,6 +92,7 @@
   float* dbg;
   unsigned long long* stamp;
   int stamp_par;
+  int units;
 };
 int launch_dattn(const DAttnArgs& a, bool kv_bf16, hipStream_t st);
 struct DRowFin {
@@ -124,6 +125,7 @@
   const float* rope_cos; const float* rope_sin;
   d16* Qb;
   d16* Kc; d16* Vc; long long slot_stride; int max_ctx, n_heads;
+  int skip_q;
 };
 int launch_pqkv(const PQkvArgs& a, hipStream_t st);
 
diff --git a/etude_amd/csrc/dec_kernels.hip b/etude_amd/csrc/dec_kernels.hip
--- a/etude_amd/csrc/dec_kernels.hip
+++ b/etude_amd/csrc/dec_kernels.hip
@@ -881,7 +881,6 @@
     }
   }
   HSTAMP(4);
-  SS_FLUSH(0, 0);
 }
 
 #ifdef ETD_HEAD_STAMP
@@ -1133,31 +1132,43 @@
   asm volatile("v_add_f32 %0, %1, %2" : "=v"(r) : "v"(t), "v"(u));
   return r;
 }
-template <typename KVT, bool DENSE, int NW, bool FIN = false, bool PAIR = false>
-__device__ __forceinline__ void dattn_core(const int m, const int head, float (&red)[NW][8][10], float* osh, float* outsh,
+template <typename KVT, bool DENSE, int NW, bool FIN = false, bool PAIR = false, bool CHAIN = false>
+__device__ __forceinline__ void dattn_core(int m, int head, float (&red)[NW][8][10], float* osh, float* outsh,
                                            const int* p_row_sp, const float* p_Q, const void* p_Kc, const void* p_Vc, long long p_slot_stride,
                                            int p_max_ctx, int p_n_heads, float p_scale, int p_identity, const DAttnArgs& a, const DRowFin* fin = nullptr,
-                                           const float* osh_other = nullptr, float* outsh_other = nullptr, bool dup = false) {
-  const int tid = PAIR ? (int)(threadIdx.x & (64 * NW - 1)) : (int)threadIdx.x, lane = tid & 63, wave = tid >> 6, j = lane >> 3, c = lane & 7;
-  SS_DECL(); SS(0);
+                                           const float* osh_other = nullptr, float* outsh_other = nullptr, bool dup = false, int lid = 0, const int lid_end = 1) {
+  static_assert(!CHAIN || (PAIR && DENSE && !FIN), "unit chaining: the paired-rows form only");
+  SS_DECL();
   constexpr int G2 = 8 * NW;
   constexpr int KI = 16 * NW;
-  int slot, pos;
   typedef int i32x2 __attribute__((ext_vector_type(2)));
   Raw8<KVT> kA, kB, wA, wB, nkA, nkB, nwA, nwB;
-  if (p_identity) {
-    const KVT* kb0 = reinterpret_cast<const KVT*>(p_Kc) + (long long)m * p_slot_stride + (long long)head * p_max_ctx * 64;
-    const KVT* vb0 = reinterpret_cast<const KVT*>(p_Vc) + (long long)m * p_slot_stride + (long long)head * p_max_ctx * 64;
+  bool ahead = false; int pos_ahead = 0;
+  for (;;) {
+  int tid_ = PAIR ? (int)(threadIdx.x & (64 * NW - 1)) : (int)threadIdx.x;
+  if constexpr (CHAIN) asm volatile("" : "+v"(tid_));
+  const int tid = tid_, lane = tid & 63, wave = tid >> 6, j = lane >> 3, c = lane & 7;
+  auto first_block = [&](int m_, int head_, Raw8<KVT>& a_, Raw8<KVT>& b_, Raw8<KVT>& c_, Raw8<KVT>& d_) {
+    const KVT* kb0 = reinterpret_cast<const KVT*>(p_Kc) + (long long)m_ * p_slot_stride + (long long)head_ * p_max_ctx * 64;
+    const KVT* vb0 = reinterpret_cast<const KVT*>(p_Vc) + (long long)m_ * p_slot_stride + (long long)head_ * p_max_ctx * 64;
     const int ka = wave * 8 + j, kbb = ka + G2;
-    kA.load(kb0 + (long long)ka * 64 + c * 8); kB.load(kb0 + (long long)kbb * 64 + c * 8);
-    wA.load(vb0 + (long long)ka * 64 + c * 8); wB.load(vb0 + (long long)kbb * 64 + c * 8);
+    a_.load(kb0 + (long long)ka * 64 + c * 8); b_.load(kb0 + (long long)kbb * 64 + c * 8);
+    c_.load(vb0 + (long long)ka * 64 + c * 8); d_.load(vb0 + (long long)kbb * 64 + c * 8);
+  };
+  SS(0);
+  int slot, pos;
+  if (CHAIN && ahead) { kA = nkA; kB = nkB; wA = nwA; wB = nwB; slot = m; pos = pos_ahead; }
+  else if (p_identity) {
+    first_block(m, head, kA, kB, wA, wB);
     slot = m; pos = __builtin_nontemporal_load(p_row_sp + 2 * m + 1);
   } else if (p_row_sp) { const i32x2 sp = __builtin_nontemporal_load(reinterpret_cast<const i32x2*>(p_row_sp + 2 * m)); slot = sp[0]; pos = sp[1]; }
   else { slot = a.rows.slot[m]; pos = a.rows.pos[m]; }
   const int ctx = (pos < p_max_ctx ? pos : p_max_ctx - 1) + 1;
   const int hidden = p_n_heads * 64;
   constexpr bool FAST = sizeof(KVT) == 2;
-  const float qs = FAST ? p_scale * 1.4426950408889634f : p_scale;
+  float scale_ = p_scale;
+  if constexpr (CHAIN) asm volatile("" : "+s"(scale_));
+  const float qs = FAST ? scale_ * 1.4426950408889634f : scale_;
   float q[8];
   {
     const float* qp = p_Q + (long long)m * hidden + head * 64 + c * 8;
@@ -1216,6 +1227,20 @@
 
   SS(2);
   constexpr int FR = PAIR ? 64 / (2 * NW) : 64 / NW, FP = FR > 8 ? 8 : FR, NPASS = FR / FP;
+  int m_nx = m, head_nx = head; bool dup_nx = dup;
+  if constexpr (CHAIN) {
+    ahead = false;
+    if (lid + 1 < lid_end) {
+      const int P = (a.M + 1) >> 1, pr = (lid + 1) % P;
+      head_nx = (lid + 1) / P; m_nx = 2 * pr + __builtin_amdgcn_readfirstlane((int)(threadIdx.x >> 8));
+      dup_nx = m_nx >= a.M; m_nx = dup_nx ? 2 * pr : m_nx;
+      if (p_identity) {
+        ahead = true;
+        first_block(m_nx, head_nx, nkA, nkB, nwA, nwB);
+        pos_ahead = __builtin_nontemporal_load(p_row_sp + 2 * m_nx + 1);
+      }
+    }
+  }
   const int dwave = PAIR ? (int)(threadIdx.x >> 6) : wave;
   constexpr int DROWS = PAIR ? 512 / (2 * NW) : 512 / NW;
   d16x8 dwv[DENSE ? FP : 1];
@@ -1373,6 +1398,12 @@
       SS(5); SS_FLUSH(2, 0);
     }
   }
+  if constexpr (!CHAIN) break;
+  else {
+    if (++lid >= lid_end) break;
+    m = m_nx; head = head_nx; dup = dup_nx;
+  }
+  }
 }
 __device__ __forceinline__ void attn_stamp_begin(unsigned long long* stp, int par, int flat_block) {
   if (stp && flat_block == 0 && threadIdx.x < 64) {
@@ -1417,7 +1448,7 @@
 #ifndef ETD_FIN_OCC
 #define ETD_FIN_OCC 4
 #endif
-template <int NW, bool FIN, bool PAIR = false>
+template <int NW, bool FIN, bool PAIR = false, bool CHAIN = false>
 __device__ __forceinline__ void dstep_attn_down_body(const int* p_row_sp, const float* p_Q, const void* p_Kc, const void* p_Vc, long long p_slot_stride,
                                                      int p_max_ctx, int p_n_heads, float p_scale, int p_identity, int p_gemm_wgs, int p_M,
                                                      const DAttnArgs& a, const DGemmArgs& g, const DRowFin& fin) {
@@ -1428,13 +1459,15 @@
   if constexpr (PAIR) {
     static_assert(!PAIR || (NW == 8 && !FIN), "paired rows: 8 waves, no in-launch row finish");
     if ((int)blockIdx.x >= p_gemm_wgs) {
-      const int lid = blockIdx.x - p_gemm_wgs, P = (p_M + 1) >> 1, pr = lid % P, half = threadIdx.x >> 8;
+      const int P = (p_M + 1) >> 1, half = CHAIN ? __builtin_amdgcn_readfirstlane((int)(threadIdx.x >> 8)) : (int)(threadIdx.x >> 8);
+      const int lid = CHAIN ? (int)(blockIdx.x - p_gemm_wgs) * a.units : (int)(blockIdx.x - p_gemm_wgs), pr = lid % P;
+      const int lid_end = CHAIN ? (lid + a.units < P * p_n_heads ? lid + a.units : P * p_n_heads) : lid + 1;
       int m = 2 * pr + half;
       const bool dup = m >= p_M;
       m = dup ? 2 * pr : m;
       float (&redh)[4][8][10] = *reinterpret_cast<float (*)[4][8][10]>(&red[4 * half][0][0]);
-      dattn_core<d16, true, 4, false, true>(m, lid / P, redh, osh + 64 * half, sh + 512 * half, p_row_sp, p_Q, p_Kc, p_Vc, p_slot_stride, p_max_ctx, p_n_heads, p_scale, p_identity, a,
-                                             nullptr, osh + 64 * (half ^ 1), sh + 512 * (half ^ 1), dup);
+      dattn_core<d16, true, 4, false, true, CHAIN>(m, lid / P, redh, osh + 64 * half, sh + 512 * half, p_row_sp, p_Q, p_Kc, p_Vc, p_slot_stride, p_max_ctx, p_n_heads, p_scale, p_identity, a,
+                                                    nullptr, osh + 64 * (half ^ 1), sh + 512 * (half ^ 1), dup, lid, lid_end);
       return;
     }
   }
@@ -1508,12 +1541,12 @@
   }
 }
 
-template <int NW, bool FIN, bool PAIR = false>
+template <int NW, bool FIN, bool PAIR = false, bool CHAIN = false>
 __global__ __launch_bounds__(64 * NW) __attribute__((amdgpu_waves_per_eu(FIN ? ETD_FIN_OCC : (PAIR ? ETD_AD_OCC : AdOcc<NW>::lo), AdOcc<NW>::hi))) void k_dstep_attn_down(const int* p_row_sp, const float* p_Q, const void* p_Kc, const void* p_Vc, long long p_slot_stride,
                                                          int p_max_ctx, int p_n_heads, float p_scale, int p_identity, int p_gemm_wgs, int p_M,
                                                          DAttnArgs a, DGemmArgs g, DRowFin fin) {
   attn_stamp_begin(a.stamp, a.stamp_par, (int)blockIdx.x);
-  dstep_attn_down_body<NW, FIN, PAIR>(p_row_sp, p_Q, p_Kc, p_Vc, p_slot_stride, p_max_ctx, p_n_heads, p_scale, p_identity, p_gemm_wgs, p_M, a, g, fin);
+  dstep_attn_down_body<NW, FIN, PAIR, CHAIN>(p_row_sp, p_Q, p_Kc, p_Vc, p_slot_stride, p_max_ctx, p_n_heads, p_scale, p_identity, p_gemm_wgs, p_M, a, g, fin);
   attn_stamp_end(a.stamp, a.stamp_par, (int)blockIdx.x);
 }
 
@@ -1525,6 +1558,10 @@
 #else
   return 4;
 #endif
+}
+static int ad_chain_units(const DAttnArgs& a, int n_units) {
+  if (a.units >= 1) return a.units < n_units ? a.units : n_units;
+  return 1;
 }
 int launch_dstep_attn_down(const DAttnArgs& a, const DGemmArgs& g, const DRowFin* fin, hipStream_t st) {
 #ifndef ETD_EXPERIMENTS
@@ -1547,7 +1584,13 @@
 #define ETD_AD_LAUNCH(NW_, FIN_) hipLaunchKernelGGL((k_dstep_attn_down<NW_, FIN_>), dim3(gemm_wgs + a.M * a.n_heads), dim3(64 * NW_), 0, st, a.row_sp, a.Q, a.Kc, a.Vc, a.slot_stride, a.max_ctx, a.n_heads, a.scale, \
                                               a.identity ? 1 : 0, gemm_wgs, a.M, a, g, f0)
   if (pair) {
-    hipLaunchKernelGGL((k_dstep_attn_down<8, false, true>), dim3(gemm_wgs + ((a.M + 1) / 2) * a.n_heads), dim3(512), 0, st, a.row_sp, a.Q, a.Kc, a.Vc, a.slot_stride, a.max_ctx, a.n_heads, a.scale,
+    const int n_units = ((a.M + 1) / 2) * a.n_heads, U = ad_chain_units(a, n_units);
+    if (U > 1) {
+      DAttnArgs ac = a; ac.units = U;
+      hipLaunchKernelGGL((k_dstep_attn_down<8, false, true, true>), dim3(gemm_wgs + (n_units + U - 1) / U), dim3(512), 0, st, a.row_sp, a.Q, a.Kc, a.Vc, a.slot_stride, a.max_ctx, a.n_heads, a.scale,
+                         a.identity ? 1 : 0, gemm_wgs, a.M, ac, g, f0);
+    } else
+    hipLaunchKernelGGL((k_dstep_attn_down<8, false, true>), dim3(gemm_wgs + n_units), dim3(512), 0, st, a.row_sp, a.Q, a.Kc, a.Vc, a.slot_stride, a.max_ctx, a.n_heads, a.scale,
                        a.identity ? 1 : 0, gemm_wgs, a.M, a, g, f0);
   } else
 #ifdef ETD_EXPERIMENTS
diff --git a/etude_amd/csrc/dec_prefill.hip b/etude_amd/csrc/dec_prefill.hip
--- a/etude_amd/csrc/dec_prefill.hip
+++ b/etude_amd/csrc/dec_prefill.hip
@@ -159,7 +159,7 @@
 typedef const __attribute__((address_space(1))) void* pq_gptr_t;
 typedef __attribute__((address_space(3))) void* pq_lptr_t;
 
-template <int NW>
+template <int NW, bool SKIPQ = false>
 __global__ __launch_bounds__(64 * NW) void k_pqkv(PQkvArgs a) {
   __shared__ __attribute__((aligned(16))) unsigned char smem[2 * PQ_TILE_ELEMS * 2 + NW * 32 * PQ_EPP * 2 + 1536 * 4];
   d16* ring = reinterpret_cast<d16*>(smem);
@@ -186,7 +186,7 @@
       __builtin_amdgcn_global_load_lds((pq_gptr_t)(src + 2048), (pq_lptr_t)(dst + 2048), 16, 3072, 0);
     }
   };
-  issue(0);
+  issue(SKIPQ ? 2 : 0);
   for (int i = tid; i < a.N; i += 64 * NW) sb[i] = a.bias[i];
   d16x8 xf[32];
   {
@@ -237,12 +237,12 @@
     PQ_MFMA(c, wf[(G) & 1][3], xf[4 * (G) + 3]);                                                                         \
     __builtin_amdgcn_sched_barrier(0);                                                                                   \
   } while (0)
-#define PQ_TILE(c, t)                                                                                                    \
+#define PQ_TILE(c, t, tn, us)                                                                                            \
   do {                                                                                                                   \
     asm volatile("s_waitcnt vmcnt(0) lgkmcnt(0)" ::: "memory");    \
     __syncthreads();                                               \
-    if ((t) + 1 < NT) issue((t) + 1);                                                                                    \
-    if ((t) >= 2 && !((t) & 1)) store_block(((t) - 2) >> 1);                                                              \
+    if ((tn) < NT) issue(tn);                                                                                            \
+    if ((us) >= 0) store_block(us);                                                                                      \
     const unsigned sl = ring_l + ((t) & 1) * (PQ_TILE_ELEMS * 2);                                                        \
     d16x8 wf[2][4];                                                                                                     \
     asm volatile("s_waitcnt lgkmcnt(0)" ::: "memory");             \
@@ -250,10 +250,13 @@
     PQ_RD4(wf[0], 0);                                                                                                    \
     PQ_GROUP(c, 0); PQ_GROUP(c, 1); PQ_GROUP(c, 2); PQ_GROUP(c, 3); PQ_GROUP(c, 4); PQ_GROUP(c, 5); PQ_GROUP(c, 6); PQ_GROUP(c, 7); \
   } while (0)
+  int up = -1;
   for (int u = 0; u < (NT >> 1); ++u) {
+    if (SKIPQ && u % 3 == 0) continue;
+    const int un = (SKIPQ && (u + 1) % 3 == 0) ? u + 2 : u + 1;
     f32x16 c0, c1;
-    PQ_TILE(c0, 2 * u);
-    PQ_TILE(c1, 2 * u + 1);
+    PQ_TILE(c0, 2 * u, 2 * u + 1, up);
+    PQ_TILE(c1, 2 * u + 1, 2 * un, -1);
     asm volatile("s_nop 15\n\ts_nop 15" : "+v"(c1) : : "memory");
     {
       const int part = u % 3;
@@ -274,13 +277,14 @@
         for (int q = 0; q < 4; ++q)
           *reinterpret_cast<d16x4*>(stg + r * PQ_EPP + nn * 32 + 8 * q + 4 * h) = pack4d(v[nn][4 * q], v[nn][4 * q + 1], v[nn][4 * q + 2], v[nn][4 * q + 3]);
     }
+    up = u;
   }
 #undef PQ_TILE
 #undef PQ_GROUP
 #undef PQ_MFMA
 #undef PQ_MFMA0
 #undef PQ_RD4
-  store_block((NT >> 1) - 1);
+  store_block(up);
 }
 
 int launch_pqkv(const PQkvArgs& a, hipStream_t st) {
@@ -288,10 +292,12 @@
       !a.rope_cos || !a.rope_sin || a.n_heads != 8 || (((uintptr_t)a.X | (uintptr_t)a.Wf | (uintptr_t)a.Qb | (uintptr_t)a.Kc | (uintptr_t)a.Vc) & 15) || (a.slot_stride % 8))
     ETD_FAIL(ETD_EINVAL, "pqkv: bad arguments");
   ETD_LAUNCH_FILTER("k_pqkv");
-  ProfScope ps("k_pqkv", st, 2.0 * a.M * a.N * 512.0, ((double)a.M * 512 + (double)a.N * 512 + 3.0 * a.M * 512) * 2);
+  const double nf = a.skip_q ? 1024.0 : a.N, np = a.skip_q ? 2.0 : 3.0;
+  ProfScope ps("k_pqkv", st, 2.0 * a.M * nf * 512.0, ((double)a.M * 512 + nf * 512 + np * a.M * 512) * 2);
   static const int nw = getenv("ETD_PQKV_WAVES") ? atoi(getenv("ETD_PQKV_WAVES")) : 8;
-  if (nw == 4) hipLaunchKernelGGL(k_pqkv<4>, dim3((a.M + 127) / 128), dim3(256), 0, st, a);
-  else hipLaunchKernelGGL(k_pqkv<8>, dim3((a.M + 255) / 256), dim3(512), 0, st, a);
+  if (nw == 4) { if (a.skip_q) hipLaunchKernelGGL((k_pqkv<4, true>), dim3((a.M + 127) / 128), dim3(256), 0, st, a); else hipLaunchKernelGGL((k_pqkv<4>), dim3((a.M + 127) / 128), dim3(256), 0, st, a); }
+  else if (a.skip_q) hipLaunchKernelGGL((k_pqkv<8, true>), dim3((a.M + 255) / 256), dim3(512), 0, st, a);
+  else hipLaunchKernelGGL((k_pqkv<8>), dim3((a.M + 255) / 256), dim3(512), 0, st, a);
   HIP_TRY(hipGetLastError());
   return ETD_OK;
 }
diff --git a/include/etude_hip_debug.h b/include/etude_hip_debug.h
--- a/include/etude_hip_debug.h
+++ b/include/etude_hip_debug.h
@@ -31,6 +31,7 @@
 int etd_debug_decoder_trace_read(etd_dec*, unsigned* out_host, long long cap_words, int n_active, int* steps_done, void* stream);
 
 int etd_debug_decoder_force_pair(etd_dec*, int mode);
+int etd_debug_decoder_attn_units(etd_dec*, int units);
 int etd_debug_decoder_step_logits(etd_dec*, int on, float* out_host, int n_active, void* stream);
 
 int etd_debug_gemm3(const float* x_dev, int M, int K, const float* w_host, const float* bias_host, int N, float x_bound, int gelu, float* y_dev,
```

Result: no change. 580.2, median of 3 (+0.2%).
